# NVlabs/InstantSplat

Hardware: AMD Instinct MI355X
Metric: train_iters_per_sec (higher is better)
Workload: dtype f32

## Files before the change

### include/mi355gs.h

```cpp
#ifndef MI355GS_H
#define MI355GS_H

#include <stddef.h>
#include <stdint.h>

#ifdef __cplusplus
extern "C" {
#endif

#define MI355GS_ABI_VERSION 10

#define MI355GS_OK 0
#define MI355GS_EINVAL (-1)
#define MI355GS_ELAUNCH (-2)
#define MI355GS_EOVERFLOW (-3)

int mi355gs_abi_version(void);
const char* mi355gs_error_string(int code);

size_t mi355gs_raster_geom_bytes(int P);
size_t mi355gs_raster_tiles_bytes(int W, int H);
size_t mi355gs_raster_binning_bytes(int64_t num_instances, int W, int H);

int mi355gs_raster_forward_preprocess(
    void* stream, int P, int D, int M, int W, int H,
    const float* means3D, const float* shs, const float* shs_rest, const float* colors_precomp, const float* opacities,
    const float* scales, float scale_modifier, const float* rotations, const float* cov3D_precomp,
    const float* viewmatrix, const float* projmatrix, const float* campos,
    float tanfovx, float tanfovy, int prefiltered,
    int32_t* radii, void* geom, void* tiles, int32_t* num_rendered, uint8_t* visible, void* grad_scratch, int debug);

int mi355gs_raster_forward_render(
    void* stream, int P, int W, int H, int64_t capacity, const float* bg,
    const void* geom, void* tiles, void* binning, float* out_color, int debug);

size_t mi355gs_raster_binning_bytes_render_only(int64_t num_instances, int W, int H);
int mi355gs_raster_forward_render_only(
    void* stream, int P, int W, int H, int64_t capacity, const float* bg,
    const void* geom, void* tiles, void* binning, float* out_color, int debug);

size_t mi355gs_raster_grad_scratch_bytes(int P);
size_t mi355gs_raster_grad_gate_offset(int P);
int mi355gs_raster_backward(
    void* stream, int P, int D, int M, int W, int H, const float* bg,
    const float* means3D, const float* shs, const float* shs_rest, const float* colors_precomp, const float* opacities,
    const float* scales, float scale_modifier, const float* rotations, const float* cov3D_precomp,
    const float* viewmatrix, const float* projmatrix, const float* campos,
    float tanfovx, float tanfovy,
    const void* geom, void* tiles, const void* binning, int64_t capacity, const int32_t* radii,
    const float* out_color, const float* dL_dpix, void* grad_scratch,
    float* dL_dmeans3D, float* dL_dmeans2D, float* dL_dshs, float* dL_dshs_rest, float* dL_dcolors, float* dL_dopacities,
    float* dL_dscales, float* dL_drotations, float* dL_dcov3D, int grad_scratch_is_clear, int debug);

int mi355gs_raster_mark_visible(void* stream, int P, const float* means3D, const float* viewmatrix,
                                const float* projmatrix, uint8_t* present);

int mi355gs_raster_frame_stats(void* stream, int W, int H, const void* tiles, int64_t* stats);

int mi355gs_tune_min_units(int min_units);

int mi355gs_tune_deterministic(int on);

int mi355gs_tune_scale_grad(int mode);

int mi355gs_profile_begin(void);
int mi355gs_profile_set_period(int every);
int mi355gs_profile_work_counters(void* counters);
int mi355gs_profile_read(int kind, double* total_ms, int* launches);
int mi355gs_profile_end(void);
int mi355gs_profile_ranges(int on);

size_t mi355gs_ssim_scratch_bytes(int B, int C, int H, int W);
int mi355gs_ssim_forward(void* stream, int B, int C, int H, int W, const float* img1, const float* img2,
                         float* dm_dmu1, float* dm_dsigma1_sq, float* dm_dsigma12,
                         void* scratch, float* ssim_mean, float* l1_mean, int padding_valid);
int mi355gs_ssim_backward(void* stream, int B, int C, int H, int W, const float* img1, const float* img2,
                          const float* dm_dmu1, const float* dm_dsigma1_sq, const float* dm_dsigma12,
                          const float* ssim_grad_scale, const float* l1_grad_scale, float* dL_dimg1, int padding_valid);
int mi355gs_l1_ssim_loss_fused(void* stream, int B, int C, int H, int W, const float* img1, const float* img2, void* scratch,
                               float lambda_dssim, float* ssim_mean, float* l1_mean, float* loss, float* dloss_dimg1);

size_t mi355gs_l1_scratch_bytes(int64_t n);
int mi355gs_l1_loss_forward(void* stream, int64_t n, const float* a, const float* b, void* scratch, float* mean_out);
int mi355gs_l1_loss_backward(void* stream, int64_t n, const float* a, const float* b, const float* grad_scale, float* d_a);
#define MI355GS_LOSS_PROGRAM_MAX 16
#define MI355GS_LOSS_OP_L1 0
#define MI355GS_LOSS_OP_SSIM 1
#define MI355GS_LOSS_OP_MULK 2
#define MI355GS_LOSS_OP_ADDK 3
#define MI355GS_LOSS_OP_RSUBK 4
#define MI355GS_LOSS_OP_DIVK 5
#define MI355GS_LOSS_OP_NEG 6
#define MI355GS_LOSS_OP_ADD 7
#define MI355GS_LOSS_OP_SUB 8
int mi355gs_l1_ssim_pair_forward(void* stream, int B, int C, int H, int W, const float* img1, const float* img2, void* scratch,
                                 float* dssim_dimg1);
int mi355gs_l1_ssim_pair_backward(void* stream, int64_t n, const float* img1, const float* img2, const float* dssim_dimg1,
                                  const float* g_l1, float c_l1, const float* g_ssim, float c_ssim, float* d_img1);
int mi355gs_loss_program_eval(void* stream, int n_ops, const int32_t* ops, const float* consts, int B, int C, int H, int W,
                              const void* scratch, float* ssim_mean, float* l1_mean, float* out, float* host_out, float ticket);
int mi355gs_loss_program_eval_grad(void* stream, int n_ops, const int32_t* ops, const float* consts, int B, int C, int H, int W,
                                   const void* scratch, float* ssim_mean, float* l1_mean, float* out, float* host_out, float ticket,
                                   const float* img1, const float* img2, const float* dssim_dimg1, float c_l1, float c_ssim, float* d_img1);

size_t mi355gs_knn_scratch_bytes(int N);
int mi355gs_knn_dist2(void* stream, int N, const float* points, float* mean_dist2, void* scratch);

int mi355gs_adam_step(void* stream, int64_t n, int row, float* param, const float* grad, float* exp_avg,
                      float* exp_avg_sq, const float* per_point_lr, const float* grad_sumsq,
                      float lr, float beta1, float beta2, float eps, int step);

int mi355gs_adam_multi_step(void* stream, int ntensors, const int64_t* numel, const int32_t* row, float* const* params,
                            const float* const* grads, float* const* exp_avg, float* const* exp_avg_sq,
                            const float* const* per_point_lr, const float* lr, float beta1, float beta2, float eps,
                            const int32_t* step, float* scratch, const float* gate, const int32_t* gate_index,
                            uint32_t* live, uint32_t seq);

int mi355gs_pose_forward(void* stream, int P, const float* xyz, const float* rot, const float* scaling,
                         const float* opacity_logit, const float* pose, float* means_cam, float* rot_cam, float* scales,
                         float* opac);
int mi355gs_pose_backward(void* stream, int P, const float* xyz, const float* rot, const float* scales, const float* opac,
                          const float* pose, const float* g_means, const float* g_rot, const float* g_scales,
                          const float* g_opac, float* d_xyz, float* d_rot, float* d_scaling, float* d_opacity_logit,
                          float* d_pose, float* scratch);

int mi355gs_posed_forward_preprocess(void* stream, int P, int D, int W, int H, const float* xyz, const float* f_dc,
                                     const float* f_rest, const float* opacity_logit, const float* log_scales, float scale_modifier,
                                     const float* rotation, const float* pose, const float* view_identity, const float* projmatrix,
                                     const float* origin, float tanfovx, float tanfovy, int32_t* radii, void* geom, void* tiles,
                                     int32_t* num_rendered, uint8_t* visible, void* grad_scratch, int debug);
int mi355gs_posed_backward(void* stream, int P, int D, int W, int H, const float* bg, const float* xyz, const float* f_dc,
                           const float* f_rest, const float* opacity_logit, const float* log_scales, float scale_modifier,
                           const float* rotation, const float* pose, const float* view_identity, const float* projmatrix,
                           const float* origin, float tanfovx, float tanfovy, const void* geom, void* tiles, const void* binning,
                           int64_t capacity, const int32_t* radii, const float* out_color, const float* dL_dpix,
                           void* grad_scratch, float* pose_scratch, float* d_xyz, float* d_means2D, float* d_f_dc, float* d_f_rest,
                           float* d_opacity_logit, float* d_log_scales, float* d_rotation, float* d_pose, int pose_rows, int pose_row,
                           int grad_scratch_is_clear, int debug);

size_t mi355gs_trainer_workspace_bytes(int P, int W, int H, int V, int64_t capacity);
void* mi355gs_trainer_create(int P, int W, int H, int V, int64_t capacity, float* xyz, float* f_dc, float* f_rest, float* opacity,
                             float* scaling, float* rotation, float* poses, float* const* exp_avg, float* const* exp_avg_sq,
                             const float* per_point_lr, void* workspace);
int mi355gs_trainer_step(void* trainer, void* stream, int view, int sh_degree, const float* gt_image, const float* projmatrix,
                         float tanfovx, float tanfovy, const float* bg, const float* lr, const int32_t* step, float beta1, float beta2, float eps,
                         float lambda_dssim, int do_optimizer_step, float* loss_out, int32_t* num_rendered_out);
int mi355gs_trainer_optimizer_step(void* trainer, void* stream, const float* lr, const int32_t* step, float beta1, float beta2,
                                   float eps, int commit_gate);
void mi355gs_trainer_destroy(void* trainer);
const float* mi355gs_trainer_grad(void* trainer, int k);

#define MI355GS_TRACKER_STATE_FLOATS 40
#define MI355GS_TRACKER_POSE 0
#define MI355GS_TRACKER_EXP_AVG 8
#define MI355GS_TRACKER_EXP_AVG_SQ 16
#define MI355GS_TRACKER_BEST 24
#define MI355GS_TRACKER_INITIAL 25
#define MI355GS_TRACKER_FLAG 26
#define MI355GS_TRACKER_COUNT 27
#define MI355GS_TRACKER_CAND 32
size_t mi355gs_tracker_workspace_bytes(int P, int W, int H, int64_t capacity);
void* mi355gs_tracker_create(int P, int M, int W, int H, int64_t capacity, const float* xyz, const float* f_dc, const float* f_rest,
                             const float* opacity, const float* scaling, const float* rotation, void* workspace);
int mi355gs_tracker_count(void* tracker, void* stream, int sh_degree, const float* projmatrix, float tanfovx, float tanfovy,
                          const float* pose, int32_t* count_out);
int mi355gs_tracker_run(void* tracker, void* stream, int sh_degree, const float* gt_image, const float* projmatrix, float tanfovx,
                        float tanfovy, const float* bg, const float* sched, int num_iter, int first_iter, int n_iters, float* state,
                        float* pose_trace, float* loss_trace, float* grad_trace);
void mi355gs_tracker_destroy(void* tracker);

int mi355gs_rgb8_from_planar(void* stream, int H, int W, const float* img, uint8_t* out);
size_t mi355gs_path_workspace_bytes(int P, int W, int H, int64_t capacity);
void* mi355gs_path_create(int P, int M, int W, int H, int64_t capacity, const float* xyz, const float* f_dc, const float* f_rest,
                          const float* opacity, const float* scaling, const float* rotation, void* workspace);
int mi355gs_path_render(void* path, void* stream, int sh_degree, const float* projmatrix, float tanfovx, float tanfovy,
                        const float* bg, const float* poses, int first, int n, uint8_t* frames, int32_t* counts);
void mi355gs_path_destroy(void* path);

size_t mi355gs_metrics_rgb8_scratch_bytes(int N, int H, int W);
int mi355gs_metrics_rgb8(void* stream, int N, int H, int W, const uint8_t* a, const uint8_t* b, void* scratch, int64_t* sq_sum,
                         float* ssim_mean);

size_t mi355gs_lpips_vgg_scratch_bytes(int N, int H, int W, const int channels[5]);
int mi355gs_lpips_vgg_rgb8(void* stream, int N, int H, int W, const uint8_t* a, const uint8_t* b, const int channels[5],
                           const float* weights, void* scratch, float* lpips, float* taps);

size_t mi355gs_png_rgb8_scratch_bytes(int N, int H, int W, int rows_per_block);
size_t mi355gs_png_rgb8_stream_bytes(int N, int H, int W, int rows_per_block);
int mi355gs_png_rgb8(void* stream, int N, int H, int W, int rows_per_block, const uint8_t* frames, void* scratch, uint8_t* out,
                     int64_t* offsets);

size_t mi355gs_jpeg_rgb8_scratch_bytes(int N, int H, int W, int subsampling);
size_t mi355gs_jpeg_rgb8_stream_bytes(int N, int H, int W, int subsampling);
int mi355gs_jpeg_rgb8(void* stream, int N, int H, int W, int subsampling, const uint8_t* qtables, const uint8_t* frames, void* scratch,
                      uint8_t* out, size_t out_bytes, int64_t* offsets);

size_t mi355gs_pointmap_stats_scratch_bytes(int V, int H, int W);
int mi355gs_pointmap_stats(void* stream, int V, int H, int W, const float* depthmaps, const float* confidences, uint8_t* overlap,
                           void* scratch, double* stats);
int mi355gs_covis_masks(void* stream, int V, int H, int W, const int32_t* order, const float* pointmaps, const float* depthmaps,
                        const float* intrinsics, const float* w2c, const double* stats, float depth_threshold, uint8_t* overlap);
size_t mi355gs_compact_scratch_bytes(int64_t n);
int mi355gs_compact_pointmaps(void* stream, int64_t n, const uint8_t* overlap, const float* pointmaps, const float* images,
                              const float* confidences, void* scratch, float* out_points, uint8_t* out_rgb8, float* out_confidence,
                              int32_t* count_dev, int32_t* count_host);

#define MI355GS_ALIGN_OPT_DEPTH 1
#define MI355GS_ALIGN_OPT_IM_POSES 2
#define MI355GS_ALIGN_OPT_FOCALS 4
#define MI355GS_ALIGN_OPT_PW_POSES 8
#define MI355GS_ALIGN_NORM_PW_SCALE 16
size_t mi355gs_align_workspace_bytes(int V, int H, int W, int E, int flags);
void* mi355gs_align_create(void* workspace, int V, int H, int W, const int32_t* edges, int E, int flags, float base_scale);
void mi355gs_align_destroy(void* handle);
int mi355gs_align_pack(void* handle, void* stream, const float* pred_i, const float* pred_j, const float* conf_i, const float* conf_j);
int mi355gs_align_grad(void* handle, void* stream, const float* depth_log, const float* im_pose, const float* focal_log, const float* pp_raw,
                       const float* pw_pose, float* g_depth_log, float* g_im_pose, float* g_focal_log, float* g_pw_pose, float* loss);
int mi355gs_align_run(void* handle, void* stream, int niter, const float* step_table, float* depth_log, float* im_pose, float* focal_log,
                      const float* pp_raw, float* pw_pose, float* m_depth_log, float* v_depth_log, float* m_im_pose, float* v_im_pose,
                      float* m_focal_log, float* v_focal_log, float* m_pw_pose, float* v_pw_pose, float* losses);
int mi355gs_align_points(void* handle, void* stream, const float* depth_log, const float* im_pose, const float* focal_log,
                         const float* pp_raw, const float* pw_pose, float* pts3d, float* depth);
const float* mi355gs_align_records(void* handle);

size_t mi355gs_align_init_workspace_bytes(int B, int n);
int mi355gs_align_init_means(void* workspace, void* stream, int rows, int n, const float* x, float* means);
int mi355gs_align_init_register(void* workspace, void* stream, int B, int n, const float* src, const int32_t* src_idx, long long src_job_stride,
                                int src_pt_stride, const float* tgt, const int32_t* tgt_idx, long long tgt_job_stride, const float* weights,
                                const int32_t* w_idx, long long w_job_stride, float* srt, float* pw_pose);
int mi355gs_align_init_apply(void* stream, int n, const float* src, int src_pt_stride, const float* srt, float* dst);
int mi355gs_align_init_focals(void* workspace, void* stream, int B, int H, int W, const float* src, const int32_t* src_idx,
                              long long src_job_stride, int src_pt_stride, float* focals);
int mi355gs_align_init_state(void* workspace, void* stream, int V, int E, int H, int W, int norm_pw_scale, float base_scale, int focal_mode,
                             float known_focal, const float* srt, const int32_t* pose_row, const float* focals, const int32_t* focal_row,
                             const float* pw_pose, float* pts3d, float* depth_log, float* im_pose, float* focal_log);

#ifdef __cplusplus
}
#endif
#endif
```

### instantsplat_amd/_lib.py

```python
from __future__ import annotations

import ctypes
import os
from ctypes import c_float, c_int, c_int64, c_size_t, c_void_p

import torch

_HERE = os.path.dirname(os.path.abspath(__file__))
LIB_PATH = os.path.join(_HERE, "lib", "libmi355gs.so")
_LIB = None
_TEST_MODE = False

_P = c_void_p
_SIGNATURES = {
    "mi355gs_abi_version": (c_int, []),
    "mi355gs_error_string": (ctypes.c_char_p, [c_int]),
    "mi355gs_raster_geom_bytes": (c_size_t, [c_int]),
    "mi355gs_raster_tiles_bytes": (c_size_t, [c_int, c_int]),
    "mi355gs_raster_binning_bytes": (c_size_t, [c_int64, c_int, c_int]),
    "mi355gs_raster_grad_scratch_bytes": (c_size_t, [c_int]),
    "mi355gs_raster_grad_gate_offset": (c_size_t, [c_int]),
    "mi355gs_raster_forward_preprocess": (c_int, [_P, c_int, c_int, c_int, c_int, c_int, _P, _P, _P, _P, _P, _P, c_float, _P, _P,
                                                  _P, _P, _P, c_float, c_float, c_int, _P, _P, _P, _P, _P, _P, c_int]),
    "mi355gs_raster_forward_render": (c_int, [_P, c_int, c_int, c_int, c_int64, _P, _P, _P, _P, _P, c_int]),
    "mi355gs_raster_binning_bytes_render_only": (c_size_t, [c_int64, c_int, c_int]),
    "mi355gs_raster_forward_render_only": (c_int, [_P, c_int, c_int, c_int, c_int64, _P, _P, _P, _P, _P, c_int]),
    "mi355gs_raster_backward": (c_int, [_P, c_int, c_int, c_int, c_int, c_int, _P, _P, _P, _P, _P, _P, _P, c_float, _P, _P, _P, _P,
                                        _P, c_float, c_float, _P, _P, _P, c_int64, _P, _P, _P, _P, _P, _P, _P, _P, _P, _P, _P, _P, _P,
                                        c_int, c_int]),
    "mi355gs_raster_mark_visible": (c_int, [_P, c_int, _P, _P, _P, _P]),
    "mi355gs_raster_frame_stats": (c_int, [_P, c_int, c_int, _P, _P]),
    "mi355gs_tune_min_units": (c_int, [c_int]),
    "mi355gs_tune_scale_grad": (c_int, [c_int]),
    "mi355gs_tune_deterministic": (c_int, [c_int]),
    "mi355gs_profile_begin": (c_int, []),
    "mi355gs_profile_set_period": (c_int, [c_int]),
    "mi355gs_profile_work_counters": (c_int, [_P]),
    "mi355gs_profile_read": (c_int, [c_int, ctypes.POINTER(ctypes.c_double), ctypes.POINTER(c_int)]),
    "mi355gs_profile_end": (c_int, []),
    "mi355gs_profile_ranges": (c_int, [c_int]),
    "mi355gs_ssim_scratch_bytes": (c_size_t, [c_int, c_int, c_int, c_int]),
    "mi355gs_ssim_forward": (c_int, [_P, c_int, c_int, c_int, c_int, _P, _P, _P, _P, _P, _P, _P, _P, c_int]),
    "mi355gs_ssim_backward": (c_int, [_P, c_int, c_int, c_int, c_int, _P, _P, _P, _P, _P, _P, _P, _P, c_int]),
    "mi355gs_l1_ssim_loss_fused": (c_int, [_P, c_int, c_int, c_int, c_int, _P, _P, _P, c_float, _P, _P, _P, _P]),
    "mi355gs_l1_ssim_pair_forward": (c_int, [_P, c_int, c_int, c_int, c_int, _P, _P, _P, _P]),
    "mi355gs_l1_ssim_pair_backward": (c_int, [_P, c_int64, _P, _P, _P, _P, c_float, _P, c_float, _P]),
    "mi355gs_loss_program_eval": (c_int, [_P, c_int, _P, _P, c_int, c_int, c_int, c_int, _P, _P, _P, _P, _P, c_float]),
    "mi355gs_loss_program_eval_grad": (c_int, [_P, c_int, _P, _P, c_int, c_int, c_int, c_int, _P, _P, _P, _P, _P, c_float, _P, _P, _P, c_float,
                                               c_float, _P]),
    "mi355gs_knn_scratch_bytes": (c_size_t, [c_int]),
    "mi355gs_knn_dist2": (c_int, [_P, c_int, _P, _P, _P]),
    "mi355gs_adam_step": (c_int, [_P, c_int64, c_int, _P, _P, _P, _P, _P, _P, c_float, c_float, c_float, c_float, c_int]),
    "mi355gs_adam_multi_step": (c_int, [_P, c_int, _P, _P, _P, _P, _P, _P, _P, _P, c_float, c_float, c_float, _P, _P, _P, _P, _P,
                                        ctypes.c_uint32]),
    "mi355gs_pose_forward": (c_int, [_P, c_int, _P, _P, _P, _P, _P, _P, _P, _P, _P]),
    "mi355gs_pose_backward": (c_int, [_P, c_int, _P, _P, _P, _P, _P, _P, _P, _P, _P, _P, _P, _P, _P, _P, _P]),
    "mi355gs_posed_forward_preprocess": (c_int, [_P, c_int, c_int, c_int, c_int, _P, _P, _P, _P, _P, c_float, _P, _P, _P, _P, _P,
                                                 c_float, c_float, _P, _P, _P, _P, _P, _P, c_int]),
    "mi355gs_posed_backward": (c_int, [_P, c_int, c_int, c_int, c_int, _P, _P, _P, _P, _P, _P, c_float, _P, _P, _P, _P, _P, c_float,
                                       c_float, _P, _P, _P, c_int64, _P, _P, _P, _P, _P, _P, _P, _P, _P, _P, _P, _P, _P, c_int, c_int, c_int, c_int]),
    "mi355gs_l1_scratch_bytes": (c_size_t, [c_int64]),
    "mi355gs_l1_loss_forward": (c_int, [_P, c_int64, _P, _P, _P, _P]),
    "mi355gs_l1_loss_backward": (c_int, [_P, c_int64, _P, _P, _P, _P]),
    "mi355gs_trainer_workspace_bytes": (c_size_t, [c_int, c_int, c_int, c_int, c_int64]),
    "mi355gs_trainer_create": (c_void_p, [c_int, c_int, c_int, c_int, c_int64, _P, _P, _P, _P, _P, _P, _P, _P, _P, _P, _P]),
    "mi355gs_trainer_step": (c_int, [_P, _P, c_int, c_int, _P, _P, c_float, c_float, _P, _P, _P, c_float, c_float, c_float, c_float,
                                     c_int, _P, _P]),
    "mi355gs_trainer_optimizer_step": (c_int, [_P, _P, _P, _P, c_float, c_float, c_float, c_int]),
    "mi355gs_trainer_destroy": (None, [_P]),
    "mi355gs_trainer_grad": (_P, [_P, c_int]),
    "mi355gs_tracker_workspace_bytes": (c_size_t, [c_int, c_int, c_int, c_int64]),
    "mi355gs_tracker_create": (c_void_p, [c_int, c_int, c_int, c_int, c_int64, _P, _P, _P, _P, _P, _P, _P]),
    "mi355gs_tracker_count": (c_int, [_P, _P, c_int, _P, c_float, c_float, _P, _P]),
    "mi355gs_tracker_run": (c_int, [_P, _P, c_int, _P, _P, c_float, c_float, _P, _P, c_int, c_int, c_int, _P, _P, _P, _P]),
    "mi355gs_tracker_destroy": (None, [_P]),
    "mi355gs_rgb8_from_planar": (c_int, [_P, c_int, c_int, _P, _P]),
    "mi355gs_path_workspace_bytes": (c_size_t, [c_int, c_int, c_int, c_int64]),
    "mi355gs_path_create": (c_void_p, [c_int, c_int, c_int, c_int, c_int64, _P, _P, _P, _P, _P, _P, _P]),
    "mi355gs_path_render": (c_int, [_P, _P, c_int, _P, c_float, c_float, _P, _P, c_int, c_int, _P, _P]),
    "mi355gs_path_destroy": (None, [_P]),
    "mi355gs_metrics_rgb8_scratch_bytes": (c_size_t, [c_int, c_int, c_int]),
    "mi355gs_metrics_rgb8": (c_int, [_P, c_int, c_int, c_int, _P, _P, _P, _P, _P]),
    "mi355gs_png_rgb8_scratch_bytes": (c_size_t, [c_int, c_int, c_int, c_int]),
    "mi355gs_png_rgb8_stream_bytes": (c_size_t, [c_int, c_int, c_int, c_int]),
    "mi355gs_png_rgb8": (c_int, [_P, c_int, c_int, c_int, c_int, _P, _P, _P, _P]),
    "mi355gs_jpeg_rgb8_scratch_bytes": (c_size_t, [c_int, c_int, c_int, c_int]),
    "mi355gs_jpeg_rgb8_stream_bytes": (c_size_t, [c_int, c_int, c_int, c_int]),
    "mi355gs_jpeg_rgb8": (c_int, [_P, c_int, c_int, c_int, c_int, _P, _P, _P, _P, c_size_t, _P]),
    "mi355gs_lpips_vgg_scratch_bytes": (c_size_t, [c_int, c_int, c_int, _P]),
    "mi355gs_lpips_vgg_rgb8": (c_int, [_P, c_int, c_int, c_int, _P, _P, _P, _P, _P, _P, _P]),
    "mi355gs_pointmap_stats_scratch_bytes": (c_size_t, [c_int, c_int, c_int]),
    "mi355gs_pointmap_stats": (c_int, [_P, c_int, c_int, c_int, _P, _P, _P, _P, _P]),
    "mi355gs_covis_masks": (c_int, [_P, c_int, c_int, c_int, _P, _P, _P, _P, _P, _P, c_float, _P]),
    "mi355gs_compact_scratch_bytes": (c_size_t, [c_int64]),
    "mi355gs_compact_pointmaps": (c_int, [_P, c_int64, _P, _P, _P, _P, _P, _P, _P, _P, _P, _P]),
    "mi355gs_align_workspace_bytes": (c_size_t, [c_int, c_int, c_int, c_int, c_int]),
    "mi355gs_align_create": (c_void_p, [_P, c_int, c_int, c_int, _P, c_int, c_int, c_float]),
    "mi355gs_align_destroy": (None, [_P]),
    "mi355gs_align_pack": (c_int, [_P, _P, _P, _P, _P, _P]),
    "mi355gs_align_grad": (c_int, [_P] * 12),
    "mi355gs_align_run": (c_int, [_P, _P, c_int] + [_P] * 15),
    "mi355gs_align_points": (c_int, [_P] * 9),
    "mi355gs_align_records": (c_void_p, [_P]),
    "mi355gs_align_init_workspace_bytes": (c_size_t, [c_int, c_int]),
    "mi355gs_align_init_means": (c_int, [_P, _P, c_int, c_int, _P, _P]),
    "mi355gs_align_init_register": (c_int, [_P, _P, c_int, c_int, _P, _P, c_int64, c_int, _P, _P, c_int64, _P, _P, c_int64, _P, _P]),
    "mi355gs_align_init_apply": (c_int, [_P, c_int, _P, c_int, _P, _P]),
    "mi355gs_align_init_focals": (c_int, [_P, _P, c_int, c_int, c_int, _P, _P, c_int64, c_int, _P]),
    "mi355gs_align_init_state": (c_int, [_P, _P, c_int, c_int, c_int, c_int, c_int, c_float, c_int, c_float] + [_P] * 9),
}
EXPORTED_SYMBOLS = tuple(_SIGNATURES)


ABI_VERSION = 10


def _bind(path: str):
    lib = ctypes.CDLL(path)
    for name, (res, args) in _SIGNATURES.items():
        fn = getattr(lib, name)
        fn.restype, fn.argtypes = res, args
    got = lib.mi355gs_abi_version()
    if got != ABI_VERSION:
        raise RuntimeError(f"{path} implements ABI v{got}, this package binds v{ABI_VERSION}: rebuild it with "
                           "`python -c 'import __graft_entry__ as g; g.build()'`")
    return lib


def lib():
    global _LIB
    if _LIB is None:
        if not os.path.exists(LIB_PATH):
            raise RuntimeError(
                f"{LIB_PATH} is missing: build it with `python -c 'import __graft_entry__ as g; g.build()'` "
                "(hipcc --offload-arch=gfx950). instantsplat_amd has no CPU or PyTorch fallback.")
        _LIB = _bind(LIB_PATH)
        if os.environ.get("MI355GS_DETERMINISTIC", "0") == "1":
            _LIB.mi355gs_tune_deterministic(1)
    return _LIB


def _use_library_for_testing(path: str | None):
    global _LIB, _TEST_MODE, _EXT_BOUND_TO
    if path is None:
        _LIB, _TEST_MODE = None, False
    else:
        _LIB, _TEST_MODE = _bind(path), True
    _EXT_BOUND_TO = None


BINDING = os.environ.get("MI355GS_BINDING", "compiled")
EXT_PATH = os.path.join(_HERE, "lib", "_mi355gs_torch.so")
_EXT = None
_EXT_BOUND_TO = None


def compiled():
    global _EXT, _EXT_BOUND_TO
    if BINDING != "compiled":
        return None
    L = lib()
    if _EXT_BOUND_TO is L:
        return _EXT
    if _EXT is None:
        if not os.path.exists(EXT_PATH):
            raise RuntimeError(f"{EXT_PATH} is missing: build it with `python -c 'import __graft_entry__ as g; g.build()'` "
                               "(or set MI355GS_BINDING=ctypes to use the Python binding)")
        import importlib.util
        spec = importlib.util.spec_from_file_location("_mi355gs_torch", EXT_PATH)
        _EXT = importlib.util.module_from_spec(spec)
        spec.loader.exec_module(_EXT)
    _EXT.forget_gates()
    _EXT.bind({name: ctypes.cast(getattr(L, name), ctypes.c_void_p).value for name in _EXT.abi_symbols()}, _TEST_MODE)
    _EXT_BOUND_TO = L
    return _EXT


def check(code: int, what: str):
    if code != 0:
        raise RuntimeError(f"mi355gs: {what} failed: {lib().mi355gs_error_string(code).decode()} ({code})")


def ptr(t: torch.Tensor | None):
    return None if t is None else t.data_ptr()


_F32 = torch.float32


def f32c_on_one_device(*tensors):
    out, dev = [], None
    for t in tensors:
        if t.dtype is not _F32:
            raise RuntimeError(f"expected float32, got {t.dtype}")
        if not t.is_contiguous():
            t = t.contiguous()
        d = t.device
        if dev is None:
            if d.type != "cuda" and not _TEST_MODE:
                raise RuntimeError("instantsplat_amd operators run on the GPU only (got a CPU tensor; there is no CPU fallback)")
            dev = d
        elif d != dev:
            raise RuntimeError(f"tensors on different devices: {dev} vs {d}")
        out.append(t)
    return out, dev


def require_device(*tensors: torch.Tensor | None):
    dev = None
    for t in tensors:
        if t is None:
            continue
        if not t.is_cuda and not _TEST_MODE:
            raise RuntimeError("instantsplat_amd operators run on the GPU only (got a CPU tensor; there is no CPU fallback)")
        if not t.is_contiguous():
            raise RuntimeError("instantsplat_amd operators need contiguous tensors")
        if dev is None:
            dev = t.device
        elif t.device != dev:
            raise RuntimeError(f"tensors on different devices: {dev} vs {t.device}")
    return dev


class _NoGuard:
    def __enter__(self):
        return None

    def __exit__(self, *a):
        return False


_NO_GUARD = _NoGuard()


def on_device(device):
    if device is not None and device.type == "cuda" and device.index is not None and device.index != torch.cuda.current_device():
        return torch.cuda.device(device)
    return _NO_GUARD


def stream_ptr(device):
    if device is not None and device.type == "cuda":
        return torch.cuda.current_stream(device).cuda_stream
    return None


def f32c(t: torch.Tensor | None):
    if t is None:
        return None
    if t.dtype != torch.float32:
        raise RuntimeError(f"expected float32, got {t.dtype}")
    return t.contiguous()
```

### instantsplat_amd/csrc/ssim.hip

```cpp
#include "common.h"

namespace {

constexpr int TS = 16;
constexpr int TSX = 32;
constexpr int HALO = 5;
constexpr int TH = TS + 2 * HALO;
constexpr int THX = TSX + 2 * HALO;
constexpr int SXP = 48;
constexpr int ROW_ITEMS = TH * TS;
constexpr float C1 = 0.01f * 0.01f;
constexpr float C2 = 0.03f * 0.03f;

__device__ __forceinline__ float gw(int k) {
  constexpr float w[11] = {0.001028380123898387f, 0.0075987582094967365f, 0.036000773310661316f, 0.10936068743467331f,
                           0.21300552785396576f,  0.26601171493530273f,   0.21300552785396576f,  0.10936068743467331f,
                           0.036000773310661316f, 0.0075987582094967365f, 0.001028380123898387f};
  return w[k];
}

__device__ __forceinline__ bool ssim_equal_window(float mu1, float mu2, float exx, float eyy, float exy, bool zero_counts) {
  return mu1 == mu2 && exx == eyy && exx == exy && (zero_counts || exx != 0.f);
}

__device__ __forceinline__ float ssim_rcp(float x) {
  const float r = __builtin_amdgcn_rcpf(x);
  return fmaf(fmaf(-x, r, 1.0f), r, r);
}
__device__ __forceinline__ gs_v2f ssim_rcp(gs_v2f x) { return gs_v2f{ssim_rcp(x[0]), ssim_rcp(x[1])}; }

template <class T> struct SsimWindow { T m, d1, d2, d3, invB; };
__device__ __forceinline__ float ssim_lane(float v, int) { return v; }
__device__ __forceinline__ float ssim_lane(gs_v2f v, int h) { return v[h]; }
__device__ __forceinline__ float ssim_sum_sq(float mu1_sq, float, float mu2_sq) { return mu1_sq + mu2_sq; }
__device__ __forceinline__ gs_v2f ssim_sum_sq(gs_v2f mu1_sq, gs_v2f mu2, gs_v2f mu2_sq) {
#ifdef __clang__
  return __builtin_elementwise_fma(mu2, mu2, mu1_sq);
#else
  return mu1_sq + mu2_sq;
#endif
}
template <class T>
__device__ __forceinline__ T ssim_all(float v) {
  if constexpr (std::is_same<T, float>::value) return v;
  else return T{v, v};
}
template <class T>
__device__ __forceinline__ SsimWindow<T> ssim_window(T mu1, T mu2, T exx, T eyy, T exy) {
  const T two = ssim_all<T>(2.f), c1 = ssim_all<T>(C1), c2 = ssim_all<T>(C2);
  const T mu1_sq = mu1 * mu1, mu2_sq = mu2 * mu2, mu12 = mu1 * mu2;
  const T s1 = exx - mu1_sq, s2 = eyy - mu2_sq, s12 = exy - mu12;
  const T A = ssim_sum_sq(mu1_sq, mu2, mu2_sq) + c1, B = s1 + s2 + c2, Cc = two * mu12 + c1, Dd = two * s12 + c2;
  const T invA = ssim_rcp(A), invB = ssim_rcp(B), invAB = invA * invB;
  const T m = Cc * Dd * invAB;
  const T t = mu1 * two * Cc * Dd * invAB;
  const T d1 = (mu2 * two * Dd) * invAB - (mu2 * two * Cc) * invAB - t * invA + t * invB;
  const T d2 = -m * invB;
  const T d3 = two * Cc * invAB;
  return {m, d1, d2, d3, invB};
}
template <class T>
__device__ __forceinline__ SsimWindow<float> ssim_exact(const SsimWindow<T>& w, int h, bool same) {
  const float invB = ssim_lane(w.invB, h);
  return {same ? 1.f : ssim_lane(w.m, h), same ? 0.f : ssim_lane(w.d1, h), same ? -invB : ssim_lane(w.d2, h),
          same ? 2.f * invB : ssim_lane(w.d3, h), invB};
}

template <int N>
__device__ __forceinline__ void ssim_tile_stage(int tid, int H, int W, int ox, int oy, const float* const (&src)[N], float (*const (&dst)[N])[SXP]) {
  constexpr int ITERS = (TH * SXP + 255) / 256;
  float v[N][ITERS];
#pragma unroll
  for (int j = 0; j < ITERS; ++j) {
    const int i = tid + 256 * j, r = i / SXP, c = i - r * SXP;
    const size_t o = (size_t)min(max(oy + r - HALO, 0), H - 1) * W + min(max(ox + c - HALO, 0), W - 1);
#pragma unroll
    for (int p = 0; p < N; ++p) v[p][j] = src[p][o];
  }
#pragma unroll
  for (int j = 0; j < ITERS; ++j) {
    const int i = tid + 256 * j, r = i / SXP, c = i - r * SXP;
    const int gy = oy + r - HALO, gx = ox + c - HALO;
    const bool in = c < THX && gy >= 0 && gy < H && gx >= 0 && gx < W;
    if (i < TH * SXP) {
#pragma unroll
      for (int p = 0; p < N; ++p) dst[p][r][c] = in ? v[p][j] : 0.f;
    }
  }
}

__device__ __forceinline__ void ssim_tile_row_pass(int tid, const float (*s_x)[SXP], const float (*s_y)[SXP], gs_v2f (*s_h)[TH][TS]) {
  for (int i = tid; i < ROW_ITEMS; i += 256) {
    const int r = i >> 4, c = i & 15;
    gs_v2f sx = {0.f, 0.f}, sy = sx, sxx = sx, syy = sx, sxy = sx;
#pragma unroll
    for (int k = 0; k < 11; ++k) {
      const gs_v2f w = {gw(k), gw(k)};
      const gs_v2f x = {s_x[r][c + k], s_x[r][c + TS + k]}, y = {s_y[r][c + k], s_y[r][c + TS + k]};
      const gs_v2f wx = w * x, wy = w * y;
      sx = gs_fma2(w, x, sx); sy = gs_fma2(w, y, sy);
      sxx = gs_fma2(wx, x, sxx); syy = gs_fma2(wy, y, syy); sxy = gs_fma2(wx, y, sxy);
    }
    s_h[0][r][c] = sx; s_h[1][r][c] = sy; s_h[2][r][c] = sxx; s_h[3][r][c] = syy; s_h[4][r][c] = sxy;
  }
}
template <int N>
__device__ __forceinline__ void ssim_tile_col_pass(const gs_v2f (*s_h)[TH][TS], int ly, int lx, gs_v2f (&out)[N]) {
#pragma unroll
  for (int m = 0; m < N; ++m) out[m] = gs_v2f{0.f, 0.f};
#pragma unroll
  for (int k = 0; k < 11; ++k) {
    const gs_v2f w = {gw(k), gw(k)};
#pragma unroll
    for (int m = 0; m < N; ++m) out[m] = gs_fma2(w, s_h[m][ly + k][lx], out[m]);
  }
}

__global__ __launch_bounds__(256) void k_ssim_fwd(int H, int W, const float* __restrict__ img1, const float* __restrict__ img2,
                                                   float* __restrict__ dm_dmu1, float* __restrict__ dm_dsigma1_sq,
                                                   float* __restrict__ dm_dsigma12, float* __restrict__ partial ,
                                                   int crop ) {
  __shared__ float s_x[TH][SXP];
  __shared__ float s_y[TH][SXP];
  __shared__ gs_v2f s_h[5][TH][TS];
  __shared__ float s_red[2][4];
  const int tid = threadIdx.y * TS + threadIdx.x;
  const int plane = blockIdx.z;
  const int ox = blockIdx.x * TSX, oy = blockIdx.y * TS;
  const float* p1 = img1 + (size_t)plane * H * W;
  const float* p2 = img2 + (size_t)plane * H * W;
  ssim_tile_stage<2>(tid, H, W, ox, oy, {p1, p2}, {s_x, s_y});
  __syncthreads();
  ssim_tile_row_pass(tid, s_x, s_y, s_h);
  __syncthreads();
  const int ly = threadIdx.y, lx = threadIdx.x;
  float val = 0.f, l1 = 0.f;
  {
    gs_v2f mo[5];
    ssim_tile_col_pass(s_h, ly, lx, mo);
    const SsimWindow<gs_v2f> pair = ssim_window(mo[0], mo[1], mo[2], mo[3], mo[4]);
    const int gy = oy + ly;
#pragma unroll
    for (int half = 0; half < 2; ++half) {
      const int gx = ox + lx + half * TS;
      if (gx < W && gy < H) {
        const bool counted = gx >= crop && gx < W - crop && gy >= crop && gy < H - crop;
        const bool same = ssim_equal_window(mo[0][half], mo[1][half], mo[2][half], mo[3][half], mo[4][half], false);
        const SsimWindow<float> win = ssim_exact(pair, half, same);
        val += counted ? win.m : 0.f;
        const size_t o = (size_t)plane * H * W + (size_t)gy * W + gx;
        if (dm_dmu1) {
          dm_dmu1[o] = counted ? win.d1 : 0.f;
          dm_dsigma1_sq[o] = counted ? win.d2 : 0.f;
          dm_dsigma12[o] = counted ? win.d3 : 0.f;
        }
        l1 += fabsf(s_x[ly + HALO][lx + half * TS + HALO] - s_y[ly + HALO][lx + half * TS + HALO]);
      }
    }
  }
  val = gs_wave_sum_row3(val);
  l1 = gs_wave_sum_row3(l1);
  const int wave = tid >> 6, lane = tid & 63;
  if (lane == 63) { s_red[0][wave] = val; s_red[1][wave] = l1; }
  __syncthreads();
  if (tid == 0) {
    const size_t b = ((size_t)blockIdx.z * gridDim.y + blockIdx.y) * gridDim.x + blockIdx.x;
    partial[2 * b] = (s_red[0][0] + s_red[0][1]) + (s_red[0][2] + s_red[0][3]);
    partial[2 * b + 1] = (s_red[1][0] + s_red[1][1]) + (s_red[1][2] + s_red[1][3]);
  }
}

__global__ __launch_bounds__(1024) void k_ssim_finish(int nblocks, double inv_n, const float* __restrict__ partial,
                                                       float* __restrict__ ssim_mean, float* __restrict__ l1_mean,
                                                       float* __restrict__ loss, float lambda_dssim) {
  float sm, lm;
  gs_finish_two_means(nblocks, inv_n, partial, sm, lm);
  if (threadIdx.x == 0) {
    if (ssim_mean) *ssim_mean = sm;
    if (l1_mean) *l1_mean = lm;
    if (loss) *loss = gs_l1_ssim_loss(lambda_dssim, lm, sm);
  }
}

__global__ __launch_bounds__(256) void k_ssim_bwd(int H, int W, float inv_n, const float* __restrict__ img1, const float* __restrict__ img2,
                                                   const float* __restrict__ dm_dmu1, const float* __restrict__ dm_dsigma1_sq,
                                                   const float* __restrict__ dm_dsigma12, const float* __restrict__ ssim_scale,
                                                   const float* __restrict__ l1_scale, float ssim_scale_host, float l1_scale_host,
                                                   float* __restrict__ dL_dimg1) {
  __shared__ float s_a[TH][SXP];
  __shared__ float s_b[TH][SXP];
  __shared__ float s_c[TH][SXP];
  __shared__ gs_v2f s_h[3][TH][TS];
  const int tid = threadIdx.y * TS + threadIdx.x;
  const int plane = blockIdx.z;
  const int ox = blockIdx.x * TSX, oy = blockIdx.y * TS;
  const size_t po = (size_t)plane * H * W;
  const float ks = (ssim_scale ? *ssim_scale : 1.f) * ssim_scale_host * inv_n;
  const float kl = (l1_scale ? *l1_scale : 1.f) * l1_scale_host * inv_n;
  float px[2], py[2];
#pragma unroll
  for (int half = 0; half < 2; ++half) {
    const size_t o = po + (size_t)min(oy + (int)threadIdx.y, H - 1) * W + min(ox + (int)threadIdx.x + half * TS, W - 1);
    px[half] = img1[o]; py[half] = img2[o];
  }
  if (ks != 0.f) {
    ssim_tile_stage<3>(tid, H, W, ox, oy, {dm_dmu1 + po, dm_dsigma1_sq + po, dm_dsigma12 + po}, {s_a, s_b, s_c});
    __syncthreads();
    for (int i = tid; i < ROW_ITEMS; i += 256) {
      const int r = i >> 4, c = i & 15;
      gs_v2f a = {0.f, 0.f}, b = a, cc = a;
#pragma unroll
      for (int k = 0; k < 11; ++k) {
        const gs_v2f w = {gw(k), gw(k)};
        a = gs_fma2(w, gs_v2f{s_a[r][c + k], s_a[r][c + TS + k]}, a);
        b = gs_fma2(w, gs_v2f{s_b[r][c + k], s_b[r][c + TS + k]}, b);
        cc = gs_fma2(w, gs_v2f{s_c[r][c + k], s_c[r][c + TS + k]}, cc);
      }
      s_h[0][r][c] = a; s_h[1][r][c] = b; s_h[2][r][c] = cc;
    }
    __syncthreads();
  }
  const int ly = threadIdx.y, lx = threadIdx.x;
  const int gy = oy + ly;
  if (gy >= H) return;
  gs_v2f abc[3] = {{0.f, 0.f}, {0.f, 0.f}, {0.f, 0.f}};
  if (ks != 0.f) ssim_tile_col_pass(s_h, ly, lx, abc);
  const gs_v2f a = abc[0], b = abc[1], cc = abc[2];
#pragma unroll
  for (int half = 0; half < 2; ++half) {
    const int gx = ox + lx + half * TS;
    if (gx >= W) continue;
    const size_t o = po + (size_t)gy * W + gx;
    const float x = px[half], y = py[half];
    float g = 0.f;
    if (ks != 0.f) g = ks * ((x == y && cc[half] == -2.f * b[half]) ? a[half] : a[half] + 2.f * x * b[half] + y * cc[half]);
    if (kl != 0.f) {
      const float d = x - y;
      g += kl * (d > 0.f ? 1.f : (d < 0.f ? -1.f : 0.f));
    }
    dL_dimg1[o] = g;
  }
}


constexpr int FT = 32;
constexpr int FR1 = FT + 2 * HALO;
constexpr int FR2 = FT + 4 * HALO;
constexpr int FXP = 58;
constexpr int FHP = 43;
constexpr int FDP = 46;
constexpr int FEP = 33;
constexpr int FTHREADS = 512;
constexpr int F_STAGE_ITERS = (FR2 * FXP + FTHREADS - 1) / FTHREADS;
constexpr int FER = FT * FT / FTHREADS;
constexpr int FCR = 7, FC_GROUPS = (FR1 + FCR - 1) / FCR;
constexpr int FDR = 8, FD_GROUPS = FT / FDR;
static_assert(FC_GROUPS * FR1 <= FTHREADS && FD_GROUPS * FR1 <= FTHREADS && FT % FDR == 0 && FDR % 2 == 0, "one item per thread");

template <int RUN>
__device__ __forceinline__ void ssim_run(const float (&v)[RUN + 10], float (&out)[RUN]) {
#pragma unroll
  for (int j = 0; j < RUN; ++j) {
    float a = 0.f;
#pragma unroll
    for (int k = 0; k < 11; ++k) a = fmaf(gw(k), v[j + k], a);
    out[j] = a;
  }
}

__global__ __launch_bounds__(FTHREADS) void k_l1_ssim_fused(int H, int W, const float* __restrict__ img1, const float* __restrict__ img2,
                                                        float ks , float kl ,
                                                        float* __restrict__ dL_dimg1, float* __restrict__ partial ) {
  __shared__ float s_xy[2][FR2][FXP];
  __shared__ float s_h[5][FR2][FHP];
  static_assert(3 * FR1 * FDP <= 2 * FR2 * FXP && 3 * FR1 * FEP <= 5 * FR2 * FHP, "aliased LDS buffers must fit");
  __shared__ float s_red[2][FTHREADS / 64];
  float (*s_d)[FR1][FDP] = reinterpret_cast<float (*)[FR1][FDP]>(&s_xy[0][0][0]);
  float (*s_e)[FR1][FEP] = reinterpret_cast<float (*)[FR1][FEP]>(&s_h[0][0][0]);
  const int tid = threadIdx.x;
  const int plane = blockIdx.z;
  const int ox = blockIdx.x * FT, oy = blockIdx.y * FT;
  const size_t po = (size_t)plane * H * W;
  const float* p1 = img1 + po;
  const float* p2 = img2 + po;
  const int ec = tid & 31, er0 = (tid >> 5) * FER;
  float ex[FER], ey[FER];
#pragma unroll
  for (int j = 0; j < FER; ++j) {
    const size_t o = (size_t)min(oy + er0 + j, H - 1) * W + min(ox + ec, W - 1);
    ex[j] = p1[o]; ey[j] = p2[o];
  }
  {
    float vx[F_STAGE_ITERS], vy[F_STAGE_ITERS];
#pragma unroll
    for (int j = 0; j < F_STAGE_ITERS; ++j) {
      const int i = tid + FTHREADS * j, r = i / FXP, c = i - r * FXP;
      const size_t o = (size_t)min(max(oy + r - 2 * HALO, 0), H - 1) * W + min(max(ox + c - 2 * HALO, 0), W - 1);
      vx[j] = p1[o]; vy[j] = p2[o];
    }
#pragma unroll
    for (int j = 0; j < F_STAGE_ITERS; ++j) {
      const int i = tid + FTHREADS * j, r = i / FXP, c = i - r * FXP;
      const int gy = oy + r - 2 * HALO, gx = ox + c - 2 * HALO;
      const bool in = gy >= 0 && gy < H && gx >= 0 && gx < W;
      if (i < FR2 * FXP) { s_xy[0][r][c] = in ? vx[j] : 0.f; s_xy[1][r][c] = in ? vy[j] : 0.f; }
    }
  }
  __syncthreads();
  for (int i = tid; i < FR2 * 7; i += FTHREADS) {
    const int r = i % FR2, c0 = (i / FR2) * 6;
    float x[16], y[16];
#pragma unroll
    for (int t = 0; t < 16; t += 2) {
      const float2 a = *reinterpret_cast<const float2*>(&s_xy[0][r][c0 + t]);
      const float2 b = *reinterpret_cast<const float2*>(&s_xy[1][r][c0 + t]);
      x[t] = a.x; x[t + 1] = a.y; y[t] = b.x; y[t + 1] = b.y;
    }
    float sx[6], sy[6], sxx[6], syy[6], sxy[6];
#pragma unroll
    for (int j = 0; j < 6; ++j) { sx[j] = sy[j] = sxx[j] = syy[j] = sxy[j] = 0.f; }
#pragma unroll
    for (int t = 0; t < 16; ++t) {
      const float xx = x[t] * x[t], yy = y[t] * y[t], xy = x[t] * y[t];
#pragma unroll
      for (int j = 0; j < 6; ++j) {
        const int k = t - j;
        if (k >= 0 && k < 11) {
          const float w = gw(k);
          sx[j] = fmaf(w, x[t], sx[j]); sy[j] = fmaf(w, y[t], sy[j]);
          sxx[j] = fmaf(w, xx, sxx[j]); syy[j] = fmaf(w, yy, syy[j]); sxy[j] = fmaf(w, xy, sxy[j]);
        }
      }
    }
#pragma unroll
    for (int j = 0; j < 6; ++j) {
      s_h[0][r][c0 + j] = sx[j]; s_h[1][r][c0 + j] = sy[j]; s_h[2][r][c0 + j] = sxx[j]; s_h[3][r][c0 + j] = syy[j];
      s_h[4][r][c0 + j] = sxy[j];
    }
  }
  __syncthreads();
  float val = 0.f;
  if (tid < FR1 * FC_GROUPS) {
    const int c = tid % FR1, r0 = (tid / FR1) * FCR;
    float mo[5][FCR];
#pragma unroll
    for (int m = 0; m < 5; ++m) {
      float v[FCR + 10];
#pragma unroll
      for (int t = 0; t < FCR + 10; ++t) v[t] = s_h[m][min(r0 + t, FR2 - 1)][c];
      ssim_run(v, mo[m]);
    }
    const int gx = ox + c - HALO;
#pragma unroll
    for (int j = 0; j < FCR; ++j) {
      const int r = r0 + j, gy = oy + r - HALO;
      const SsimWindow<float> win = ssim_exact(ssim_window(mo[0][j], mo[1][j], mo[2][j], mo[3][j], mo[4][j]), 0,
                                               ssim_equal_window(mo[0][j], mo[1][j], mo[2][j], mo[3][j], mo[4][j], false));
      const bool in_img = gx >= 0 && gx < W && gy >= 0 && gy < H && r < FR1;
      mo[0][j] = in_img ? win.d1 : 0.f; mo[1][j] = in_img ? win.d2 : 0.f; mo[2][j] = in_img ? win.d3 : 0.f;
      const bool in_tile = c >= HALO && c < HALO + FT && r >= HALO && r < HALO + FT;
      val += (in_img && in_tile) ? win.m : 0.f;
    }
#pragma unroll
    for (int j = 0; j < FCR; ++j)
      if (FR1 % FCR == 0 || r0 + j < FR1) { s_d[0][r0 + j][c] = mo[0][j]; s_d[1][r0 + j][c] = mo[1][j]; s_d[2][r0 + j][c] = mo[2][j]; }
  }
  __syncthreads();
  if (tid < FR1 * FD_GROUPS) {
    const int r = tid % FR1, c0 = (tid / FR1) * FDR;
#pragma unroll
    for (int m = 0; m < 3; ++m) {
      float v[FDR + 10];
#pragma unroll
      for (int t = 0; t < FDR + 10; t += 2) {
        const float2 a = *reinterpret_cast<const float2*>(&s_d[m][r][c0 + t]);
        v[t] = a.x; v[t + 1] = a.y;
      }
      float e[FDR];
      ssim_run(v, e);
#pragma unroll
      for (int j = 0; j < FDR; ++j) s_e[m][r][c0 + j] = e[j];
    }
  }
  __syncthreads();
  float l1 = 0.f;
  {
    float out[3][FER];
#pragma unroll
    for (int m = 0; m < 3; ++m) {
      float v[FER + 10];
#pragma unroll
      for (int t = 0; t < FER + 10; ++t) v[t] = s_e[m][er0 + t][ec];
      ssim_run(v, out[m]);
    }
    const int gx = ox + ec;
#pragma unroll
    for (int j = 0; j < FER; ++j) {
      const int gy = oy + er0 + j;
      if (gx < W && gy < H) {
        const float x = ex[j], y = ey[j], d = x - y;
        l1 += fabsf(d);
        const float gs = (d == 0.f && out[2][j] == -2.f * out[1][j]) ? out[0][j] : out[0][j] + 2.f * x * out[1][j] + y * out[2][j];
        const float g = ks * gs + kl * (d > 0.f ? 1.f : (d < 0.f ? -1.f : 0.f));
        dL_dimg1[po + (size_t)gy * W + gx] = g;
      }
    }
  }
  val = gs_wave_sum_row3(val);
  l1 = gs_wave_sum_row3(l1);
  const int wave = tid >> 6, lane = tid & 63;
  if (lane == 63) { s_red[0][wave] = val; s_red[1][wave] = l1; }
  __syncthreads();
  if (tid == 0) {
    const size_t b = ((size_t)blockIdx.z * gridDim.y + blockIdx.y) * gridDim.x + blockIdx.x;
    float ta = 0.f, tb = 0.f;
#pragma unroll
    for (int w = 0; w < FTHREADS / 64; ++w) { ta += s_red[0][w]; tb += s_red[1][w]; }
    partial[2 * b] = ta;
    partial[2 * b + 1] = tb;
  }
}

constexpr int L1_THREADS = 256, L1_PER_THREAD = 16;
__global__ __launch_bounds__(L1_THREADS) void k_l1_partial(long long n, const float* __restrict__ a, const float* __restrict__ b,
                                                           float* __restrict__ partial) {
  __shared__ float s_red[L1_THREADS / 64];
  const long long base = (long long)blockIdx.x * (L1_THREADS * L1_PER_THREAD);
  float acc = 0.f;
  const bool vec = ((((uintptr_t)a | (uintptr_t)b) & 15) == 0) && base + L1_THREADS * L1_PER_THREAD <= n;
  if (vec) {
#pragma unroll
    for (int r = 0; r < L1_PER_THREAD / 4; ++r) {
      const long long j = (base >> 2) + threadIdx.x + (long long)L1_THREADS * r;
      const float4 x = reinterpret_cast<const float4*>(a)[j], y = reinterpret_cast<const float4*>(b)[j];
      acc += (fabsf(x.x - y.x) + fabsf(x.y - y.y)) + (fabsf(x.z - y.z) + fabsf(x.w - y.w));
    }
  } else {
    for (int r = 0; r < L1_PER_THREAD; ++r) {
      const long long i = base + threadIdx.x + (long long)L1_THREADS * r;
      if (i < n) acc += fabsf(a[i] - b[i]);
    }
  }
  acc = gs_wave_sum_row3(acc);
  if ((threadIdx.x & 63) == 63) s_red[threadIdx.x >> 6] = acc;
  __syncthreads();
  if (threadIdx.x == 0) {
    partial[2 * blockIdx.x] = (s_red[0] + s_red[1]) + (s_red[2] + s_red[3]);
    partial[2 * blockIdx.x + 1] = 0.f;
  }
}

__global__ __launch_bounds__(256) void k_l1_bwd(long long n, const float* __restrict__ a, const float* __restrict__ b,
                                                const float* __restrict__ grad_scale, float n_as_float, float* __restrict__ d_a) {
  const float s = *grad_scale / n_as_float;
  const long long i0 = ((long long)blockIdx.x * 256 + threadIdx.x) * 4;
  if (((((uintptr_t)a | (uintptr_t)b | (uintptr_t)d_a) & 15) == 0) && i0 + 4 <= n) {
    const float4 x = reinterpret_cast<const float4*>(a)[i0 >> 2], y = reinterpret_cast<const float4*>(b)[i0 >> 2];
    auto sg = [&](float d) { return d > 0.f ? s : (d < 0.f ? -s : 0.f); };
    reinterpret_cast<float4*>(d_a)[i0 >> 2] = make_float4(sg(x.x - y.x), sg(x.y - y.y), sg(x.z - y.z), sg(x.w - y.w));
  } else {
    for (long long i = i0; i < min(n, i0 + 4); ++i) { const float d = a[i] - b[i]; d_a[i] = d > 0.f ? s : (d < 0.f ? -s : 0.f); }
  }
}

struct GsLossProgram {
  int n;
  signed char op[MI355GS_LOSS_PROGRAM_MAX];
  float k[MI355GS_LOSS_PROGRAM_MAX];
};

__device__ __forceinline__ void loss_program_body(const GsLossProgram& p, int nblocks, double inv_n, const float* __restrict__ partial,
                                                  float* __restrict__ ssim_mean, float* __restrict__ l1_mean, float* __restrict__ out,
                                                  float* __restrict__ host_out, float ticket) {
#pragma clang fp contract(off)
  float sm, lm;
  gs_finish_two_means(nblocks, inv_n, partial, sm, lm);
  if (threadIdx.x != 0) return;
  *ssim_mean = sm; *l1_mean = lm;
  float st[MI355GS_LOSS_PROGRAM_MAX];
  int sp = 0;
  for (int i = 0; i < p.n; ++i) {
    const float k = p.k[i];
    switch (p.op[i]) {
      case MI355GS_LOSS_OP_L1: st[sp++] = lm; break;
      case MI355GS_LOSS_OP_SSIM: st[sp++] = sm; break;
      case MI355GS_LOSS_OP_MULK: st[sp - 1] = st[sp - 1] * k; break;
      case MI355GS_LOSS_OP_ADDK: st[sp - 1] = st[sp - 1] + k; break;
      case MI355GS_LOSS_OP_RSUBK: st[sp - 1] = k - st[sp - 1]; break;
      case MI355GS_LOSS_OP_DIVK: st[sp - 1] = st[sp - 1] * (1.0f / k); break;
      case MI355GS_LOSS_OP_NEG: st[sp - 1] = -st[sp - 1]; break;
      case MI355GS_LOSS_OP_ADD: st[sp - 2] = st[sp - 2] + st[sp - 1]; --sp; break;
      case MI355GS_LOSS_OP_SUB: st[sp - 2] = st[sp - 2] - st[sp - 1]; --sp; break;
      default: break;
    }
  }
  const float value = sp > 0 ? st[sp - 1] : 0.f;
  *out = value;
  if (host_out) {
    typedef float v2f __attribute__((vector_size(8)));
    v2f both = {value, ticket};
    *reinterpret_cast<v2f*>(host_out) = both;
  }
}

__global__ __launch_bounds__(1024) void k_loss_program(GsLossProgram p, int nblocks, double inv_n, const float* __restrict__ partial,
                                                      float* __restrict__ ssim_mean, float* __restrict__ l1_mean, float* __restrict__ out,
                                                      float* __restrict__ host_out, float ticket) {
  loss_program_body(p, nblocks, inv_n, partial, ssim_mean, l1_mean, out, host_out, ticket);
}

__device__ __forceinline__ void loss_pair_bwd_four(long long n, long long i0, const float* __restrict__ a, const float* __restrict__ b,
                                                   const float* __restrict__ dssim, float gl, float c_l1, float gs, float c_ssim,
                                                   float n_as_float, float* __restrict__ d_a) {
#pragma clang fp contract(off)
  const float sl = (gl * c_l1) / n_as_float;
  const float ss = gs * c_ssim;
  const bool use_l1 = c_l1 != 0.0f, use_ss = c_ssim != 0.0f && dssim != nullptr;
  auto one = [&](float x, float y, float ds) {
    const float d = x - y;
    const float tl = use_l1 ? (d > 0.f ? sl : (d < 0.f ? -sl : 0.f)) : 0.f;
    return use_ss ? tl + ss * ds : tl;
  };
  const uintptr_t al = (uintptr_t)a | (uintptr_t)b | (uintptr_t)d_a | (uintptr_t)(use_ss ? dssim : a);
  if (((al & 15) == 0) && i0 + 4 <= n) {
    const float4 x = reinterpret_cast<const float4*>(a)[i0 >> 2], y = reinterpret_cast<const float4*>(b)[i0 >> 2];
    const float4 s = use_ss ? reinterpret_cast<const float4*>(dssim)[i0 >> 2] : make_float4(0.f, 0.f, 0.f, 0.f);
    reinterpret_cast<float4*>(d_a)[i0 >> 2] = make_float4(one(x.x, y.x, s.x), one(x.y, y.y, s.y), one(x.z, y.z, s.z), one(x.w, y.w, s.w));
  } else {
    for (long long i = i0; i < min(n, i0 + 4); ++i) d_a[i] = one(a[i], b[i], use_ss ? dssim[i] : 0.f);
  }
}

__global__ __launch_bounds__(256) void k_loss_pair_bwd(long long n, const float* __restrict__ a, const float* __restrict__ b,
                                                       const float* __restrict__ dssim, const float* __restrict__ g_l1, float c_l1,
                                                       const float* __restrict__ g_ssim, float c_ssim, float n_as_float,
                                                       float* __restrict__ d_a) {
#pragma clang fp contract(off)
  loss_pair_bwd_four(n, ((long long)blockIdx.x * 256 + threadIdx.x) * 4, a, b, dssim, g_l1 ? *g_l1 : 1.0f, c_l1, g_ssim ? *g_ssim : 1.0f, c_ssim,
                     n_as_float, d_a);
}

__global__ __launch_bounds__(1024) void k_loss_program_grad(GsLossProgram p, int nblocks, double inv_n, const float* __restrict__ partial,
                                                           float* __restrict__ ssim_mean, float* __restrict__ l1_mean, float* __restrict__ out,
                                                           float* __restrict__ host_out, float ticket, long long n,
                                                           const float* __restrict__ a, const float* __restrict__ b,
                                                           const float* __restrict__ dssim, float c_l1, float c_ssim, float n_as_float,
                                                           float* __restrict__ d_a) {
#pragma clang fp contract(off)
  if (blockIdx.x == 0) {
    loss_program_body(p, nblocks, inv_n, partial, ssim_mean, l1_mean, out, host_out, ticket);
    return;
  }
  loss_pair_bwd_four(n, ((long long)(blockIdx.x - 1) * 1024 + threadIdx.x) * 4, a, b, dssim, 1.0f, c_l1, 1.0f, c_ssim, n_as_float, d_a);
}

constexpr int MB_ROW_BYTES = THX * 3;
constexpr int MB_ROW_WORDS = 32;
constexpr int MB_BYTE_ITERS = (TH * MB_ROW_BYTES + 255) / 256;
constexpr int MB_WORD_ITERS = (TH * MB_ROW_WORDS + 255) / 256;
static_assert(MB_ROW_WORDS * 4 >= MB_ROW_BYTES + 1 && (TSX * 3) % 4 == 0, "a staged row fits the aligned words");

__global__ __launch_bounds__(256) void k_metrics_rgb8(int H, int W, const uint8_t* __restrict__ a, const uint8_t* __restrict__ b,
                                                      float* __restrict__ part_ssim, uint32_t* __restrict__ part_sq, int aligned) {
  __shared__ float s_lut[256];
  __shared__ float s_x[3][TH][SXP];
  __shared__ float s_y[3][TH][SXP];
  __shared__ gs_v2f s_h[5][TH][TS];
  __shared__ float s_red[4];
  __shared__ uint32_t s_redu[4];
  const int tid = threadIdx.y * TS + threadIdx.x;
  const int ox = blockIdx.x * TSX, oy = blockIdx.y * TS;
  const int row_bytes = 3 * W;
  const size_t frame = (size_t)blockIdx.z * (size_t)H * (size_t)row_bytes;
  const uint8_t* __restrict__ pa = a + frame;
  const uint8_t* __restrict__ pb = b + frame;
  s_lut[tid] = (float)tid / 255.0f;
  uint32_t sq = 0;
  if (aligned) {
    uint32_t va[MB_WORD_ITERS], vb[MB_WORD_ITERS];
#pragma unroll
    for (int j = 0; j < MB_WORD_ITERS; ++j) {
      const int i = tid + 256 * j, r = min(i >> 5, TH - 1), w = i & 31;
      const int gy = min(max(oy + r - HALO, 0), H - 1), off = min(max(3 * ox - 16 + 4 * w, 0), row_bytes - 4);
      const size_t o = (size_t)gy * row_bytes + off;
      va[j] = *reinterpret_cast<const uint32_t*>(pa + o); vb[j] = *reinterpret_cast<const uint32_t*>(pb + o);
    }
    __syncthreads();
#pragma unroll
    for (int j = 0; j < MB_WORD_ITERS; ++j) {
      const int i = tid + 256 * j, r = i >> 5, w = i & 31;
      if (i >= TH * MB_ROW_WORDS) break;
      const int gy = oy + r - HALO, off = 3 * ox - 16 + 4 * w;
      const bool in = gy >= 0 && gy < H && off >= 0 && off < row_bytes;
      const uint32_t wa = in ? va[j] : 0u, wb = in ? vb[j] : 0u;
#pragma unroll
      for (int k = 0; k < 4; ++k) {
        const int p = 4 * w + k - 1;
        if (p < 0 || p >= MB_ROW_BYTES) continue;
        const int c = p / 3, ch = p - 3 * c;
        const uint32_t ba = (wa >> (8 * k)) & 255u, bb = (wb >> (8 * k)) & 255u;
        s_x[ch][r][c] = s_lut[ba]; s_y[ch][r][c] = s_lut[bb];
        if (r >= HALO && r < HALO + TS && c >= HALO && c < HALO + TSX) { const int d = (int)ba - (int)bb; sq += (uint32_t)(d * d); }
      }
    }
  } else {
    uint8_t va[MB_BYTE_ITERS], vb[MB_BYTE_ITERS];
#pragma unroll
    for (int j = 0; j < MB_BYTE_ITERS; ++j) {
      const int i = tid + 256 * j, r = min(i / MB_ROW_BYTES, TH - 1), p = i - (i / MB_ROW_BYTES) * MB_ROW_BYTES;
      const int gy = min(max(oy + r - HALO, 0), H - 1), off = min(max(3 * (ox - HALO) + p, 0), row_bytes - 1);
      const size_t o = (size_t)gy * row_bytes + off;
      va[j] = pa[o]; vb[j] = pb[o];
    }
    __syncthreads();
#pragma unroll
    for (int j = 0; j < MB_BYTE_ITERS; ++j) {
      const int i = tid + 256 * j, r = i / MB_ROW_BYTES, p = i - r * MB_ROW_BYTES;
      if (i >= TH * MB_ROW_BYTES) break;
      const int gy = oy + r - HALO, off = 3 * (ox - HALO) + p;
      const bool in = gy >= 0 && gy < H && off >= 0 && off < row_bytes;
      const int c = p / 3, ch = p - 3 * c;
      const uint32_t ba = in ? (uint32_t)va[j] : 0u, bb = in ? (uint32_t)vb[j] : 0u;
      s_x[ch][r][c] = s_lut[ba]; s_y[ch][r][c] = s_lut[bb];
      if (r >= HALO && r < HALO + TS && c >= HALO && c < HALO + TSX) { const int d = (int)ba - (int)bb; sq += (uint32_t)(d * d); }
    }
  }
  __syncthreads();
  const int ly = threadIdx.y, lx = threadIdx.x;
  const int gy = oy + ly;
  float val = 0.f;
  for (int ch = 0; ch < 3; ++ch) {
    if (ch) __syncthreads();
    ssim_tile_row_pass(tid, s_x[ch], s_y[ch], s_h);
    __syncthreads();
    gs_v2f mo[5];
    ssim_tile_col_pass(s_h, ly, lx, mo);
    const gs_v2f mu1 = mo[0], mu2 = mo[1], exx = mo[2], eyy = mo[3], exy = mo[4];
    const gs_v2f two = {2.f, 2.f}, c1 = {C1, C1}, c2 = {C2, C2};
    const gs_v2f mu1_sq = mu1 * mu1, mu2_sq = mu2 * mu2, mu12 = mu1 * mu2;
    const gs_v2f s1 = exx - mu1_sq, s2 = eyy - mu2_sq, s12 = exy - mu12;
    const gs_v2f A = ssim_sum_sq(mu1_sq, mu2, mu2_sq) + c1, B = s1 + s2 + c2, Cc = two * mu12 + c1, Dd = two * s12 + c2;
    const gs_v2f m = Cc * Dd * (ssim_rcp(A) * ssim_rcp(B));
#pragma unroll
    for (int half = 0; half < 2; ++half) {
      const bool same = ssim_equal_window(mu1[half], mu2[half], exx[half], eyy[half], exy[half], true);
      if (ox + lx + half * TS < W && gy < H) val += same ? 1.f : m[half];
    }
  }
  val = gs_wave_sum_row3(val);
  sq = gs_wave_sum_row3(sq);
  const int wave = tid >> 6, lane = tid & 63;
  if (lane == 63) { s_red[wave] = val; s_redu[wave] = sq; }
  __syncthreads();
  if (tid == 0) {
    const size_t t = ((size_t)blockIdx.z * gridDim.y + blockIdx.y) * gridDim.x + blockIdx.x;
    part_ssim[t] = (s_red[0] + s_red[1]) + (s_red[2] + s_red[3]);
    part_sq[t] = (s_redu[0] + s_redu[1]) + (s_redu[2] + s_redu[3]);
  }
}

__global__ __launch_bounds__(256) void k_metrics_rgb8_finish(int tiles, double n, const float* __restrict__ part_ssim,
                                                             const uint32_t* __restrict__ part_sq, int64_t* __restrict__ sq_sum,
                                                             float* __restrict__ ssim_mean) {
  __shared__ double s_a[4];
  __shared__ unsigned long long s_q[4];
  const size_t base = (size_t)blockIdx.x * (size_t)tiles;
  double acc = 0.0;
  unsigned long long q = 0;
  for (int i = threadIdx.x; i < tiles; i += 256) { acc += (double)part_ssim[base + i]; q += part_sq[base + i]; }
  acc = gs_wave_sum_row3(acc); q = gs_wave_sum_row3(q);
  const int wave = threadIdx.x >> 6, lane = threadIdx.x & 63;
  if (lane == 63) { s_a[wave] = acc; s_q[wave] = q; }
  __syncthreads();
  if (threadIdx.x == 0) {
    ssim_mean[blockIdx.x] = (float)((((s_a[0] + s_a[1]) + s_a[2]) + s_a[3]) / n);
    sq_sum[blockIdx.x] = (int64_t)(((s_q[0] + s_q[1]) + s_q[2]) + s_q[3]);
  }
}

}

static inline int l1_nblocks(long long n) { return (int)((n + L1_THREADS * L1_PER_THREAD - 1) / (L1_THREADS * L1_PER_THREAD)); }

static inline int ssim_nblocks(int B, int C, int H, int W) { return B * C * ((H + TS - 1) / TS) * ((W + TSX - 1) / TSX); }
static inline int fused_nblocks(int B, int C, int H, int W) { return B * C * ((H + FT - 1) / FT) * ((W + FT - 1) / FT); }

static inline bool planes_ok(int B, int C, int H, int W) { return B > 0 && C > 0 && H > 0 && W > 0 && (size_t)B * C <= 65535; }
static inline dim3 plane_grid(int planes, int H, int W, int tw, int th) { return dim3((W + tw - 1) / tw, (H + th - 1) / th, planes); }

static int launch_l1_ssim_fused(hipStream_t stream, int planes, int H, int W, const float* img1, const float* img2, float ks, float kl,
                                float* dL_dimg1, void* scratch, const char* name) {
  const int debug = 0;
  {
    GsProfScope prof(3, stream);
    GS_KRANGE(name);
    hipLaunchKernelGGL(k_l1_ssim_fused, plane_grid(planes, H, W, FT, FT), dim3(FTHREADS), 0, stream, H, W, img1, img2, ks, kl, dL_dimg1,
                       (float*)scratch);
  }
  GS_CHECK_LAUNCH(name);
  return MI355GS_OK;
}
static int launch_l1_ssim_loss(hipStream_t stream, int planes, int H, int W, const float* img1, const float* img2, float lambda_dssim,
                               float* dL_dimg1, void* scratch) {
  const double inv_n = 1.0 / ((double)planes * H * W);
  return launch_l1_ssim_fused(stream, planes, H, W, img1, img2, (float)(-(double)lambda_dssim * inv_n),
                              (float)((1.0 - (double)lambda_dssim) * inv_n), dL_dimg1, scratch, "l1_ssim_fused");
}

extern "C" {

size_t mi355gs_ssim_scratch_bytes(int B, int C, int H, int W) {
  if (B <= 0 || C <= 0 || H <= 0 || W <= 0) return 256;
  return gs_align((size_t)ssim_nblocks(B, C, H, W) * 2 * sizeof(float));
}

int mi355gs_ssim_forward(void* stream_, int B, int C, int H, int W, const float* img1, const float* img2, float* dm_dmu1,
                         float* dm_dsigma1_sq, float* dm_dsigma12, void* scratch, float* ssim_mean, float* l1_mean, int padding_valid) {
  GS_RANGE();
  hipStream_t stream = (hipStream_t)stream_;
  const int debug = 0;
  if (!planes_ok(B, C, H, W) || !img1 || !img2 || !scratch) return MI355GS_EINVAL;
  const int crop = padding_valid ? HALO : 0;
  if (padding_valid && (l1_mean || H <= 2 * HALO || W <= 2 * HALO)) return MI355GS_EINVAL;
  if ((dm_dmu1 == nullptr) != (dm_dsigma1_sq == nullptr) || (dm_dmu1 == nullptr) != (dm_dsigma12 == nullptr)) return MI355GS_EINVAL;
  GS_KRANGE("ssim_fwd");
  hipLaunchKernelGGL(k_ssim_fwd, plane_grid(B * C, H, W, TSX, TS), dim3(TS, TS), 0, stream, H, W, img1, img2, dm_dmu1, dm_dsigma1_sq, dm_dsigma12,
                     (float*)scratch, crop);
  GS_CHECK_LAUNCH("ssim_fwd");
  const double inv_n = 1.0 / ((double)B * C * (H - 2 * crop) * (W - 2 * crop));
  GS_KRANGE("ssim_finish");
  hipLaunchKernelGGL(k_ssim_finish, dim3(1), dim3(1024), 0, stream, ssim_nblocks(B, C, H, W), inv_n, (const float*)scratch, ssim_mean,
                     l1_mean, (float*)nullptr, 0.f);
  GS_CHECK_LAUNCH("ssim_finish");
  return MI355GS_OK;
}

int mi355gs_ssim_backward(void* stream_, int B, int C, int H, int W, const float* img1, const float* img2, const float* dm_dmu1,
                          const float* dm_dsigma1_sq, const float* dm_dsigma12, const float* ssim_grad_scale,
                          const float* l1_grad_scale, float* dL_dimg1, int padding_valid) {
  GS_RANGE();
  hipStream_t stream = (hipStream_t)stream_;
  const int debug = 0;
  if (!planes_ok(B, C, H, W) || !img1 || !img2 || !dL_dimg1) return MI355GS_EINVAL;
  if (ssim_grad_scale && (!dm_dmu1 || !dm_dsigma1_sq || !dm_dsigma12)) return MI355GS_EINVAL;
  const int crop = padding_valid ? HALO : 0;
  if (padding_valid && (l1_grad_scale || H <= 2 * HALO || W <= 2 * HALO)) return MI355GS_EINVAL;
  const float inv_n = (float)(1.0 / ((double)B * C * (H - 2 * crop) * (W - 2 * crop)));
  GS_KRANGE("ssim_bwd");
  hipLaunchKernelGGL(k_ssim_bwd, plane_grid(B * C, H, W, TSX, TS), dim3(TS, TS), 0, stream, H, W, inv_n, img1, img2, dm_dmu1, dm_dsigma1_sq,
                     dm_dsigma12, ssim_grad_scale, l1_grad_scale, ssim_grad_scale ? 1.f : 0.f, l1_grad_scale ? 1.f : 0.f, dL_dimg1);
  GS_CHECK_LAUNCH("ssim_bwd");
  return MI355GS_OK;
}

size_t mi355gs_l1_scratch_bytes(int64_t n) { return gs_align((size_t)(n > 0 ? l1_nblocks(n) : 1) * 2 * sizeof(float)); }

int mi355gs_l1_loss_forward(void* stream_, int64_t n, const float* a, const float* b, void* scratch, float* mean_out) {
  GS_RANGE();
  hipStream_t stream = (hipStream_t)stream_;
  const int debug = 0;
  if (n <= 0 || n > (int64_t)1 << 40 || !a || !b || !scratch || !mean_out) return MI355GS_EINVAL;
  GS_KRANGE("l1_partial");
  hipLaunchKernelGGL(k_l1_partial, dim3(l1_nblocks(n)), dim3(L1_THREADS), 0, stream, (long long)n, a, b, (float*)scratch);
  GS_CHECK_LAUNCH("l1_partial");
  GS_KRANGE("l1_finish");
  hipLaunchKernelGGL(k_ssim_finish, dim3(1), dim3(1024), 0, stream, l1_nblocks(n), 1.0 / (double)n, (const float*)scratch, mean_out,
                     (float*)nullptr, (float*)nullptr, 0.f);
  GS_CHECK_LAUNCH("l1_finish");
  return MI355GS_OK;
}

int mi355gs_l1_loss_backward(void* stream_, int64_t n, const float* a, const float* b, const float* grad_scale, float* d_a) {
  GS_RANGE();
  hipStream_t stream = (hipStream_t)stream_;
  const int debug = 0;
  if (n <= 0 || n > (int64_t)1 << 40 || !a || !b || !grad_scale || !d_a) return MI355GS_EINVAL;
  GS_KRANGE("l1_bwd");
  hipLaunchKernelGGL(k_l1_bwd, dim3((unsigned)((n + 1023) / 1024)), dim3(256), 0, stream, (long long)n, a, b, grad_scale, (float)n, d_a);
  GS_CHECK_LAUNCH("l1_bwd");
  return MI355GS_OK;
}

int mi355gs_l1_ssim_loss_fused(void* stream_, int B, int C, int H, int W, const float* img1, const float* img2, void* scratch,
                               float lambda_dssim, float* ssim_mean, float* l1_mean, float* loss, float* dloss_dimg1) {
  GS_RANGE();
  hipStream_t stream = (hipStream_t)stream_;
  const int debug = 0;
  if (!planes_ok(B, C, H, W) || !img1 || !img2 || !scratch || !loss || !dloss_dimg1) return MI355GS_EINVAL;
  const int rc = launch_l1_ssim_loss(stream, B * C, H, W, img1, img2, lambda_dssim, dloss_dimg1, scratch);
  if (rc != MI355GS_OK) return rc;
  const double inv_n = 1.0 / ((double)B * C * H * W);
  GS_KRANGE("ssim_finish");
  hipLaunchKernelGGL(k_ssim_finish, dim3(1), dim3(1024), 0, stream, fused_nblocks(B, C, H, W), inv_n, (const float*)scratch, ssim_mean,
                     l1_mean, loss, lambda_dssim);
  GS_CHECK_LAUNCH("ssim_finish");
  return MI355GS_OK;
}

int mi355gs_l1_ssim_pair_forward(void* stream_, int B, int C, int H, int W, const float* img1, const float* img2, void* scratch,
                                 float* dssim_dimg1) {
  GS_RANGE();
  if (!planes_ok(B, C, H, W) || !img1 || !img2 || !scratch || !dssim_dimg1) return MI355GS_EINVAL;
  return launch_l1_ssim_fused((hipStream_t)stream_, B * C, H, W, img1, img2, (float)(1.0 / ((double)B * C * H * W)), 0.0f, dssim_dimg1, scratch,
                              "l1_ssim_pair");
}

int mi355gs_l1_ssim_pair_backward(void* stream_, int64_t n, const float* img1, const float* img2, const float* dssim_dimg1,
                                  const float* g_l1, float c_l1, const float* g_ssim, float c_ssim, float* d_img1) {
  GS_RANGE();
  hipStream_t stream = (hipStream_t)stream_;
  const int debug = 0;
  if (n <= 0 || n > (int64_t)1 << 40 || !img1 || !img2 || !d_img1) return MI355GS_EINVAL;
  if (c_ssim != 0.0f && !dssim_dimg1) return MI355GS_EINVAL;
  GS_KRANGE("loss_pair_bwd");
  hipLaunchKernelGGL(k_loss_pair_bwd, dim3((unsigned)((n + 1023) / 1024)), dim3(256), 0, stream, (long long)n, img1, img2, dssim_dimg1, g_l1,
                     c_l1, g_ssim, c_ssim, (float)n, d_img1);
  GS_CHECK_LAUNCH("loss_pair_bwd");
  return MI355GS_OK;
}

static int build_loss_program(int n_ops, const int32_t* ops, const float* consts, GsLossProgram& p) {
  if (n_ops <= 0 || n_ops > MI355GS_LOSS_PROGRAM_MAX || !ops || !consts) return MI355GS_EINVAL;
  p.n = n_ops;
  int depth = 0;
  for (int i = 0; i < MI355GS_LOSS_PROGRAM_MAX; ++i) {
    p.op[i] = 0; p.k[i] = 0.f;
    if (i >= n_ops) continue;
    const int op = ops[i];
    if (op == MI355GS_LOSS_OP_L1 || op == MI355GS_LOSS_OP_SSIM) ++depth;
    else if (op == MI355GS_LOSS_OP_ADD || op == MI355GS_LOSS_OP_SUB) { if (depth < 2) return MI355GS_EINVAL; --depth; }
    else if (op >= MI355GS_LOSS_OP_MULK && op <= MI355GS_LOSS_OP_NEG) { if (depth < 1) return MI355GS_EINVAL; }
    else return MI355GS_EINVAL;
    p.op[i] = (signed char)op; p.k[i] = consts[i];
  }
  return depth == 1 ? MI355GS_OK : MI355GS_EINVAL;
}

int mi355gs_loss_program_eval(void* stream_, int n_ops, const int32_t* ops, const float* consts, int B, int C, int H, int W,
                              const void* scratch, float* ssim_mean, float* l1_mean, float* out, float* host_out, float ticket) {
  GS_RANGE();
  hipStream_t stream = (hipStream_t)stream_;
  const int debug = 0;
  if (!scratch || !l1_mean || !ssim_mean || !out) return MI355GS_EINVAL;
  if (B <= 0 || C <= 0 || H <= 0 || W <= 0 || ((uintptr_t)host_out & 7) != 0) return MI355GS_EINVAL;
  GsLossProgram p;
  if (build_loss_program(n_ops, ops, consts, p) != MI355GS_OK) return MI355GS_EINVAL;
  GS_KRANGE("loss_program");
  hipLaunchKernelGGL(k_loss_program, dim3(1), dim3(1024), 0, stream, p, fused_nblocks(B, C, H, W), 1.0 / ((double)B * C * H * W),
                     (const float*)scratch, ssim_mean, l1_mean, out, host_out, ticket);
  GS_CHECK_LAUNCH("loss_program");
  return MI355GS_OK;
}

int mi355gs_loss_program_eval_grad(void* stream_, int n_ops, const int32_t* ops, const float* consts, int B, int C, int H, int W,
                                   const void* scratch, float* ssim_mean, float* l1_mean, float* out, float* host_out, float ticket,
                                   const float* img1, const float* img2, const float* dssim_dimg1, float c_l1, float c_ssim, float* d_img1) {
  GS_RANGE();
  hipStream_t stream = (hipStream_t)stream_;
  const int debug = 0;
  if (!scratch || !l1_mean || !ssim_mean || !out || !img1 || !img2 || !d_img1) return MI355GS_EINVAL;
  if (B <= 0 || C <= 0 || H <= 0 || W <= 0 || ((uintptr_t)host_out & 7) != 0) return MI355GS_EINVAL;
  if (c_ssim != 0.0f && !dssim_dimg1) return MI355GS_EINVAL;
  GsLossProgram p;
  if (build_loss_program(n_ops, ops, consts, p) != MI355GS_OK) return MI355GS_EINVAL;
  const long long n = (long long)B * C * H * W;
  GS_KRANGE("loss_program_grad");
  hipLaunchKernelGGL(k_loss_program_grad, dim3(1u + (unsigned)((n + 4095) / 4096)), dim3(1024), 0, stream, p, fused_nblocks(B, C, H, W),
                     1.0 / (double)n, (const float*)scratch, ssim_mean, l1_mean, out, host_out, ticket, n, img1, img2, dssim_dimg1, c_l1, c_ssim,
                     (float)n, d_img1);
  GS_CHECK_LAUNCH("loss_program_grad");
  return MI355GS_OK;
}

static inline bool metrics_rgb8_size_ok(int N, int H, int W) {
  if (N <= 0 || H <= 0 || W <= 0 || N > 65535 || H > 65535 * TS) return false;
  if ((long long)H * W > 0x7fffffffLL / 3) return false;
  return (long long)N * ssim_nblocks(1, 1, H, W) <= 0x7fffffffLL;
}

size_t mi355gs_metrics_rgb8_scratch_bytes(int N, int H, int W) {
  if (!metrics_rgb8_size_ok(N, H, W)) return 0;
  return 2 * gs_align((size_t)N * ssim_nblocks(1, 1, H, W) * sizeof(float));
}

int mi355gs_metrics_rgb8(void* stream_, int N, int H, int W, const uint8_t* a, const uint8_t* b, void* scratch, int64_t* sq_sum,
                         float* ssim_mean) {
  GS_RANGE();
  hipStream_t stream = (hipStream_t)stream_;
  const int debug = 0;
  if (!metrics_rgb8_size_ok(N, H, W) || !a || !b || !scratch || !sq_sum || !ssim_mean) return MI355GS_EINVAL;
  const int tiles = ssim_nblocks(1, 1, H, W);
  float* part_ssim = (float*)scratch;
  uint32_t* part_sq = (uint32_t*)((char*)scratch + gs_align((size_t)N * tiles * sizeof(float)));
  const int aligned = (W % 4 == 0) && ((((uintptr_t)a | (uintptr_t)b) & 3) == 0);
  GS_KRANGE("metrics_rgb8");
  hipLaunchKernelGGL(k_metrics_rgb8, plane_grid(N, H, W, TSX, TS), dim3(TS, TS), 0, stream, H, W, a, b, part_ssim, part_sq, aligned);
  GS_CHECK_LAUNCH("metrics_rgb8");
  GS_KRANGE("metrics_rgb8_finish");
  hipLaunchKernelGGL(k_metrics_rgb8_finish, dim3(N), dim3(256), 0, stream, tiles, 3.0 * (double)H * (double)W, (const float*)part_ssim,
                     (const uint32_t*)part_sq, sq_sum, ssim_mean);
  GS_CHECK_LAUNCH("metrics_rgb8_finish");
  return MI355GS_OK;
}

}

int gs_loss_fused(hipStream_t stream, int C, int H, int W, const float* img1, const float* img2, float lambda_dssim, float* dL_dimg1,
                  void* scratch) {
  return launch_l1_ssim_loss(stream, C, H, W, img1, img2, lambda_dssim, dL_dimg1, scratch);
}
int gs_loss_fused_nblocks(int C, int H, int W) { return fused_nblocks(1, C, H, W); }
```

### instantsplat_amd/csrc_torch/binding.cpp

```cpp
#include <torch/extension.h>
#include <ATen/hip/impl/HIPGuardImplMasqueradingAsCUDA.h>
#include <c10/hip/HIPStream.h>

#include <chrono>
#include <optional>
#include <map>
#include <mutex>

#include "../../include/mi355gs.h"

namespace {

using torch::Tensor;
using torch::autograd::AutogradContext;
using torch::autograd::variable_list;

#define GS_ABI_LIST(X)                                                 \
  X(geom_bytes, mi355gs_raster_geom_bytes)                             \
  X(tiles_bytes, mi355gs_raster_tiles_bytes)                           \
  X(binning_bytes, mi355gs_raster_binning_bytes)                       \
  X(grad_scratch_bytes, mi355gs_raster_grad_scratch_bytes)             \
  X(grad_gate_offset, mi355gs_raster_grad_gate_offset)                 \
  X(posed_forward_preprocess, mi355gs_posed_forward_preprocess)        \
  X(forward_preprocess, mi355gs_raster_forward_preprocess)             \
  X(raster_backward, mi355gs_raster_backward)                          \
  X(forward_render, mi355gs_raster_forward_render)                     \
  X(binning_bytes_render_only, mi355gs_raster_binning_bytes_render_only) \
  X(forward_render_only, mi355gs_raster_forward_render_only)           \
  X(posed_backward, mi355gs_posed_backward)                            \
  X(ssim_scratch_bytes, mi355gs_ssim_scratch_bytes)                    \
  X(l1_ssim_loss_fused, mi355gs_l1_ssim_loss_fused)                    \
  X(l1_scratch_bytes, mi355gs_l1_scratch_bytes)                        \
  X(l1_loss_forward, mi355gs_l1_loss_forward)                          \
  X(l1_loss_backward, mi355gs_l1_loss_backward)                        \
  X(pair_forward, mi355gs_l1_ssim_pair_forward)                        \
  X(pair_backward, mi355gs_l1_ssim_pair_backward)                      \
  X(program_eval, mi355gs_loss_program_eval)                           \
  X(program_eval_grad, mi355gs_loss_program_eval_grad)                 \
  X(ssim_forward, mi355gs_ssim_forward)                                \
  X(ssim_backward, mi355gs_ssim_backward)                              \
  X(adam_multi_step, mi355gs_adam_multi_step)                          \
  X(error_string, mi355gs_error_string)

struct Abi {
#define GS_MEMBER(field, name) decltype(&name) field = nullptr;
  GS_ABI_LIST(GS_MEMBER)
#undef GS_MEMBER
  bool bound = false;
  bool allow_cpu = false;
} g_abi;

std::vector<std::string> abi_symbols() {
#define GS_NAME(field, name) #name,
  return {GS_ABI_LIST(GS_NAME)};
#undef GS_NAME
}

void bind_abi(const std::map<std::string, uintptr_t>& sym, bool allow_cpu_tensors) {
  g_abi.allow_cpu = allow_cpu_tensors;
  auto get = [&](const char* name) {
    auto it = sym.find(name);
    TORCH_CHECK(it != sym.end() && it->second, "mi355gs torch binding: entry point ", name, " was not provided");
    return it->second;
  };
#define GS_BIND(field, name) g_abi.field = reinterpret_cast<decltype(&name)>(get(#name));
  GS_ABI_LIST(GS_BIND)
#undef GS_BIND
  g_abi.bound = true;
}

void check(int code, const char* what) {
  TORCH_CHECK(code == 0, "mi355gs: ", what, " failed: ", g_abi.error_string ? g_abi.error_string(code) : "?", " (", code, ")");
}

struct DeviceScope {
  c10::hip::OptionalHIPGuardMasqueradingAsCUDA guard;
  void* stream = nullptr;
  explicit DeviceScope(const Tensor& t) {
    if (t.is_cuda()) {
      guard.set_device(t.device());
      stream = (void*)c10::hip::getCurrentHIPStream(t.device().index()).stream();
    }
  }
  void synchronize(const Tensor& t) const {
    if (t.is_cuda()) c10::hip::getCurrentHIPStream(t.device().index()).synchronize();
  }
};

void wait_for_count(const int32_t* count, const DeviceScope& dev, const Tensor& t) {
  if (!t.is_cuda()) return;
  std::optional<py::gil_scoped_release> nogil;
  if (PyGILState_Check()) nogil.emplace();
  const auto t0 = std::chrono::steady_clock::now();
  for (unsigned spin = 0;; ++spin) {
    if (*reinterpret_cast<const volatile int32_t*>(count) >= 0) return;
    if ((spin & 1023u) == 1023u && std::chrono::steady_clock::now() - t0 > std::chrono::milliseconds(2)) break;
  }
  dev.synchronize(t);
  TORCH_CHECK(*reinterpret_cast<const volatile int32_t*>(count) >= 0, "mi355gs: the forward did not report its instance count");
}

void wait_for_words(Tensor words, int64_t sentinel, Tensor like, int64_t timeout_us) {
  TORCH_CHECK(words.scalar_type() == at::kInt && !words.is_cuda() && words.is_contiguous(), "wait_for_words: an int32 host tensor");
  const volatile int32_t* w = words.data_ptr<int32_t>();
  const int64_t n = words.numel();
  auto all_there = [&]() {
    for (int64_t i = 0; i < n; ++i)
      if (w[i] == (int32_t)sentinel) return false;
    return true;
  };
  if (all_there()) return;
  {
    std::optional<py::gil_scoped_release> nogil;
    if (PyGILState_Check()) nogil.emplace();
    const auto t0 = std::chrono::steady_clock::now();
    for (unsigned spin = 0;; ++spin) {
      if (all_there()) return;
      if ((spin & 1023u) == 1023u && std::chrono::steady_clock::now() - t0 > std::chrono::microseconds(timeout_us)) break;
    }
    if (like.is_cuda()) {
      const DeviceScope dev(like);
      dev.synchronize(like);
    }
  }
  TORCH_CHECK(all_there(), "mi355gs: the step did not report its results");
}

Tensor f32c(const Tensor& t, const char* name, const Tensor& like) {
  TORCH_CHECK(t.is_cuda() || g_abi.allow_cpu, "instantsplat_amd operators run on the GPU only (got a CPU tensor; there is no CPU fallback)");
  TORCH_CHECK(t.scalar_type() == at::kFloat, "expected float32, got ", t.scalar_type(), " (", name, ")");
  TORCH_CHECK(t.device() == like.device(), "tensors on different devices: ", like.device(), " vs ", t.device(), " (", name, ")");
  return t.is_contiguous() ? t : t.contiguous();
}
float* fp(const Tensor& t) { return t.defined() && t.numel() ? t.data_ptr<float>() : nullptr; }

Tensor empty_bytes(size_t n, const Tensor& like) {
  return at::empty({(int64_t)(n > 0 ? n : 1)}, like.options().dtype(at::kByte));
}

struct HostClock {
  std::chrono::steady_clock::time_point t0 = std::chrono::steady_clock::now();
  double* acc;
  explicit HostClock(double* a) : acc(a) {}
  ~HostClock() { *acc += std::chrono::duration<double, std::micro>(std::chrono::steady_clock::now() - t0).count(); }
};
double g_host_us[6] = {0, 0, 0, 0, 0, 0};

struct GateRecord {
  Tensor scratch;
  const float* gate = nullptr;
  std::vector<c10::weak_intrusive_ptr<c10::StorageImpl>> storage;
  int64_t numel[7] = {0, 0, 0, 0, 0, 0, 0};
  int64_t version[7] = {0, 0, 0, 0, 0, 0, 0};
  bool valid = false;
};
std::mutex g_gate_mutex;
GateRecord g_gates;

template <class... T> bool any_requires_grad(const T&... t) {
  if (!at::GradMode::is_enabled()) return false;
  bool any = false;
  ((any = any || (t.defined() && t.requires_grad())), ...);
  return any;
}
thread_local bool t_backward_follows = false;
struct BackwardFollows {
  explicit BackwardFollows(bool v) { t_backward_follows = v; }
  ~BackwardFollows() { t_backward_follows = false; }
};

struct ZeroGrad { Tensor buf; uint32_t version = 0; };
std::mutex g_zero_mutex;
std::map<std::string, ZeroGrad> g_zero_pool;
bool g_share_zero_grad = true;
Tensor zero_grad_like(const Tensor& like) {
  if (!g_share_zero_grad) return at::zeros_like(like);
  std::ostringstream key;
  key << like.device() << ":" << like.sizes() << "@" << like.data_ptr();
  std::lock_guard<std::mutex> lock(g_zero_mutex);
  if (g_zero_pool.size() > 8 && !g_zero_pool.count(key.str())) g_zero_pool.clear();
  ZeroGrad& z = g_zero_pool[key.str()];
  if (!z.buf.defined()) {
    z.buf = at::zeros_like(like, like.options().requires_grad(false), at::MemoryFormat::Contiguous);
    z.version = z.buf._version();
  } else if (z.buf._version() != z.version) {
    z.buf.zero_();
    z.version = z.buf._version();
  }
  return z.buf.detach();
}

struct PoseRowSeen {
  c10::weak_intrusive_ptr<c10::TensorImpl> row{c10::intrusive_ptr<c10::TensorImpl>()};
  int64_t rows = 0, index = 0;
};
thread_local PoseRowSeen t_pose_row;
struct PoseTableWritten {
  c10::weak_intrusive_ptr<c10::StorageImpl> storage{c10::intrusive_ptr<c10::StorageImpl>()};
  int64_t rows = 0, index = 0;
  bool valid = false;
};
PoseTableWritten g_pose_table;

struct PoseRowFn : public torch::autograd::Function<PoseRowFn> {
  static Tensor forward(AutogradContext* ctx, Tensor table, int64_t index) {
    TORCH_CHECK(table.dim() == 2 && table.size(1) == 7, "pose_row: the pose table must be [views, 7]");
    const int64_t rows = table.size(0);
    if (index < 0) index += rows;
    TORCH_CHECK(index >= 0 && index < rows, "pose_row: index ", index, " is out of range for ", rows, " poses");
    ctx->saved_data["rows"] = rows;
    ctx->saved_data["index"] = index;
    Tensor row = table.select(0, index).detach();
    t_pose_row.row = c10::weak_intrusive_ptr<c10::TensorImpl>(row.getIntrusivePtr());
    t_pose_row.rows = table.is_contiguous() && table.scalar_type() == at::kFloat ? rows : 0;
    t_pose_row.index = index;
    return row;
  }
  static variable_list backward(AutogradContext* ctx, variable_list grad_out) {
    const int64_t rows = ctx->saved_data["rows"].toInt(), index = ctx->saved_data["index"].toInt();
    const Tensor& g = grad_out[0];
    if (!g.defined()) return {Tensor(), Tensor()};
    {
      std::lock_guard<std::mutex> lock(g_gate_mutex);
      auto strong = g_pose_table.storage.lock();
      const bool mine = g_pose_table.valid && strong && strong.get() == g.storage().unsafeGetStorageImpl() && g_pose_table.rows == rows &&
                        g_pose_table.index == index && g.scalar_type() == at::kFloat && g.dim() == 1 && g.numel() == 7 && g.is_contiguous() &&
                        g.storage_offset() == 7 * index;
      g_pose_table.valid = false;
      if (mine) {
        Tensor full = at::empty({0}, g.options());
        full.set_(g.storage(), 0, {rows, 7}, {7, 1});
        if (g_gates.valid && g_gates.storage.size() == 7) {
          g_gates.storage[6] = full.storage().getWeakStorageImpl();
          g_gates.numel[6] = full.numel();
          g_gates.version[6] = (int64_t)full._version();
        }
        return {full, Tensor()};
      }
    }
    Tensor full = at::zeros({rows, 7}, g.options());
    full.select(0, index).copy_(g);
    return {full, Tensor()};
  }
};

Tensor pose_row(Tensor table, int64_t index) { return PoseRowFn::apply(table, index); }

void check_frame_buffers(const Tensor& binning, const Tensor& scratch, int64_t R, int P, int W, int H) {
  const size_t need_b = g_abi.binning_bytes(R, W, H), need_s = g_abi.grad_scratch_bytes(P);
  TORCH_CHECK(!binning.defined() || (size_t)binning.numel() >= need_b || R <= 0,
              "mi355gs: this frame's binning buffer (", binning.numel(), " bytes) is smaller than the backward's layout needs (", need_b,
              "): the deterministic-backward mode was switched on between the frame's forward and its backward");
  TORCH_CHECK(!scratch.defined() || (size_t)scratch.numel() >= need_s,
              "mi355gs: this frame's gradient scratch (", scratch.numel(), " bytes) is smaller than the backward needs (", need_s,
              "): the deterministic-backward mode was switched on between the frame's forward and its backward");
}

struct FrameForward {
  Tensor radii, color, geom, tiles, binning;
  Tensor scratch;
  int64_t R = 0;
  int32_t* count;

  FrameForward(const Tensor& like, int P, const Tensor& count_slot) {
    TORCH_CHECK(count_slot.scalar_type() == at::kInt && count_slot.numel() == 1, "count_slot must be one int32");
    count = count_slot.data_ptr<int32_t>();
    radii = at::empty({P}, like.options().dtype(at::kInt));
  }

  template <class Project>
  void run(const DeviceScope& dev, const Tensor& like, int P, int W, int H, const Tensor& bg, int64_t capacity, int64_t count_hint,
           const Project& project) {
    color = at::empty({3, H, W}, like.options());
    geom = empty_bytes(g_abi.geom_bytes(P), like);
    tiles = empty_bytes(g_abi.tiles_bytes(W, H), like);
    if (t_backward_follows) scratch = empty_bytes(g_abi.grad_scratch_bytes(P), like);
    auto preprocess = [&]() {
      *reinterpret_cast<volatile int32_t*>(count) = -1;
      project(*this);
    };
    auto stage2 = [&](int64_t cap) {
      if (t_backward_follows) {
        binning = empty_bytes(g_abi.binning_bytes(cap, W, H), like);
        check(g_abi.forward_render(dev.stream, P, W, H, cap, fp(bg), geom.data_ptr(), tiles.data_ptr(), binning.data_ptr(), fp(color), 0),
              "raster_forward_render");
      } else {
        binning = empty_bytes(g_abi.binning_bytes_render_only(cap, W, H), like);
        check(g_abi.forward_render_only(dev.stream, P, W, H, cap, fp(bg), geom.data_ptr(), tiles.data_ptr(), binning.data_ptr(), fp(color), 0),
              "raster_forward_render_only");
      }
    };
    preprocess();
    R = capacity;
    if (R >= 0) {
      stage2(R);
      return;
    }
    const int64_t guess = count_hint > 0 ? count_hint + count_hint / 2 + 16384 : -1;
    if (guess > 0) stage2(guess);
    {
      HostClock wait_clock(&g_host_us[5]);
      wait_for_count(count, dev, like);
    }
    R = *reinterpret_cast<volatile int32_t*>(count);
    if (guess > 0 && R <= guess) {
      R = guess;
    } else {
      if (guess > 0) {
        preprocess();
        wait_for_count(count, dev, like);
      }
      stage2(R);
    }
  }
};

std::pair<Tensor, int> backward_scratch(AutogradContext* ctx, Tensor scratch, const Tensor& like, const Tensor& binning, int64_t R, int P,
                                        int W, int H) {
  const int is_clear = (scratch.defined() && ctx->saved_data["scratch_is_clear"].toBool()) ? 1 : 0;
  ctx->saved_data["scratch_is_clear"] = false;
  if (!scratch.defined()) scratch = empty_bytes(g_abi.grad_scratch_bytes(P), like);
  check_frame_buffers(binning, scratch, R, P, W, H);
  return {scratch, is_clear};
}

struct RenderPosedFn : public torch::autograd::Function<RenderPosedFn> {
  static variable_list forward(AutogradContext* ctx, Tensor xyz_, Tensor rot_, Tensor scaling_, Tensor opl_, Tensor f_dc_,
                               Tensor f_rest_, Tensor pose_, Tensor means2D, Tensor bg_, Tensor view_, Tensor proj_, Tensor origin_,
                               int64_t H, int64_t W, double tanfovx, double tanfovy, double scale_modifier, int64_t D,
                               int64_t capacity, int64_t count_hint, Tensor count_slot) {
    TORCH_CHECK(g_abi.bound, "mi355gs torch binding: bind() has not been called");
    HostClock clock(&g_host_us[0]);
    (void)means2D;
    const Tensor xyz = f32c(xyz_, "xyz", xyz_), rot = f32c(rot_, "rotation", xyz), scaling = f32c(scaling_, "scaling", xyz),
                 opl = f32c(opl_, "opacity", xyz), f_dc = f32c(f_dc_, "features_dc", xyz), f_rest = f32c(f_rest_, "features_rest", xyz),
                 pose = f32c(pose_, "camera_pose", xyz), bg = f32c(bg_, "bg", xyz), view = f32c(view_, "viewmatrix", xyz),
                 proj = f32c(proj_, "projmatrix", xyz), origin = f32c(origin_, "campos", xyz);
    TORCH_CHECK(xyz.dim() == 2 && xyz.size(1) == 3, "means3D must have dimensions (num_points, 3)");
    const int P = (int)xyz.size(0);
    const DeviceScope dev(xyz);
    FrameForward f(xyz, P, count_slot);
    Tensor visible = at::empty({P}, xyz.options().dtype(at::kBool));
    f.run(dev, xyz, P, (int)W, (int)H, bg, capacity, count_hint, [&](const FrameForward& frame) {
      check(g_abi.posed_forward_preprocess(dev.stream, P, (int)D, (int)W, (int)H, fp(xyz), fp(f_dc), fp(f_rest), fp(opl), fp(scaling),
                                           (float)scale_modifier, fp(rot), fp(pose), fp(view), fp(proj), fp(origin), (float)tanfovx,
                                           (float)tanfovy, frame.radii.data_ptr<int32_t>(), frame.geom.data_ptr(), frame.tiles.data_ptr(), frame.count,
                                           P > 0 ? reinterpret_cast<uint8_t*>(visible.data_ptr<bool>()) : nullptr,
                                           frame.scratch.defined() ? frame.scratch.data_ptr() : nullptr, 0),
            "posed_forward_preprocess");
    });
    ctx->saved_data["dims"] = std::vector<int64_t>{P, D, W, H, f.R};
    ctx->saved_data["scalars"] = std::vector<double>{tanfovx, tanfovy, scale_modifier};
    ctx->saved_data["scratch_is_clear"] = f.scratch.defined();
    {
      auto seen = t_pose_row.row.lock();
      const bool is_row = seen && seen.get() == pose_.unsafeGetTensorImpl() && t_pose_row.rows > 0;
      ctx->saved_data["pose_table"] = std::vector<int64_t>{is_row ? t_pose_row.rows : 0, is_row ? t_pose_row.index : 0};
    }
    ctx->save_for_backward({xyz, rot, scaling, opl, f_dc, f_rest, pose, f.radii, f.geom, f.tiles, f.binning, bg, view, proj, origin, f.color,
                            f.scratch});
    ctx->mark_non_differentiable({f.radii, visible});
    ctx->set_materialize_grads(false);
    return {f.color, f.radii, visible};
  }

  static variable_list backward(AutogradContext* ctx, variable_list grad_out) {
    HostClock clock(&g_host_us[1]);
    const auto saved = ctx->get_saved_variables();
    const Tensor &xyz = saved[0], &rot = saved[1], &scaling = saved[2], &opl = saved[3], &f_dc = saved[4], &f_rest = saved[5],
                 &pose = saved[6], &radii = saved[7], &geom = saved[8], &tiles = saved[9], &binning = saved[10], &bg = saved[11],
                 &view = saved[12], &proj = saved[13], &origin = saved[14], &color = saved[15];
    const auto dims = ctx->saved_data["dims"].toIntVector();
    const auto sc = ctx->saved_data["scalars"].toDoubleVector();
    const int P = (int)dims[0], D = (int)dims[1], W = (int)dims[2], H = (int)dims[3];
    const int64_t R = dims[4];
    if (!grad_out[0].defined()) return variable_list(21);
    const Tensor g = f32c(grad_out[0], "grad_color", xyz);
    const DeviceScope dev(xyz);
    Tensor d_xyz = at::empty_like(xyz), d_rot = at::empty_like(rot), d_scaling = at::empty_like(scaling), d_opl = at::empty_like(opl),
           d_fdc = at::empty_like(f_dc), d_m2d = at::empty_like(xyz);
    Tensor d_frest = D == 0 ? zero_grad_like(f_rest) : at::empty_like(f_rest);
    const auto pose_table = ctx->saved_data["pose_table"].toIntVector();
    const int64_t pose_rows = pose_table[0], pose_index = pose_table[1];
    Tensor d_pose_store = at::empty({pose_rows > 0 ? pose_rows * 7 : 7}, xyz.options());
    Tensor d_pose = d_pose_store;
    if (pose_rows > 0) {
      d_pose = at::empty({0}, xyz.options());
      d_pose.set_(d_pose_store.storage(), 7 * pose_index, {7}, {1});
    }
    const auto [scratch, scratch_is_clear] = backward_scratch(ctx, saved[16], xyz, binning, R, P, W, H);
    Tensor pose_scratch = at::empty({16 * (((int64_t)P + 255) / 256) + 32}, xyz.options());
    check(g_abi.posed_backward(dev.stream, P, D, W, H, fp(bg), fp(xyz), fp(f_dc), fp(f_rest), fp(opl), fp(scaling), (float)sc[2], fp(rot),
                               fp(pose), fp(view), fp(proj), fp(origin), (float)sc[0], (float)sc[1], geom.data_ptr(), tiles.data_ptr(),
                               binning.data_ptr(), R, radii.data_ptr<int32_t>(), fp(color), fp(g), scratch.data_ptr(), fp(pose_scratch),
                               fp(d_xyz), fp(d_m2d), fp(d_fdc), D ? fp(d_frest) : nullptr, fp(d_opl), fp(d_scaling), fp(d_rot),
                               fp(d_pose_store), (int)pose_rows, (int)pose_index, scratch_is_clear, 0),
          "posed_backward");
    {
      std::lock_guard<std::mutex> lock(g_gate_mutex);
      g_pose_table.valid = pose_rows > 0;
      if (pose_rows > 0) {
        g_pose_table.storage = d_pose_store.storage().getWeakStorageImpl();
        g_pose_table.rows = pose_rows; g_pose_table.index = pose_index;
      }
      const Tensor* outs[7] = {&d_xyz, &d_fdc, &d_frest, &d_opl, &d_scaling, &d_rot, &d_pose};
      g_gates.storage.clear();
      for (int k = 0; k < 7; ++k) {
        g_gates.storage.push_back(outs[k]->storage().getWeakStorageImpl());
        g_gates.numel[k] = outs[k]->numel();
        g_gates.version[k] = (int64_t)outs[k]->_version();
      }
      g_gates.scratch = scratch;
      g_gates.gate = reinterpret_cast<const float*>(static_cast<const char*>(scratch.data_ptr()) + g_abi.grad_gate_offset(P));
      g_gates.valid = true;
    }
    Tensor none;
    return {d_xyz, d_rot, d_scaling, d_opl, d_fdc, d_frest, d_pose, d_m2d, none, none, none, none,
            none, none, none, none, none, none, none, none, none};
  }
};

std::vector<Tensor> render_posed(Tensor xyz, Tensor rot, Tensor scaling, Tensor opl, Tensor f_dc, Tensor f_rest, Tensor pose,
                                 Tensor means2D, Tensor bg, Tensor view, Tensor proj, Tensor origin, int64_t H, int64_t W,
                                 double tanfovx, double tanfovy, double scale_modifier, int64_t D, int64_t capacity, int64_t count_hint,
                                 Tensor count_slot) {
  const BackwardFollows scope(any_requires_grad(xyz, rot, scaling, opl, f_dc, f_rest, pose, means2D));
  return RenderPosedFn::apply(xyz, rot, scaling, opl, f_dc, f_rest, pose, means2D, bg, view, proj, origin, H, W, tanfovx, tanfovy,
                              scale_modifier, D, capacity, count_hint, count_slot);
}

struct RasterizeFn : public torch::autograd::Function<RasterizeFn> {
  using OptTensor = c10::optional<Tensor>;
  static variable_list forward(AutogradContext* ctx, Tensor means3D_, Tensor means2D, OptTensor sh_, OptTensor colors_, Tensor opac_,
                               OptTensor scales_, OptTensor rot_, OptTensor cov_, OptTensor sh_rest_, Tensor bg_, Tensor view_, Tensor proj_,
                               Tensor campos_,
                               int64_t H, int64_t W, double tanfovx, double tanfovy, double scale_modifier, int64_t D, bool prefiltered,
                               int64_t capacity, int64_t count_hint, Tensor count_slot) {
    TORCH_CHECK(g_abi.bound, "mi355gs torch binding: bind() has not been called");
    HostClock clock(&g_host_us[0]);
    (void)means2D;
    auto opt = [&](const OptTensor& t, const char* name, const Tensor& like) {
      return (t.has_value() && t->defined() && t->numel()) ? f32c(*t, name, like) : Tensor();
    };
    const Tensor means3D = f32c(means3D_, "means3D", means3D_), opac = f32c(opac_, "opacities", means3D);
    const Tensor sh = opt(sh_, "sh", means3D), colors = opt(colors_, "colors_precomp", means3D), scales = opt(scales_, "scales", means3D),
                 rot = opt(rot_, "rotations", means3D), cov = opt(cov_, "cov3Ds_precomp", means3D), sh_rest = opt(sh_rest_, "sh_rest", means3D);
    const Tensor bg = f32c(bg_, "bg", means3D), view = f32c(view_, "viewmatrix", means3D), proj = f32c(proj_, "projmatrix", means3D),
                 campos = f32c(campos_, "campos", means3D);
    TORCH_CHECK(means3D.dim() == 2 && means3D.size(1) == 3, "means3D must have dimensions (num_points, 3)");
    const int P = (int)means3D.size(0);
    const int M = sh.defined() ? (int)(sh.size(1) + (sh_rest.defined() ? sh_rest.size(1) : 0)) : 0;
    const DeviceScope dev(means3D);
    FrameForward f(means3D, P, count_slot);
    f.run(dev, means3D, P, (int)W, (int)H, bg, capacity, count_hint, [&](const FrameForward& frame) {
      check(g_abi.forward_preprocess(dev.stream, P, (int)D, M, (int)W, (int)H, fp(means3D), fp(sh), fp(sh_rest), fp(colors), fp(opac), fp(scales),
                                     (float)scale_modifier, fp(rot), fp(cov), fp(view), fp(proj), fp(campos), (float)tanfovx, (float)tanfovy,
                                     prefiltered ? 1 : 0, frame.radii.data_ptr<int32_t>(), frame.geom.data_ptr(), frame.tiles.data_ptr(), frame.count, nullptr,
                                     frame.scratch.defined() ? frame.scratch.data_ptr() : nullptr, 0),
            "raster_forward_preprocess");
    });
    ctx->saved_data["dims"] = std::vector<int64_t>{P, D, M, W, H, f.R};
    ctx->saved_data["scalars"] = std::vector<double>{tanfovx, tanfovy, scale_modifier};
    ctx->saved_data["opacity_shape"] = opac_.sizes().vec();
    ctx->saved_data["scratch_is_clear"] = f.scratch.defined();
    ctx->save_for_backward({means3D, sh, colors, opac, scales, rot, cov, sh_rest, f.radii, f.geom, f.tiles, f.binning, bg, view, proj, campos,
                            f.color, f.scratch});
    ctx->mark_non_differentiable({f.radii});
    ctx->set_materialize_grads(false);
    return {f.color, f.radii};
  }

  static variable_list backward(AutogradContext* ctx, variable_list grad_out) {
    if (!grad_out[0].defined()) return variable_list(23);
    const auto saved = ctx->get_saved_variables();
    const Tensor &means3D = saved[0], &sh = saved[1], &colors = saved[2], &opac = saved[3], &scales = saved[4], &rot = saved[5], &cov = saved[6],
                 &sh_rest = saved[7], &radii = saved[8], &geom = saved[9], &tiles = saved[10], &binning = saved[11], &bg = saved[12],
                 &view = saved[13], &proj = saved[14], &campos = saved[15], &color = saved[16];
    const auto dims = ctx->saved_data["dims"].toIntVector();
    const auto sc = ctx->saved_data["scalars"].toDoubleVector();
    const int P = (int)dims[0], D = (int)dims[1], M = (int)dims[2], W = (int)dims[3], H = (int)dims[4];
    const int64_t R = dims[5];
    const Tensor g = f32c(grad_out[0], "grad_color", means3D);
    const DeviceScope dev(means3D);
    const auto o = means3D.options();
    Tensor d_means3D = at::empty({P, 3}, o), d_means2D = at::empty({P, 3}, o), d_opac = at::empty({P}, o), d_col = at::empty({P, 3}, o);
    Tensor d_sh, d_shr, d_scales, d_rot, d_cov;
    if (sh.defined()) d_sh = at::empty({P, sh_rest.defined() ? 1 : M, 3}, o);
    if (sh_rest.defined()) d_shr = at::empty({P, M - 1, 3}, o);
    if (cov.defined()) d_cov = at::empty({P, 6}, o); else { d_scales = at::empty({P, 3}, o); d_rot = at::empty({P, 4}, o); }
    const auto [scratch, scratch_is_clear] = backward_scratch(ctx, saved[17], means3D, binning, R, P, W, H);
    check(g_abi.raster_backward(dev.stream, P, D, M, W, H, fp(bg), fp(means3D), fp(sh), fp(sh_rest), fp(colors), fp(opac), fp(scales), (float)sc[2],
                                fp(rot), fp(cov), fp(view), fp(proj), fp(campos), (float)sc[0], (float)sc[1], geom.data_ptr(), tiles.data_ptr(),
                                binning.data_ptr(), R, radii.data_ptr<int32_t>(), fp(color), fp(g), scratch.data_ptr(), fp(d_means3D), fp(d_means2D),
                                fp(d_sh), fp(d_shr), fp(d_col), fp(d_opac), fp(d_scales), fp(d_rot), fp(d_cov), scratch_is_clear, 0),
          "raster_backward");
    Tensor none;
    const auto shape = ctx->saved_data["opacity_shape"].toIntVector();
    return {d_means3D, d_means2D, d_sh, sh.defined() ? none : d_col, d_opac.reshape(shape), d_scales, d_rot, d_cov, d_shr,
            none, none, none, none, none, none, none, none, none, none, none, none, none, none};
  }
};

std::vector<Tensor> rasterize(Tensor means3D, Tensor means2D, c10::optional<Tensor> sh, c10::optional<Tensor> colors, Tensor opac,
                              c10::optional<Tensor> scales, c10::optional<Tensor> rot, c10::optional<Tensor> cov, c10::optional<Tensor> sh_rest,
                              Tensor bg, Tensor view, Tensor proj, Tensor campos, int64_t H, int64_t W, double tanfovx, double tanfovy,
                              double scale_modifier, int64_t D, bool prefiltered, int64_t capacity, int64_t count_hint, Tensor count_slot) {
  const Tensor none;
  auto val = [&](const c10::optional<Tensor>& t) -> const Tensor& { return t.has_value() ? *t : none; };
  const BackwardFollows scope(any_requires_grad(means3D, means2D, opac, val(sh), val(colors), val(scales), val(rot), val(cov), val(sh_rest)));
  return RasterizeFn::apply(means3D, means2D, sh, colors, opac, scales, rot, cov, sh_rest, bg, view, proj, campos, H, W,
                            tanfovx, tanfovy, scale_modifier, D, prefiltered, capacity, count_hint, count_slot);
}

struct L1SsimLossFn : public torch::autograd::Function<L1SsimLossFn> {
  static variable_list forward(AutogradContext* ctx, Tensor img1, Tensor img2, double lambda_dssim) {
    TORCH_CHECK(g_abi.bound, "mi355gs torch binding: bind() has not been called");
    HostClock clock(&g_host_us[2]);
    const Tensor a = f32c(img1, "img1", img1), b = f32c(img2, "img2", a);
    TORCH_CHECK(a.dim() == 4 && a.sizes() == b.sizes(), "fused_ssim expects two [B,C,H,W] tensors of equal shape");
    const int B = (int)a.size(0), C = (int)a.size(1), H = (int)a.size(2), W = (int)a.size(3);
    const DeviceScope dev(a);
    Tensor scratch = empty_bytes(g_abi.ssim_scratch_bytes(B, C, H, W), a);
    Tensor out = at::empty({2}, a.options());
    Tensor loss = at::empty({}, a.options());
    Tensor grad = at::empty_like(a);
    check(g_abi.l1_ssim_loss_fused(dev.stream, B, C, H, W, fp(a), fp(b), scratch.data_ptr(), (float)lambda_dssim, fp(out), fp(out) + 1,
                                   fp(loss), fp(grad)),
          "l1_ssim_loss_fused");
    ctx->save_for_backward({grad});
    ctx->mark_non_differentiable({out});
    ctx->set_materialize_grads(false);
    return {loss, out};
  }
  static variable_list backward(AutogradContext* ctx, variable_list grad_out) {
    HostClock clock(&g_host_us[3]);
    Tensor none;
    if (!grad_out[0].defined()) return {none, none, none};
    const auto saved = ctx->get_saved_variables();
    return {saved[0] * grad_out[0], none, none};
  }
};

std::vector<Tensor> l1_ssim_loss(Tensor img1, Tensor img2, double lambda_dssim) { return L1SsimLossFn::apply(img1, img2, lambda_dssim); }

struct L1LossFn : public torch::autograd::Function<L1LossFn> {
  static Tensor forward(AutogradContext* ctx, Tensor a_, Tensor b_) {
    TORCH_CHECK(g_abi.bound, "mi355gs torch binding: bind() has not been called");
    const Tensor a = f32c(a_, "network_output", a_), b = f32c(b_, "gt", a);
    TORCH_CHECK(a.sizes() == b.sizes() && a.numel() > 0, "l1_loss expects two non-empty tensors of equal shape");
    const DeviceScope dev(a);
    Tensor scratch = empty_bytes(g_abi.l1_scratch_bytes(a.numel()), a);
    Tensor out = at::empty({}, a.options());
    check(g_abi.l1_loss_forward(dev.stream, a.numel(), fp(a), fp(b), scratch.data_ptr(), fp(out)), "l1_loss_forward");
    ctx->save_for_backward({a, b});
    return out;
  }
  static variable_list backward(AutogradContext* ctx, variable_list grad_out) {
    const auto saved = ctx->get_saved_variables();
    const Tensor &a = saved[0], &b = saved[1];
    const Tensor g = f32c(grad_out[0], "grad", a);
    const DeviceScope dev(a);
    Tensor d = at::empty_like(a);
    check(g_abi.l1_loss_backward(dev.stream, a.numel(), fp(a), fp(b), fp(g), fp(d)), "l1_loss_backward");
    return {d, Tensor()};
  }
};

Tensor l1_loss(Tensor a, Tensor b) { return L1LossFn::apply(a, b); }

std::vector<Tensor> loss_pair_forward(Tensor img1, Tensor img2) {
  TORCH_CHECK(g_abi.bound, "mi355gs torch binding: bind() has not been called");
  HostClock clock(&g_host_us[2]);
  const Tensor a = f32c(img1, "img1", img1), b = f32c(img2, "img2", a);
  TORCH_CHECK((a.dim() == 3 || a.dim() == 4) && a.sizes() == b.sizes() && a.numel() > 0, "the loss pair expects two [C,H,W] or [B,C,H,W] tensors of equal shape");
  const int64_t o = a.dim() == 4 ? 1 : 0;
  const int B = o ? (int)a.size(0) : 1, C = (int)a.size(o), H = (int)a.size(o + 1), W = (int)a.size(o + 2);
  const DeviceScope dev(a);
  Tensor scratch = empty_bytes(g_abi.ssim_scratch_bytes(B, C, H, W), a);
  Tensor means = at::empty({2}, a.options());
  Tensor dmap = at::empty_like(a);
  check(g_abi.pair_forward(dev.stream, B, C, H, W, fp(a), fp(b), scratch.data_ptr(), fp(dmap)), "l1_ssim_pair_forward");
  return {means, scratch, dmap, a, b};
}

struct LossAffineFn : public torch::autograd::Function<LossAffineFn> {
  static Tensor forward(AutogradContext* ctx, Tensor image, Tensor a, Tensor b, Tensor dmap, Tensor means, Tensor scratch,
                        std::vector<int64_t> ops, std::vector<double> consts, double c_l1, double c_ssim, Tensor host_slot, double ticket,
                        c10::optional<Tensor> unit_grad_) {
    const Tensor unit_grad = unit_grad_.has_value() ? *unit_grad_ : Tensor();
    TORCH_CHECK(g_abi.bound, "mi355gs torch binding: bind() has not been called");
    TORCH_CHECK(ops.size() == consts.size() && !ops.empty() && ops.size() <= MI355GS_LOSS_PROGRAM_MAX, "loss_affine: 1..16 operations");
    TORCH_CHECK(image.numel() == a.numel() && means.numel() == 2, "loss_affine: image and its contiguous copy differ in size");
    const int64_t o = a.dim() == 4 ? 1 : 0;
    const int B = o ? (int)a.size(0) : 1, C = (int)a.size(o), H = (int)a.size(o + 1), W = (int)a.size(o + 2);
    const DeviceScope dev(a);
    int32_t op32[MI355GS_LOSS_PROGRAM_MAX]; float k32[MI355GS_LOSS_PROGRAM_MAX];
    for (size_t i = 0; i < ops.size(); ++i) { op32[i] = (int32_t)ops[i]; k32[i] = (float)consts[i]; }
    Tensor out = at::empty({}, a.options());
    float* host_out = nullptr;
    if (host_slot.defined() && host_slot.numel() >= 2) {
      TORCH_CHECK(host_slot.scalar_type() == at::kFloat && !host_slot.is_cuda() && host_slot.is_contiguous(), "loss_affine: the host slot is float32[2] host memory");
      host_out = host_slot.data_ptr<float>();
    }
    Tensor d;
    const bool with_grad = unit_grad.defined() && unit_grad.numel() == 1;
    if (with_grad) {
      d = at::empty_like(a);
      check(g_abi.program_eval_grad(dev.stream, (int)ops.size(), op32, k32, B, C, H, W, scratch.data_ptr(), fp(means) + 1, fp(means), fp(out), host_out,
                                    (float)ticket, fp(a), fp(b), fp(dmap), (float)c_l1, (float)c_ssim, fp(d)),
            "loss_program_eval_grad");
    } else {
      check(g_abi.program_eval(dev.stream, (int)ops.size(), op32, k32, B, C, H, W, scratch.data_ptr(), fp(means) + 1, fp(means), fp(out), host_out,
                               (float)ticket),
            "loss_program_eval");
    }
    ctx->save_for_backward({a, b, dmap, with_grad ? d : Tensor()});
    ctx->saved_data["c"] = std::vector<double>{c_l1, c_ssim};
    ctx->saved_data["shape"] = image.sizes().vec();
    ctx->saved_data["unit_grad_ptr"] = with_grad ? (int64_t)(uintptr_t)unit_grad.data_ptr() : (int64_t)0;
    return out;
  }
  static variable_list backward(AutogradContext* ctx, variable_list grad_out) {
    HostClock clock(&g_host_us[3]);
    const auto saved = ctx->get_saved_variables();
    const Tensor &a = saved[0], &b = saved[1], &dmap = saved[2];
    const auto c = ctx->saved_data["c"].toDoubleVector();
    Tensor none;
    const int64_t unit_ptr = ctx->saved_data["unit_grad_ptr"].toInt();
    if (unit_ptr != 0 && saved.size() > 3 && saved[3].defined() && (int64_t)(uintptr_t)grad_out[0].data_ptr() == unit_ptr) {
      return {saved[3].view(ctx->saved_data["shape"].toIntVector()), none, none, none, none, none, none, none, none, none, none, none, none};
    }
    const Tensor g = f32c(grad_out[0].reshape({1}), "grad", a);
    const DeviceScope dev(a);
    Tensor d = at::empty_like(a);
    check(g_abi.pair_backward(dev.stream, a.numel(), fp(a), fp(b), fp(dmap), fp(g), (float)c[0], fp(g), (float)c[1], fp(d)), "l1_ssim_pair_backward");
    return {d.view(ctx->saved_data["shape"].toIntVector()), none, none, none, none, none, none, none, none, none, none, none, none};
  }
};

Tensor loss_affine(Tensor image, Tensor a, Tensor b, Tensor dmap, Tensor means, Tensor scratch, std::vector<int64_t> ops,
                   std::vector<double> consts, double c_l1, double c_ssim, Tensor host_slot, double ticket) {
  return LossAffineFn::apply(image, a, b, dmap, means, scratch, ops, consts, c_l1, c_ssim, host_slot, ticket, c10::optional<Tensor>());
}

py::object wait_for_loss(Tensor host_slot, double ticket, int64_t timeout_us) {
  TORCH_CHECK(host_slot.scalar_type() == at::kFloat && !host_slot.is_cuda() && host_slot.numel() >= 2, "wait_for_loss: float32[2] host memory");
  const volatile float* w = host_slot.data_ptr<float>();
  const float want = (float)ticket;
  auto taken_over = [want](float have) {
    if (have == 0.f || have == want) return false;
    float ahead = have - want;
    if (ahead < 0.f) ahead += 16000000.f;
    return ahead < 8000000.f;
  };
  bool there = w[1] == want;
  if (!there && !taken_over(w[1])) {
    py::gil_scoped_release nogil;
    const auto t0 = std::chrono::steady_clock::now();
    for (unsigned spin = 0;; ++spin) {
      const float have = w[1];
      if (have == want) { there = true; break; }
      if (taken_over(have)) break;
      if ((spin & 1023u) == 1023u && std::chrono::steady_clock::now() - t0 > std::chrono::microseconds(timeout_us)) break;
    }
  }
  if (!there) return py::none();
  const float v = w[0];
  if (w[1] != want) return py::none();
  return py::float_((double)v);
}

Tensor loss_affine_backward(Tensor image, Tensor a, Tensor b, Tensor dmap, Tensor means, Tensor scratch, std::vector<int64_t> ops,
                            std::vector<double> consts, double c_l1, double c_ssim, Tensor host_slot, double ticket) {
  static std::mutex mu;
  static std::map<std::string, std::pair<Tensor, uint32_t>> ones;
  Tensor one;
  {
    std::lock_guard<std::mutex> lock(mu);
    std::ostringstream key;
    key << a.device();
    auto& slot = ones[key.str()];
    if (!slot.first.defined() || slot.first._version() != slot.second) {
      slot.first = at::ones({}, a.options().requires_grad(false));
      slot.second = slot.first._version();
    }
    one = slot.first;
  }
  const bool will_run = at::GradMode::is_enabled() && image.requires_grad();
  Tensor out = LossAffineFn::apply(image, a, b, dmap, means, scratch, ops, consts, c_l1, c_ssim, host_slot, ticket, will_run ? c10::optional<Tensor>(one) : c10::optional<Tensor>());
  if (!out.requires_grad()) return out;
  py::gil_scoped_release nogil;
  torch::autograd::backward({out}, {one}, false, false);
  return out;
}

struct SsimFn : public torch::autograd::Function<SsimFn> {
  static Tensor forward(AutogradContext* ctx, Tensor img1, Tensor img2, bool train, bool valid) {
    TORCH_CHECK(g_abi.bound, "mi355gs torch binding: bind() has not been called");
    const Tensor a = f32c(img1, "img1", img1), b = f32c(img2, "img2", a);
    TORCH_CHECK(a.dim() == 4 && a.sizes() == b.sizes(), "fused_ssim expects two [B,C,H,W] tensors of equal shape");
    const int B = (int)a.size(0), C = (int)a.size(1), H = (int)a.size(2), W = (int)a.size(3);
    TORCH_CHECK(!valid || (H > 10 && W > 10), "fused_ssim(padding=\"valid\") needs images larger than the 11x11 window");
    const DeviceScope dev(a);
    Tensor dm1, dm2, dm3;
    if (train) { dm1 = at::empty_like(a); dm2 = at::empty_like(a); dm3 = at::empty_like(a); }
    Tensor scratch = empty_bytes(g_abi.ssim_scratch_bytes(B, C, H, W), a);
    Tensor out = at::empty({2}, a.options());
    check(g_abi.ssim_forward(dev.stream, B, C, H, W, fp(a), fp(b), fp(dm1), fp(dm2), fp(dm3), scratch.data_ptr(), fp(out),
                             valid ? nullptr : fp(out) + 1, valid ? 1 : 0),
          "ssim_forward");
    if (train) ctx->save_for_backward({a, b, dm1, dm2, dm3});
    ctx->saved_data["flags"] = std::vector<int64_t>{train ? 1 : 0, valid ? 1 : 0};
    return out.select(0, 0).clone();
  }
  static variable_list backward(AutogradContext* ctx, variable_list grad_out) {
    const auto flags = ctx->saved_data["flags"].toIntVector();
    TORCH_CHECK(flags[0] == 1, "fused_ssim was called with train=False; no gradient is available");
    const auto saved = ctx->get_saved_variables();
    const Tensor &a = saved[0], &b = saved[1];
    const int B = (int)a.size(0), C = (int)a.size(1), H = (int)a.size(2), W = (int)a.size(3);
    const DeviceScope dev(a);
    const Tensor scale = f32c(grad_out[0].reshape({1}), "grad", a);
    Tensor grad = at::empty_like(a);
    check(g_abi.ssim_backward(dev.stream, B, C, H, W, fp(a), fp(b), fp(saved[2]), fp(saved[3]), fp(saved[4]), fp(scale), nullptr, fp(grad),
                              (int)flags[1]),
          "ssim_backward");
    Tensor none;
    return {grad, none, none, none};
  }
};

Tensor fused_ssim(Tensor img1, Tensor img2, bool train, bool valid) { return SsimFn::apply(img1, img2, train, valid); }

struct AdamPlan {
  std::vector<Tensor> params, exp_avg, exp_avg_sq, pplr;
  std::vector<int64_t> numel;
  std::vector<int32_t> row;
  double beta1, beta2, eps;
  int64_t last_used_gates = 0;
  std::string last_gate_note;
  Tensor live;
  uint32_t seq = 0;
  std::vector<int64_t> moment_version;
  std::vector<Tensor> owners;

  AdamPlan(std::vector<Tensor> p, std::vector<Tensor> m, std::vector<Tensor> v, std::vector<c10::optional<Tensor>> pp, double b1, double b2,
           double e)
      : params(std::move(p)), exp_avg(std::move(m)), exp_avg_sq(std::move(v)), beta1(b1), beta2(b2), eps(e) {
    const size_t n = params.size();
    TORCH_CHECK(n >= 1 && n <= 8 && exp_avg.size() == n && exp_avg_sq.size() == n && pp.size() == n, "AdamPlan: 1..8 tensors, equal-length lists");
    for (size_t t = 0; t < n; ++t) {
      const Tensor& q = params[t];
      TORCH_CHECK(q.is_cuda() || g_abi.allow_cpu, "instantsplat_amd operators run on the GPU only (got a CPU tensor; there is no CPU fallback)");
      TORCH_CHECK(q.scalar_type() == at::kFloat && q.is_contiguous(), "AdamPlan: parameters must be contiguous float32");
      for (const Tensor* s : {&exp_avg[t], &exp_avg_sq[t]})
        TORCH_CHECK(s->scalar_type() == at::kFloat && s->is_contiguous() && s->device() == q.device() && s->numel() == q.numel(),
                    "AdamPlan: moments must match their parameter");
      numel.push_back(q.numel());
      if (pp[t].has_value() && pp[t]->defined()) {
        const Tensor& l = *pp[t];
        TORCH_CHECK(l.scalar_type() == at::kFloat && l.is_contiguous() && l.device() == q.device() && q.dim() >= 1 && q.size(0) > 0 &&
                        l.numel() == q.size(0),
                    "AdamPlan: per_point_lr must hold one contiguous float32 per point");
        pplr.push_back(l);
        row.push_back((int32_t)(q.numel() / q.size(0)));
      } else {
        pplr.emplace_back();
        row.push_back(1);
      }
    }
  }

  void set_owners(std::vector<Tensor> o) {
    TORCH_CHECK(o.size() == params.size(), "AdamPlan.set_owners: one Parameter per tensor");
    owners = std::move(o);
  }
  bool step_owned(const std::vector<double>& lr, const std::vector<int64_t>& step_counts) {
    const size_t n = params.size();
    if (owners.size() != n) return false;
    std::vector<Tensor> grads(n);
    for (size_t t = 0; t < n; ++t) {
      const Tensor& g = owners[t].grad();
      if (!g.defined() || g.is_sparse() || owners[t].data_ptr() != params[t].data_ptr() || g.numel() != numel[t]) return false;
      grads[t] = g;
    }
    this->step(grads, lr, step_counts);
    return true;
  }
  void zero_owned() {
    for (Tensor& o : owners) o.mutable_grad().reset();
  }

  void step(const std::vector<Tensor>& grads, const std::vector<double>& lr, const std::vector<int64_t>& step) {
    const size_t n = params.size();
    TORCH_CHECK(grads.size() == n && lr.size() == n && step.size() == n, "AdamPlan.step: list lengths");
    HostClock clock(&g_host_us[4]);
    const DeviceScope dev(params[0]);
    int64_t nm[8]; int32_t rw[8], st[8], gidx[8];
    float* pp[8]; const float* gg[8]; float* mm[8]; float* vv[8]; const float* ll[8]; float lrs[8];
    std::vector<Tensor> keep;
    int64_t n_flagged = 0;
    GateRecord rec;
    {
      std::lock_guard<std::mutex> lock(g_gate_mutex);
      rec = g_gates;
    }
    for (size_t t = 0; t < n; ++t) {
      Tensor g = grads[t];
      TORCH_CHECK(g.defined() && g.numel() == numel[t] && g.device() == params[t].device(), "AdamPlan.step: gradient ", t, " does not match its parameter");
      bool mine = false;
      if (rec.valid && g.scalar_type() == at::kFloat && g.is_contiguous() && g.storage_offset() == 0) {
        const c10::StorageImpl* impl = g.storage().unsafeGetStorageImpl();
        for (int k = 0; k < (int)rec.storage.size() && !mine; ++k) {
          auto strong = rec.storage[k].lock();
          if (strong && strong.get() == impl && rec.numel[k] == g.numel() && rec.version[k] == (int64_t)g._version()) { gidx[t] = k; mine = true; }
        }
      }
      if (!mine) {
        std::ostringstream why;
        why << "tensor " << t << ": record " << (rec.valid ? "valid" : "absent") << ", offset " << g.storage_offset() << ", version " << g._version()
            << ", storage " << (const void*)g.storage().unsafeGetStorageImpl() << ", numel " << g.numel();
        last_gate_note = why.str();
      }
      if (!mine) gidx[t] = -1;
      n_flagged += mine ? 1 : 0;
      if (g.scalar_type() != at::kFloat || !g.is_contiguous()) { g = g.to(at::kFloat).contiguous(); keep.push_back(g); }
      nm[t] = numel[t]; rw[t] = row[t]; st[t] = (int32_t)step[t]; lrs[t] = (float)lr[t];
      pp[t] = params[t].data_ptr<float>(); gg[t] = g.data_ptr<float>(); mm[t] = exp_avg[t].data_ptr<float>();
      vv[t] = exp_avg_sq[t].data_ptr<float>(); ll[t] = pplr[t].defined() ? pplr[t].data_ptr<float>() : nullptr;
    }
    const bool gated = n_flagged > 0;
    Tensor scratch;
    if (n_flagged < (int64_t)n) scratch = at::empty({8}, params[0].options());
    last_used_gates = n_flagged;
    bool moments_touched = !live.defined();
    if (moment_version.size() != 2 * n) moment_version.assign(2 * n, -1);
    for (size_t t = 0; t < n; ++t) {
      const int64_t v0 = (int64_t)exp_avg[t]._version(), v1 = (int64_t)exp_avg_sq[t]._version();
      moments_touched = moments_touched || v0 != moment_version[2 * t] || v1 != moment_version[2 * t + 1];
      moment_version[2 * t] = v0; moment_version[2 * t + 1] = v1;
    }
    if (!live.defined()) live = at::zeros({16}, params[0].options().dtype(at::kInt));
    else if (moments_touched) live.zero_();
    if (++seq == 0u) seq = 1u;
    check(g_abi.adam_multi_step(dev.stream, (int)n, nm, rw, pp, gg, mm, vv, ll, lrs, (float)beta1, (float)beta2, (float)eps, st,
                                scratch.defined() ? scratch.data_ptr<float>() : nullptr, gated ? rec.gate : nullptr, gated ? gidx : nullptr,
                                reinterpret_cast<uint32_t*>(live.data_ptr<int32_t>()), seq),
          "adam_multi_step");
  }
};

}

PYBIND11_MODULE(TORCH_EXTENSION_NAME, m) {
  m.doc() = "compiled PyTorch binding of libmi355gs.so's drop-in operators (no compute of its own)";
  m.def("abi_symbols", &abi_symbols, "the C symbols bind() must be given, in the order of the list they are generated from");
  m.def("bind", &bind_abi, "hand over the C-ABI entry points (name -> address) of the loaded libmi355gs build; allow_cpu_tensors: test tier only");
  m.def("l1_loss", &l1_loss, "utils/loss_utils.py::l1_loss as one node (the library's l1_loss forward / backward pair)");
  m.def("render_posed", &render_posed);
  m.def("wait_for_words", &wait_for_words, "spin (GIL released) until no element of an int32 pinned host tensor holds the sentinel; stream wait after timeout_us");
  m.def("pose_row", &pose_row, "GaussianModel.get_RT: row `index` of the [views, 7] pose table as a node the render node's backward cooperates with");
  m.def("rasterize", &rasterize);
  m.def("l1_ssim_loss", &l1_ssim_loss);
  m.def("loss_pair_forward", &loss_pair_forward, "-> [means (l1, ssim: filled by the first loss_affine), partial sums, d(ssim_mean)/dimg1, img1, img2 (contiguous)]: one launch, no autograd node");
  m.def("wait_for_loss", &wait_for_loss, "the value the program kernel stored to a pinned host slot under this ticket, or None (timeout / slot taken over)");
  m.def("loss_affine_backward", &loss_affine_backward, "loss_affine + the engine run of loss.backward() in one call (root gradient: a cached 1)");
  m.def("loss_affine", &loss_affine, "the recorded scalar expression over (l1_mean, ssim_mean) as ONE node on `image`");
  m.def("fused_ssim", &fused_ssim);
  m.def("host_times_us", [](bool reset) {
    std::vector<double> v(g_host_us, g_host_us + 6);
    if (reset) for (double& x : g_host_us) x = 0;
    return v;
  }, "accumulated host microseconds: render fwd (incl. the count wait), render bwd, loss fwd, loss bwd, adam step, count wait");
  m.def("forget_gates", []() { std::lock_guard<std::mutex> lock(g_gate_mutex); g_gates = GateRecord(); });
  m.def("shared_zero_grad", [](bool on) {
    std::lock_guard<std::mutex> lock(g_zero_mutex);
    const bool old = g_share_zero_grad;
    g_share_zero_grad = on;
    if (!on) g_zero_pool.clear();
    return old;
  }, "f_rest's all-zero gradient below its SH degree: true (default) = aliases of one persistent zero buffer, false = a fresh zeros tensor per backward");
  py::class_<AdamPlan>(m, "AdamPlan")
      .def(py::init<std::vector<Tensor>, std::vector<Tensor>, std::vector<Tensor>, std::vector<c10::optional<Tensor>>, double, double, double>())
      .def("step", &AdamPlan::step)
      .def("set_owners", &AdamPlan::set_owners)
      .def("step_owned", &AdamPlan::step_owned)
      .def("zero_owned", &AdamPlan::zero_owned)
      .def_readonly("last_used_gates", &AdamPlan::last_used_gates)
      .def_readonly("last_gate_note", &AdamPlan::last_gate_note);
}
```

### instantsplat_amd/fused_ssim/__init__.py

```python
from __future__ import annotations

import torch

from .. import _lib
from .. import lazy_loss


def _run_forward(img1, img2, train, valid=False):
    L = _lib.lib()
    a, b = _lib.f32c(img1), _lib.f32c(img2)
    if a.dim() != 4 or a.shape != b.shape:
        raise RuntimeError("fused_ssim expects two [B,C,H,W] tensors of equal shape")
    dev = _lib.require_device(a, b)
    B, C, H, W = a.shape
    new = lambda: torch.empty_like(a)
    dm1, dm2, dm3 = (new(), new(), new()) if train else (None, None, None)
    scratch = torch.empty(int(L.mi355gs_ssim_scratch_bytes(B, C, H, W)), dtype=torch.uint8, device=dev)
    if valid and (H <= 10 or W <= 10):
        raise RuntimeError('fused_ssim(padding="valid") needs images larger than the 11x11 window')
    out = torch.empty(2, dtype=torch.float32, device=dev)
    with _lib.on_device(dev):
        _lib.check(L.mi355gs_ssim_forward(_lib.stream_ptr(dev), B, C, H, W, _lib.ptr(a), _lib.ptr(b), _lib.ptr(dm1), _lib.ptr(dm2),
                                          _lib.ptr(dm3), _lib.ptr(scratch), _lib.ptr(out[0:1]), None if valid else _lib.ptr(out[1:2]),
                                          1 if valid else 0), "ssim_forward")
    return a, b, dm1, dm2, dm3, out


def _run_backward(a, b, dm1, dm2, dm3, ssim_scale, l1_scale, valid=False):
    L = _lib.lib()
    dev = a.device
    B, C, H, W = a.shape
    grad = torch.empty_like(a)
    with _lib.on_device(dev):
        _lib.check(L.mi355gs_ssim_backward(_lib.stream_ptr(dev), B, C, H, W, _lib.ptr(a), _lib.ptr(b), _lib.ptr(dm1), _lib.ptr(dm2),
                                           _lib.ptr(dm3), _lib.ptr(ssim_scale), _lib.ptr(l1_scale), _lib.ptr(grad), 1 if valid else 0),
                   "ssim_backward")
    return grad


class _FusedSSIM(torch.autograd.Function):
    @staticmethod
    def forward(ctx, img1, img2, train, valid=False):
        a, b, dm1, dm2, dm3, out = _run_forward(img1, img2, train, valid)
        if train:
            ctx.save_for_backward(a, b, dm1, dm2, dm3)
        ctx.train, ctx.valid = train, valid
        return out[0].clone()

    @staticmethod
    def backward(ctx, g):
        if not ctx.train:
            raise RuntimeError("fused_ssim was called with train=False; no gradient is available")
        a, b, dm1, dm2, dm3 = ctx.saved_tensors
        scale = _lib.f32c(g.reshape(1))
        return _run_backward(a, b, dm1, dm2, dm3, scale, None, ctx.valid), None, None, None


def fused_ssim(img1, img2, padding="same", train=True):
    if padding not in ("same", "valid"):
        raise ValueError(f'padding must be "same" or "valid", got {padding!r}')
    if train and padding == "same" and lazy_loss._LAST[0] is not None and isinstance(img1, torch.Tensor) and isinstance(img2, torch.Tensor):
        half = lazy_loss.ssim_of_pair(img1, img2)
        if half is not None:
            return half
    ext = _lib.compiled()
    if ext is not None:
        return ext.fused_ssim(img1, img2, bool(train), padding == "valid")
    return _FusedSSIM.apply(img1, img2, train, padding == "valid")


_SCRATCH_BYTES = {}


def _scratch_bytes(L, B, C, H, W):
    key = (B, C, H, W)
    n = _SCRATCH_BYTES.get(key)
    if n is None:
        if len(_SCRATCH_BYTES) > 64:
            _SCRATCH_BYTES.clear()
        n = _SCRATCH_BYTES[key] = int(L.mi355gs_ssim_scratch_bytes(B, C, H, W))
    return n


class _FusedL1SSIM(torch.autograd.Function):

    @staticmethod
    def forward(ctx, img1, img2, lambda_dssim):
        L = _lib.lib()
        (a, b), dev = _lib.f32c_on_one_device(img1, img2)
        if a.dim() != 4 or a.shape != b.shape:
            raise RuntimeError("fused_ssim expects two [B,C,H,W] tensors of equal shape")
        B, C, H, W = a.shape
        scratch = torch.empty(_scratch_bytes(L, B, C, H, W), dtype=torch.uint8, device=dev)
        out = torch.empty(2, dtype=torch.float32, device=dev)
        loss = torch.empty((), dtype=torch.float32, device=dev)
        grad = torch.empty_like(a)
        p0 = out.data_ptr()
        with _lib.on_device(dev):
            _lib.check(L.mi355gs_l1_ssim_loss_fused(_lib.stream_ptr(dev), B, C, H, W, _lib.ptr(a), _lib.ptr(b), _lib.ptr(scratch),
                                                    float(lambda_dssim), p0, p0 + 4, _lib.ptr(loss), _lib.ptr(grad)),
                       "l1_ssim_loss_fused")
        ctx.save_for_backward(grad)
        ctx.mark_non_differentiable(out)
        return loss, out

    @staticmethod
    def backward(ctx, g, _):
        (grad,) = ctx.saved_tensors
        return grad * g, None, None


def fused_l1_ssim_loss(img1, img2, lambda_dssim=0.2):
    ext = _lib.compiled()
    if ext is not None:
        return ext.l1_ssim_loss(img1, img2, float(lambda_dssim))
    return _FusedL1SSIM.apply(img1, img2, lambda_dssim)
```

### instantsplat_amd/lazy_loss.py

```python
from __future__ import annotations

import os
import time
import warnings

import numpy as np
import torch

from . import _lib

ENABLED = os.environ.get("MI355GS_LAZY_LOSS", "1") != "0"

OP_L1, OP_SSIM, OP_MULK, OP_ADDK, OP_RSUBK, OP_DIVK, OP_NEG, OP_ADD, OP_SUB = range(9)
PROGRAM_MAX = 16

_PLACEHOLDER = {}


def _placeholder(dev):
    t = _PLACEHOLDER.get(dev)
    if t is None:
        t = _PLACEHOLDER[dev] = torch.full((), float("nan"), dtype=torch.float32, device=dev)
    return t


def _tensor_key(t):
    return (t.data_ptr(), t._version, t.numel(), tuple(t.shape[-3:]))


class Pair:
    __slots__ = ("image", "gt", "image_key", "gt_key", "a", "b", "dmap", "means", "scratch", "dev")

    def __init__(self, image, gt):
        ext = _lib.compiled()
        if ext is not None:
            self.means, self.scratch, self.dmap, self.a, self.b = ext.loss_pair_forward(image, gt)
        else:
            self.means, self.scratch, self.dmap, self.a, self.b = _pair_forward_ctypes(image, gt)
        self.image, self.gt = image, gt
        self.image_key, self.gt_key = _tensor_key(image), _tensor_key(gt)
        self.dev = self.a.device

    @property
    def l1(self):
        return self.means[0]

    @property
    def ssim(self):
        return self.means[1]

    def matches(self, img1, img2):
        return (_tensor_key(img1) == self.image_key and _tensor_key(img2) == self.gt_key and img1.is_contiguous() and img2.is_contiguous()
                and img1.dtype is torch.float32 and img2.dtype is torch.float32 and not img2.requires_grad)


_LAST = [None]


def eligible(network_output, gt):
    return (ENABLED and torch.is_grad_enabled() and network_output.requires_grad and not gt.requires_grad
            and network_output.dim() in (3, 4) and network_output.dtype is torch.float32 and gt.dtype is torch.float32
            and network_output.shape == gt.shape and network_output.numel() > 0 and network_output.device == gt.device
            and (network_output.is_cuda or _lib._TEST_MODE) and network_output.is_contiguous() and gt.is_contiguous()
            and network_output.shape[-3] * (network_output.shape[0] if network_output.dim() == 4 else 1) <= 65535)


def l1_of_pair(network_output, gt):
    rec = _LAST[0] = Pair(network_output, gt)
    return _new(rec, ((OP_L1, 0.0),))


def ssim_of_pair(img1, img2):
    rec = _LAST[0]
    if rec is None or not ENABLED or not torch.is_grad_enabled() or not rec.matches(img1, img2):
        return None
    return _new(rec, ((OP_SSIM, 0.0),))


def forget():
    _LAST[0] = None


def _new(rec, prog):
    t = torch.Tensor._make_subclass(LazyScalar, _placeholder(rec.dev), False)
    t._rec, t._prog, t._real, t._slot = rec, prog, None, None
    return t


def _is_number(k):
    return isinstance(k, (int, float)) and not isinstance(k, bool)


def _is_lazy(x):
    return type(x) is LazyScalar


EARLY_ITEM = os.environ.get("MI355GS_EARLY_ITEM", "1") != "0"
_NO_SLOT = torch.empty(0)
_SLOTS = {}
_N_SLOTS = 64
_TICKET = [0]


def _host_slot(dev):
    ring = _SLOTS.get(dev)
    if ring is None:
        words = torch.zeros(_N_SLOTS, 2, dtype=torch.float32, pin_memory=(dev.type == "cuda"))
        ring = _SLOTS[dev] = [words, [words[i] for i in range(_N_SLOTS)], 0]
    k = ring[2]
    ring[2] = (k + 1) % _N_SLOTS
    t = _TICKET[0] = _TICKET[0] % 16000000 + 1
    return ring[1][k], float(t)


_PARTIALS = {}


def partials(prog):
    c = _PARTIALS.get(prog)
    if c is not None:
        return c
    f = np.float32
    st = []
    for op, k in prog:
        k = f(k)
        if op == OP_L1:
            st.append((f(1), f(0)))
        elif op == OP_SSIM:
            st.append((f(0), f(1)))
        elif op == OP_MULK:
            a = st[-1]
            st[-1] = (a[0] * k, a[1] * k)
        elif op == OP_DIVK:
            a, r = st[-1], f(1) / k
            st[-1] = (a[0] * r, a[1] * r)
        elif op in (OP_RSUBK, OP_NEG):
            a = st[-1]
            st[-1] = (-a[0], -a[1])
        elif op == OP_ADD:
            b, a = st.pop(), st.pop()
            st.append((a[0] + b[0], a[1] + b[1]))
        elif op == OP_SUB:
            b, a = st.pop(), st.pop()
            st.append((a[0] - b[0], a[1] - b[1]))
        elif op != OP_ADDK:
            raise ValueError(f"unknown loss-program operation {op}")
    assert len(st) == 1, prog
    if len(_PARTIALS) > 256:
        _PARTIALS.clear()
    c = _PARTIALS[prog] = (float(st[0][0]), float(st[0][1]))
    return c


def materialize(x):
    rec = x._rec
    need_grad = torch.is_grad_enabled() and rec.image.requires_grad
    real = x._real
    if real is not None and (real.requires_grad or not need_grad):
        return real
    c_l1, c_ssim = partials(x._prog)
    ops, consts = [p[0] for p in x._prog], [float(p[1]) for p in x._prog]
    ext = _lib.compiled()
    if ext is not None:
        slot, ticket = _host_slot(rec.dev) if EARLY_ITEM else (None, 0.0)
        real = ext.loss_affine(rec.image, rec.a, rec.b, rec.dmap, rec.means, rec.scratch, ops, consts, c_l1, c_ssim, _NO_SLOT if slot is None else slot, ticket)
        x._slot = (slot, ticket) if slot is not None else None
    else:
        real = _LossAffine.apply(rec.image, rec, ops, consts, c_l1, c_ssim)
        x._slot = None
    x._real = real
    return real


def _unary(x, op, k=0.0):
    if len(x._prog) >= PROGRAM_MAX:
        return NotImplemented
    return _new(x._rec, x._prog + ((op, float(k)),))


def _binary(a, b, op):
    if a._rec is not b._rec or len(a._prog) + len(b._prog) >= PROGRAM_MAX:
        return NotImplemented
    return _new(a._rec, a._prog + b._prog + ((op, 0.0),))


def _h_mul(a, b):
    if _is_lazy(a) and _is_number(b):
        return _unary(a, OP_MULK, b)
    if _is_lazy(b) and _is_number(a):
        return _unary(b, OP_MULK, a)
    return NotImplemented


def _h_add(a, b, alpha=1):
    if alpha != 1:
        return NotImplemented
    if _is_lazy(a) and _is_lazy(b):
        return _binary(a, b, OP_ADD)
    if _is_lazy(a) and _is_number(b):
        return _unary(a, OP_ADDK, b)
    if _is_lazy(b) and _is_number(a):
        return _unary(b, OP_ADDK, a)
    return NotImplemented


def _h_sub(a, b, alpha=1):
    if alpha != 1:
        return NotImplemented
    if _is_lazy(a) and _is_lazy(b):
        return _binary(a, b, OP_SUB)
    if _is_lazy(a) and _is_number(b):
        return _unary(a, OP_ADDK, -b)
    if _is_lazy(b) and _is_number(a):
        return _unary(b, OP_RSUBK, a)
    return NotImplemented


def _h_rsub(a, b, alpha=1):
    return _h_sub(b, a, alpha)


def _h_div(a, b, rounding_mode=None):
    if rounding_mode is None and _is_lazy(a) and _is_number(b) and b != 0:
        return _unary(a, OP_DIVK, b)
    return NotImplemented


def _h_neg(a):
    return _unary(a, OP_NEG) if _is_lazy(a) else NotImplemented


_T = torch.Tensor
_HANDLERS = {}
for _fns, _h in (((_T.__mul__, _T.__rmul__, _T.mul, torch.mul, _T.multiply, torch.multiply), _h_mul),
                 ((_T.__add__, _T.__radd__, _T.add, torch.add), _h_add),
                 ((_T.__sub__, _T.sub, torch.sub, _T.subtract, torch.subtract), _h_sub),
                 ((_T.__rsub__, torch.rsub), _h_rsub),
                 ((_T.__truediv__, _T.div, torch.div, _T.true_divide, torch.true_divide, _T.divide, torch.divide), _h_div),
                 ((_T.__neg__, _T.neg, torch.neg, _T.negative, torch.negative), _h_neg)):
    for _f in _fns:
        _HANDLERS[_f] = _h


def _real_args(x):
    if _is_lazy(x):
        return materialize(x)
    if isinstance(x, (list, tuple)):
        return type(x)(_real_args(v) for v in x)
    if isinstance(x, dict):
        return {k: _real_args(v) for k, v in x.items()}
    return x


class LazyScalar(torch.Tensor):

    def __mul__(self, k):
        return _unary(self, OP_MULK, k) if _is_number(k) and len(self._prog) < PROGRAM_MAX else _T.__mul__(self, k)

    __rmul__ = __mul__

    def __add__(self, k):
        if type(k) is LazyScalar:
            out = _binary(self, k, OP_ADD)
            return out if out is not NotImplemented else _T.__add__(self, k)
        return _unary(self, OP_ADDK, k) if _is_number(k) and len(self._prog) < PROGRAM_MAX else _T.__add__(self, k)

    __radd__ = __add__

    def __sub__(self, k):
        if type(k) is LazyScalar:
            out = _binary(self, k, OP_SUB)
            return out if out is not NotImplemented else _T.__sub__(self, k)
        return _unary(self, OP_ADDK, -k) if _is_number(k) and len(self._prog) < PROGRAM_MAX else _T.__sub__(self, k)

    def __rsub__(self, k):
        return _unary(self, OP_RSUBK, k) if _is_number(k) and len(self._prog) < PROGRAM_MAX else _T.__rsub__(self, k)

    def __truediv__(self, k):
        return _unary(self, OP_DIVK, k) if _is_number(k) and k != 0 and len(self._prog) < PROGRAM_MAX else _T.__truediv__(self, k)

    def __neg__(self):
        return _unary(self, OP_NEG) if len(self._prog) < PROGRAM_MAX else _T.__neg__(self)

    def backward(self, gradient=None, retain_graph=None, create_graph=False, inputs=None):
        if gradient is None and not retain_graph and not create_graph and inputs is None and torch.is_grad_enabled():
            real = self._real
            if real is None or not real.requires_grad:
                ext = _lib.compiled()
                rec = self._rec
                if ext is not None and rec.image.requires_grad:
                    c_l1, c_ssim = partials(self._prog)
                    prog = self._prog
                    slot, ticket = _host_slot(rec.dev) if EARLY_ITEM else (None, 0.0)
                    self._real = ext.loss_affine_backward(rec.image, rec.a, rec.b, rec.dmap, rec.means, rec.scratch, [p[0] for p in prog],
                                                          [p[1] for p in prog], c_l1, c_ssim, _NO_SLOT if slot is None else slot, ticket)
                    self._slot = (slot, ticket) if slot is not None else None
                    return None
        return materialize(self).backward(gradient, retain_graph, create_graph, inputs)

    def item(self):
        real = materialize(self)
        slot = self._slot
        if slot is not None:
            ext = _lib.compiled()
            if ext is not None:
                t0 = time.perf_counter()
                v = ext.wait_for_loss(slot[0], slot[1], 200_000)
                if v is not None:
                    return v
                if time.perf_counter() - t0 > 0.1:
                    global EARLY_ITEM
                    EARLY_ITEM = False
                    warnings.warn("instantsplat_amd.lazy_loss: the pinned loss slot did not receive the value within 200 ms; "
                                  "loss.item() falls back to an ordinary read for the rest of the process (MI355GS_EARLY_ITEM=0)")
        return real.item()

    def __float__(self):
        return float(materialize(self).detach())

    def detach(self):
        return materialize(self).detach()

    @classmethod
    def __torch_function__(cls, func, types, args=(), kwargs=None):
        kwargs = kwargs or {}
        h = _HANDLERS.get(func)
        if h is not None:
            try:
                out = h(*args, **kwargs)
            except TypeError:
                out = NotImplemented
            if out is not NotImplemented:
                return out
        args, kwargs = _real_args(args), _real_args(kwargs)
        with torch._C.DisableTorchFunctionSubclass():
            return func(*args, **kwargs)


def _pair_forward_ctypes(img1, img2):
    L = _lib.lib()
    (a, b), dev = _lib.f32c_on_one_device(img1, img2)
    if a.dim() not in (3, 4) or a.shape != b.shape or a.numel() == 0:
        raise RuntimeError("the loss pair expects two [C,H,W] or [B,C,H,W] tensors of equal shape")
    B = a.shape[0] if a.dim() == 4 else 1
    C, H, W = a.shape[-3:]
    scratch = torch.empty(int(L.mi355gs_ssim_scratch_bytes(B, C, H, W)), dtype=torch.uint8, device=dev)
    means = torch.empty(2, dtype=torch.float32, device=dev)
    dmap = torch.empty_like(a)
    with _lib.on_device(dev):
        _lib.check(L.mi355gs_l1_ssim_pair_forward(_lib.stream_ptr(dev), B, C, H, W, _lib.ptr(a), _lib.ptr(b), _lib.ptr(scratch),
                                                  _lib.ptr(dmap)), "l1_ssim_pair_forward")
    return means, scratch, dmap, a, b


class _LossAffine(torch.autograd.Function):
    @staticmethod
    def forward(ctx, image, rec, ops, consts, c_l1, c_ssim):
        import ctypes
        L = _lib.lib()
        dev = rec.dev
        out = torch.empty((), dtype=torch.float32, device=dev)
        n = len(ops)
        a = rec.a
        B = a.shape[0] if a.dim() == 4 else 1
        C, H, W = a.shape[-3:]
        with _lib.on_device(dev):
            _lib.check(L.mi355gs_loss_program_eval(_lib.stream_ptr(dev), n, (ctypes.c_int32 * n)(*ops), (ctypes.c_float * n)(*consts), B, C, H, W,
                                                   _lib.ptr(rec.scratch), rec.means.data_ptr() + 4, rec.means.data_ptr(), _lib.ptr(out), None, 0.0),
                       "loss_program_eval")
        ctx.save_for_backward(rec.a, rec.b, rec.dmap)
        ctx.c, ctx.shape = (c_l1, c_ssim), image.shape
        return out

    @staticmethod
    def backward(ctx, g):
        a, b, dmap = ctx.saved_tensors
        L = _lib.lib()
        g = _lib.f32c(g.reshape(1))
        d = torch.empty_like(a)
        with _lib.on_device(a.device):
            _lib.check(L.mi355gs_l1_ssim_pair_backward(_lib.stream_ptr(a.device), a.numel(), _lib.ptr(a), _lib.ptr(b), _lib.ptr(dmap),
                                                       _lib.ptr(g), ctx.c[0], _lib.ptr(g), ctx.c[1], _lib.ptr(d)), "l1_ssim_pair_backward")
        return d.view(ctx.shape), None, None, None, None, None
```

Before: 3554.

## Cache ground-truth SSIM window moments across iterations and skip recomputing them

Adds a kernel that precomputes the Gaussian-windowed mean and second moment of each ground-truth image. These maps are kept in an LRU cache keyed by pointer, version, shape and device, and fed to a templated cached variant of the fused L1+SSIM kernel. That variant convolves only three moment channels instead of five, uses less LDS, and asks for higher occupancy through launch bounds. The cost is extra memory for the cached maps and a risk of stale entries if an image is changed in place without its version being bumped.

```diff
diff --git a/include/mi355gs.h b/include/mi355gs.h
--- a/include/mi355gs.h
+++ b/include/mi355gs.h
@@ -79,6 +79,10 @@
                           const float* ssim_grad_scale, const float* l1_grad_scale, float* dL_dimg1, int padding_valid);
 int mi355gs_l1_ssim_loss_fused(void* stream, int B, int C, int H, int W, const float* img1, const float* img2, void* scratch,
                                float lambda_dssim, float* ssim_mean, float* l1_mean, float* loss, float* dloss_dimg1);
+size_t mi355gs_ssim_gt_moments_bytes(int B, int C, int H, int W);
+int mi355gs_ssim_gt_moments(void* stream, int B, int C, int H, int W, const float* img2, void* maps);
+int mi355gs_l1_ssim_loss_fused_cached(void* stream, int B, int C, int H, int W, const float* img1, const float* img2, const void* gt_maps,
+                                      void* scratch, float lambda_dssim, float* ssim_mean, float* l1_mean, float* loss, float* dloss_dimg1);
 
 size_t mi355gs_l1_scratch_bytes(int64_t n);
 int mi355gs_l1_loss_forward(void* stream, int64_t n, const float* a, const float* b, void* scratch, float* mean_out);
@@ -95,6 +99,8 @@
 #define MI355GS_LOSS_OP_SUB 8
 int mi355gs_l1_ssim_pair_forward(void* stream, int B, int C, int H, int W, const float* img1, const float* img2, void* scratch,
                                  float* dssim_dimg1);
+int mi355gs_l1_ssim_pair_forward_cached(void* stream, int B, int C, int H, int W, const float* img1, const float* img2, const void* gt_maps,
+                                        void* scratch, float* dssim_dimg1);
 int mi355gs_l1_ssim_pair_backward(void* stream, int64_t n, const float* img1, const float* img2, const float* dssim_dimg1,
                                   const float* g_l1, float c_l1, const float* g_ssim, float c_ssim, float* d_img1);
 int mi355gs_loss_program_eval(void* stream, int n_ops, const int32_t* ops, const float* consts, int B, int C, int H, int W,
diff --git a/instantsplat_amd/_lib.py b/instantsplat_amd/_lib.py
--- a/instantsplat_amd/_lib.py
+++ b/instantsplat_amd/_lib.py
@@ -44,6 +44,10 @@
     "mi355gs_ssim_backward": (c_int, [_P, c_int, c_int, c_int, c_int, _P, _P, _P, _P, _P, _P, _P, _P, c_int]),
     "mi355gs_l1_ssim_loss_fused": (c_int, [_P, c_int, c_int, c_int, c_int, _P, _P, _P, c_float, _P, _P, _P, _P]),
     "mi355gs_l1_ssim_pair_forward": (c_int, [_P, c_int, c_int, c_int, c_int, _P, _P, _P, _P]),
+    "mi355gs_ssim_gt_moments_bytes": (c_size_t, [c_int, c_int, c_int, c_int]),
+    "mi355gs_ssim_gt_moments": (c_int, [_P, c_int, c_int, c_int, c_int, _P, _P]),
+    "mi355gs_l1_ssim_loss_fused_cached": (c_int, [_P, c_int, c_int, c_int, c_int, _P, _P, _P, _P, c_float, _P, _P, _P, _P]),
+    "mi355gs_l1_ssim_pair_forward_cached": (c_int, [_P, c_int, c_int, c_int, c_int, _P, _P, _P, _P, _P]),
     "mi355gs_l1_ssim_pair_backward": (c_int, [_P, c_int64, _P, _P, _P, _P, c_float, _P, c_float, _P]),
     "mi355gs_loss_program_eval": (c_int, [_P, c_int, _P, _P, c_int, c_int, c_int, c_int, _P, _P, _P, _P, _P, c_float]),
     "mi355gs_loss_program_eval_grad": (c_int, [_P, c_int, _P, _P, c_int, c_int, c_int, c_int, _P, _P, _P, _P, _P, c_float, _P, _P, _P, c_float,
@@ -170,7 +174,12 @@
         spec = importlib.util.spec_from_file_location("_mi355gs_torch", EXT_PATH)
         _EXT = importlib.util.module_from_spec(spec)
         spec.loader.exec_module(_EXT)
+        import atexit
+        from . import gt_cache
+        _EXT.gt_cache_cap(gt_cache._CAP[0])
+        atexit.register(_EXT.gt_cache_clear)
     _EXT.forget_gates()
+    _EXT.gt_cache_clear()
     _EXT.bind({name: ctypes.cast(getattr(L, name), ctypes.c_void_p).value for name in _EXT.abi_symbols()}, _TEST_MODE)
     _EXT_BOUND_TO = L
     return _EXT
diff --git a/instantsplat_amd/csrc/ssim.hip b/instantsplat_amd/csrc/ssim.hip
--- a/instantsplat_amd/csrc/ssim.hip
+++ b/instantsplat_amd/csrc/ssim.hip
@@ -268,13 +268,18 @@
   }
 }
 
-__global__ __launch_bounds__(FTHREADS) void k_l1_ssim_fused(int H, int W, const float* __restrict__ img1, const float* __restrict__ img2,
+constexpr int F_LDS_BUDGET = 53248;
+template <bool GT_CACHED>
+__global__ __launch_bounds__(FTHREADS, GT_CACHED ? 6 : 1) void k_l1_ssim_fused(int H, int W, const float* __restrict__ img1, const float* __restrict__ img2,
+                                                        const float* __restrict__ gt_my, const float* __restrict__ gt_myy,
                                                         float ks , float kl ,
                                                         float* __restrict__ dL_dimg1, float* __restrict__ partial ) {
+  constexpr int NM = GT_CACHED ? 3 : 5;
   __shared__ float s_xy[2][FR2][FXP];
-  __shared__ float s_h[5][FR2][FHP];
-  static_assert(3 * FR1 * FDP <= 2 * FR2 * FXP && 3 * FR1 * FEP <= 5 * FR2 * FHP, "aliased LDS buffers must fit");
+  __shared__ float s_h[NM][FR2][FHP];
+  static_assert(3 * FR1 * FDP <= 2 * FR2 * FXP && 3 * FR1 * FEP <= NM * FR2 * FHP, "aliased LDS buffers must fit");
   __shared__ float s_red[2][FTHREADS / 64];
+  static_assert(!GT_CACHED || sizeof(s_xy) + sizeof(s_h) + sizeof(s_red) <= F_LDS_BUDGET, "three workgroups per CU");
   float (*s_d)[FR1][FDP] = reinterpret_cast<float (*)[FR1][FDP]>(&s_xy[0][0][0]);
   float (*s_e)[FR1][FEP] = reinterpret_cast<float (*)[FR1][FEP]>(&s_h[0][0][0]);
   const int tid = threadIdx.x;
@@ -285,10 +290,12 @@
   const float* p2 = img2 + po;
   const int ec = tid & 31, er0 = (tid >> 5) * FER;
   float ex[FER], ey[FER];
-#pragma unroll
-  for (int j = 0; j < FER; ++j) {
-    const size_t o = (size_t)min(oy + er0 + j, H - 1) * W + min(ox + ec, W - 1);
-    ex[j] = p1[o]; ey[j] = p2[o];
+  if constexpr (!GT_CACHED) {
+#pragma unroll
+    for (int j = 0; j < FER; ++j) {
+      const size_t o = (size_t)min(oy + er0 + j, H - 1) * W + min(ox + ec, W - 1);
+      ex[j] = p1[o]; ey[j] = p2[o];
+    }
   }
   {
     float vx[F_STAGE_ITERS], vy[F_STAGE_ITERS];
@@ -327,15 +334,35 @@
         const int k = t - j;
         if (k >= 0 && k < 11) {
           const float w = gw(k);
-          sx[j] = fmaf(w, x[t], sx[j]); sy[j] = fmaf(w, y[t], sy[j]);
-          sxx[j] = fmaf(w, xx, sxx[j]); syy[j] = fmaf(w, yy, syy[j]); sxy[j] = fmaf(w, xy, sxy[j]);
+          if constexpr (GT_CACHED) {
+            sx[j] = fmaf(w, x[t], sx[j]); sxx[j] = fmaf(w, xx, sxx[j]); sxy[j] = fmaf(w, xy, sxy[j]);
+          } else {
+            sx[j] = fmaf(w, x[t], sx[j]); sy[j] = fmaf(w, y[t], sy[j]);
+            sxx[j] = fmaf(w, xx, sxx[j]); syy[j] = fmaf(w, yy, syy[j]); sxy[j] = fmaf(w, xy, sxy[j]);
+          }
         }
       }
     }
 #pragma unroll
     for (int j = 0; j < 6; ++j) {
-      s_h[0][r][c0 + j] = sx[j]; s_h[1][r][c0 + j] = sy[j]; s_h[2][r][c0 + j] = sxx[j]; s_h[3][r][c0 + j] = syy[j];
-      s_h[4][r][c0 + j] = sxy[j];
+      if constexpr (GT_CACHED) {
+        s_h[0][r][c0 + j] = sx[j]; s_h[1][r][c0 + j] = sxx[j]; s_h[2][r][c0 + j] = sxy[j];
+      } else {
+        s_h[0][r][c0 + j] = sx[j]; s_h[1][r][c0 + j] = sy[j]; s_h[2][r][c0 + j] = sxx[j]; s_h[3][r][c0 + j] = syy[j];
+        s_h[4][r][c0 + j] = sxy[j];
+      }
+    }
+  }
+  float gmy[FCR], gmyy[FCR];
+  if constexpr (GT_CACHED) {
+    if (tid < FR1 * FC_GROUPS) {
+      const int c = tid % FR1, r0 = (tid / FR1) * FCR;
+      const int cx = min(max(ox + c - HALO, 0), W - 1);
+#pragma unroll
+      for (int j = 0; j < FCR; ++j) {
+        const size_t o = po + (size_t)min(max(oy + r0 + j - HALO, 0), H - 1) * W + cx;
+        gmy[j] = gt_my[o]; gmyy[j] = gt_myy[o];
+      }
     }
   }
   __syncthreads();
@@ -344,11 +371,15 @@
     const int c = tid % FR1, r0 = (tid / FR1) * FCR;
     float mo[5][FCR];
 #pragma unroll
-    for (int m = 0; m < 5; ++m) {
+    for (int m = 0; m < NM; ++m) {
       float v[FCR + 10];
 #pragma unroll
       for (int t = 0; t < FCR + 10; ++t) v[t] = s_h[m][min(r0 + t, FR2 - 1)][c];
-      ssim_run(v, mo[m]);
+      ssim_run(v, mo[GT_CACHED ? 2 * m : m]);
+    }
+    if constexpr (GT_CACHED) {
+#pragma unroll
+      for (int j = 0; j < FCR; ++j) { mo[1][j] = gmy[j]; mo[3][j] = gmyy[j]; }
     }
     const int gx = ox + c - HALO;
 #pragma unroll
@@ -366,6 +397,13 @@
       if (FR1 % FCR == 0 || r0 + j < FR1) { s_d[0][r0 + j][c] = mo[0][j]; s_d[1][r0 + j][c] = mo[1][j]; s_d[2][r0 + j][c] = mo[2][j]; }
   }
   __syncthreads();
+  if constexpr (GT_CACHED) {
+#pragma unroll
+    for (int j = 0; j < FER; ++j) {
+      const size_t o = (size_t)min(oy + er0 + j, H - 1) * W + min(ox + ec, W - 1);
+      ex[j] = p1[o]; ey[j] = p2[o];
+    }
+  }
   if (tid < FR1 * FD_GROUPS) {
     const int r = tid % FR1, c0 = (tid / FR1) * FDR;
 #pragma unroll
@@ -418,6 +456,49 @@
     for (int w = 0; w < FTHREADS / 64; ++w) { ta += s_red[0][w]; tb += s_red[1][w]; }
     partial[2 * b] = ta;
     partial[2 * b + 1] = tb;
+  }
+}
+
+constexpr int GR = 4;
+__global__ __launch_bounds__(256) void k_ssim_gt_moments(int H, int W, const float* __restrict__ y, float* __restrict__ my,
+                                                         float* __restrict__ myy) {
+  __shared__ float s_y[FR1][FR1 + 1];
+  __shared__ float s_r[2][FR1][FT + 1];
+  const int tid = threadIdx.x;
+  const int ox = blockIdx.x * FT, oy = blockIdx.y * FT;
+  const size_t po = (size_t)blockIdx.z * H * W;
+  for (int i = tid; i < FR1 * FR1; i += 256) {
+    const int r = i / FR1, c = i - r * FR1;
+    const int gy = oy + r - HALO, gx = ox + c - HALO;
+    const bool in = gy >= 0 && gy < H && gx >= 0 && gx < W;
+    s_y[r][c] = in ? y[po + (size_t)gy * W + gx] : 0.f;
+  }
+  __syncthreads();
+  for (int i = tid; i < FR1 * FT; i += 256) {
+    const int r = i / FT, c = i - r * FT;
+    float a = 0.f, b = 0.f;
+#pragma unroll
+    for (int k = 0; k < 11; ++k) {
+      const float v = s_y[r][c + k], vv = v * v;
+      a = fmaf(gw(k), v, a); b = fmaf(gw(k), vv, b);
+    }
+    s_r[0][r][c] = a; s_r[1][r][c] = b;
+  }
+  __syncthreads();
+  const int c = tid & 31, r0 = (tid >> 5) * GR;
+  const int gx = ox + c;
+#pragma unroll
+  for (int m = 0; m < 2; ++m) {
+    float v[GR + 10], out[GR];
+#pragma unroll
+    for (int t = 0; t < GR + 10; ++t) v[t] = s_r[m][r0 + t][c];
+    ssim_run(v, out);
+    float* __restrict__ dst = m == 0 ? my : myy;
+#pragma unroll
+    for (int j = 0; j < GR; ++j) {
+      const int gy = oy + r0 + j;
+      if (gx < W && gy < H) dst[po + (size_t)gy * W + gx] = out[j];
+    }
   }
 }
 
@@ -688,22 +769,28 @@
 static inline bool planes_ok(int B, int C, int H, int W) { return B > 0 && C > 0 && H > 0 && W > 0 && (size_t)B * C <= 65535; }
 static inline dim3 plane_grid(int planes, int H, int W, int tw, int th) { return dim3((W + tw - 1) / tw, (H + th - 1) / th, planes); }
 
-static int launch_l1_ssim_fused(hipStream_t stream, int planes, int H, int W, const float* img1, const float* img2, float ks, float kl,
-                                float* dL_dimg1, void* scratch, const char* name) {
+static int launch_l1_ssim_fused(hipStream_t stream, int planes, int H, int W, const float* img1, const float* img2, const void* gt_maps,
+                                float ks, float kl, float* dL_dimg1, void* scratch, const char* name) {
   const int debug = 0;
+  const float* my = (const float*)gt_maps;
+  const float* myy = my ? my + (size_t)planes * H * W : nullptr;
   {
     GsProfScope prof(3, stream);
     GS_KRANGE(name);
-    hipLaunchKernelGGL(k_l1_ssim_fused, plane_grid(planes, H, W, FT, FT), dim3(FTHREADS), 0, stream, H, W, img1, img2, ks, kl, dL_dimg1,
-                       (float*)scratch);
+    if (my)
+      hipLaunchKernelGGL(k_l1_ssim_fused<true>, plane_grid(planes, H, W, FT, FT), dim3(FTHREADS), 0, stream, H, W, img1, img2, my, myy, ks, kl,
+                         dL_dimg1, (float*)scratch);
+    else
+      hipLaunchKernelGGL(k_l1_ssim_fused<false>, plane_grid(planes, H, W, FT, FT), dim3(FTHREADS), 0, stream, H, W, img1, img2, my, myy, ks, kl,
+                         dL_dimg1, (float*)scratch);
   }
   GS_CHECK_LAUNCH(name);
   return MI355GS_OK;
 }
-static int launch_l1_ssim_loss(hipStream_t stream, int planes, int H, int W, const float* img1, const float* img2, float lambda_dssim,
-                               float* dL_dimg1, void* scratch) {
+static int launch_l1_ssim_loss(hipStream_t stream, int planes, int H, int W, const float* img1, const float* img2, const void* gt_maps,
+                               float lambda_dssim, float* dL_dimg1, void* scratch) {
   const double inv_n = 1.0 / ((double)planes * H * W);
-  return launch_l1_ssim_fused(stream, planes, H, W, img1, img2, (float)(-(double)lambda_dssim * inv_n),
+  return launch_l1_ssim_fused(stream, planes, H, W, img1, img2, gt_maps, (float)(-(double)lambda_dssim * inv_n),
                               (float)((1.0 - (double)lambda_dssim) * inv_n), dL_dimg1, scratch, "l1_ssim_fused");
 }
 
@@ -781,13 +868,12 @@
   return MI355GS_OK;
 }
 
-int mi355gs_l1_ssim_loss_fused(void* stream_, int B, int C, int H, int W, const float* img1, const float* img2, void* scratch,
-                               float lambda_dssim, float* ssim_mean, float* l1_mean, float* loss, float* dloss_dimg1) {
-  GS_RANGE();
+static int l1_ssim_loss_fused(void* stream_, int B, int C, int H, int W, const float* img1, const float* img2, const void* gt_maps,
+                              void* scratch, float lambda_dssim, float* ssim_mean, float* l1_mean, float* loss, float* dloss_dimg1) {
   hipStream_t stream = (hipStream_t)stream_;
   const int debug = 0;
   if (!planes_ok(B, C, H, W) || !img1 || !img2 || !scratch || !loss || !dloss_dimg1) return MI355GS_EINVAL;
-  const int rc = launch_l1_ssim_loss(stream, B * C, H, W, img1, img2, lambda_dssim, dloss_dimg1, scratch);
+  const int rc = launch_l1_ssim_loss(stream, B * C, H, W, img1, img2, gt_maps, lambda_dssim, dloss_dimg1, scratch);
   if (rc != MI355GS_OK) return rc;
   const double inv_n = 1.0 / ((double)B * C * H * W);
   GS_KRANGE("ssim_finish");
@@ -796,13 +882,51 @@
   GS_CHECK_LAUNCH("ssim_finish");
   return MI355GS_OK;
 }
-
-int mi355gs_l1_ssim_pair_forward(void* stream_, int B, int C, int H, int W, const float* img1, const float* img2, void* scratch,
+int mi355gs_l1_ssim_loss_fused(void* stream, int B, int C, int H, int W, const float* img1, const float* img2, void* scratch,
+                               float lambda_dssim, float* ssim_mean, float* l1_mean, float* loss, float* dloss_dimg1) {
+  GS_RANGE();
+  return l1_ssim_loss_fused(stream, B, C, H, W, img1, img2, nullptr, scratch, lambda_dssim, ssim_mean, l1_mean, loss, dloss_dimg1);
+}
+int mi355gs_l1_ssim_loss_fused_cached(void* stream, int B, int C, int H, int W, const float* img1, const float* img2, const void* gt_maps,
+                                      void* scratch, float lambda_dssim, float* ssim_mean, float* l1_mean, float* loss, float* dloss_dimg1) {
+  GS_RANGE();
+  if (!gt_maps) return MI355GS_EINVAL;
+  return l1_ssim_loss_fused(stream, B, C, H, W, img1, img2, gt_maps, scratch, lambda_dssim, ssim_mean, l1_mean, loss, dloss_dimg1);
+}
+
+size_t mi355gs_ssim_gt_moments_bytes(int B, int C, int H, int W) {
+  if (B <= 0 || C <= 0 || H <= 0 || W <= 0) return 256;
+  return gs_align((size_t)2 * B * C * H * W * sizeof(float));
+}
+
+int mi355gs_ssim_gt_moments(void* stream_, int B, int C, int H, int W, const float* img2, void* maps) {
+  GS_RANGE();
+  hipStream_t stream = (hipStream_t)stream_;
+  const int debug = 0;
+  if (!planes_ok(B, C, H, W) || !img2 || !maps) return MI355GS_EINVAL;
+  float* my = (float*)maps;
+  GS_KRANGE("ssim_gt_moments");
+  hipLaunchKernelGGL(k_ssim_gt_moments, plane_grid(B * C, H, W, FT, FT), dim3(256), 0, stream, H, W, img2, my, my + (size_t)B * C * H * W);
+  GS_CHECK_LAUNCH("ssim_gt_moments");
+  return MI355GS_OK;
+}
+
+static int l1_ssim_pair_forward(void* stream_, int B, int C, int H, int W, const float* img1, const float* img2, const void* gt_maps,
+                                void* scratch, float* dssim_dimg1) {
+  if (!planes_ok(B, C, H, W) || !img1 || !img2 || !scratch || !dssim_dimg1) return MI355GS_EINVAL;
+  return launch_l1_ssim_fused((hipStream_t)stream_, B * C, H, W, img1, img2, gt_maps, (float)(1.0 / ((double)B * C * H * W)), 0.0f, dssim_dimg1,
+                              scratch, "l1_ssim_pair");
+}
+int mi355gs_l1_ssim_pair_forward(void* stream, int B, int C, int H, int W, const float* img1, const float* img2, void* scratch,
                                  float* dssim_dimg1) {
   GS_RANGE();
-  if (!planes_ok(B, C, H, W) || !img1 || !img2 || !scratch || !dssim_dimg1) return MI355GS_EINVAL;
-  return launch_l1_ssim_fused((hipStream_t)stream_, B * C, H, W, img1, img2, (float)(1.0 / ((double)B * C * H * W)), 0.0f, dssim_dimg1, scratch,
-                              "l1_ssim_pair");
+  return l1_ssim_pair_forward(stream, B, C, H, W, img1, img2, nullptr, scratch, dssim_dimg1);
+}
+int mi355gs_l1_ssim_pair_forward_cached(void* stream, int B, int C, int H, int W, const float* img1, const float* img2, const void* gt_maps,
+                                        void* scratch, float* dssim_dimg1) {
+  GS_RANGE();
+  if (!gt_maps) return MI355GS_EINVAL;
+  return l1_ssim_pair_forward(stream, B, C, H, W, img1, img2, gt_maps, scratch, dssim_dimg1);
 }
 
 int mi355gs_l1_ssim_pair_backward(void* stream_, int64_t n, const float* img1, const float* img2, const float* dssim_dimg1,
@@ -907,6 +1031,6 @@
 
 int gs_loss_fused(hipStream_t stream, int C, int H, int W, const float* img1, const float* img2, float lambda_dssim, float* dL_dimg1,
                   void* scratch) {
-  return launch_l1_ssim_loss(stream, C, H, W, img1, img2, lambda_dssim, dL_dimg1, scratch);
+  return launch_l1_ssim_loss(stream, C, H, W, img1, img2, nullptr, lambda_dssim, dL_dimg1, scratch);
 }
 int gs_loss_fused_nblocks(int C, int H, int W) { return fused_nblocks(1, C, H, W); }
diff --git a/instantsplat_amd/csrc_torch/binding.cpp b/instantsplat_amd/csrc_torch/binding.cpp
--- a/instantsplat_amd/csrc_torch/binding.cpp
+++ b/instantsplat_amd/csrc_torch/binding.cpp
@@ -3,6 +3,7 @@
 #include <c10/hip/HIPStream.h>
 
 #include <chrono>
+#include <cstdlib>
 #include <optional>
 #include <map>
 #include <mutex>
@@ -30,6 +31,10 @@
   X(posed_backward, mi355gs_posed_backward)                            \
   X(ssim_scratch_bytes, mi355gs_ssim_scratch_bytes)                    \
   X(l1_ssim_loss_fused, mi355gs_l1_ssim_loss_fused)                    \
+  X(gt_moments_bytes, mi355gs_ssim_gt_moments_bytes)                   \
+  X(gt_moments, mi355gs_ssim_gt_moments)                               \
+  X(l1_ssim_loss_fused_cached, mi355gs_l1_ssim_loss_fused_cached)      \
+  X(pair_forward_cached, mi355gs_l1_ssim_pair_forward_cached)          \
   X(l1_scratch_bytes, mi355gs_l1_scratch_bytes)                        \
   X(l1_loss_forward, mi355gs_l1_loss_forward)                          \
   X(l1_loss_backward, mi355gs_l1_loss_backward)                        \
@@ -512,6 +517,69 @@
                             tanfovx, tanfovy, scale_modifier, D, prefiltered, capacity, count_hint, count_slot);
 }
 
+struct GtEntry {
+  Tensor gt, maps;
+  uint32_t version = 0;
+  int64_t numel = 0, c = 0, h = 0, w = 0;
+  uint64_t used = 0;
+  size_t bytes = 0;
+};
+size_t gt_cache_default_cap() {
+  const char* e = std::getenv("MI355GS_GT_CACHE_MB");
+  if (!e || !*e) return (size_t)1 << 30;
+  const double mb = std::atof(e);
+  return mb > 0 ? (size_t)(mb * 1048576.0) : 0;
+}
+std::mutex g_gt_mutex;
+std::map<const void*, GtEntry> g_gt_cache;
+size_t g_gt_bytes = 0, g_gt_cap = gt_cache_default_cap();
+uint64_t g_gt_tick = 0, g_gt_hits = 0, g_gt_computed = 0, g_gt_evicted = 0;
+
+void gt_cache_clear() {
+  std::lock_guard<std::mutex> lock(g_gt_mutex);
+  g_gt_cache.clear();
+  g_gt_bytes = 0;
+}
+
+Tensor gt_maps_for(const Tensor& b, const Tensor& given, int B, int C, int H, int W, const DeviceScope& dev) {
+  if (b.requires_grad() || !b.is_same(given)) return Tensor();
+  std::lock_guard<std::mutex> lock(g_gt_mutex);
+  if (g_gt_cap == 0) return Tensor();
+  const void* key = b.data_ptr();
+  const uint32_t version = b._version();
+  auto it = g_gt_cache.find(key);
+  if (it != g_gt_cache.end()) {
+    GtEntry& e = it->second;
+    if (e.version == version && e.numel == b.numel() && e.c == C && e.h == H && e.w == W && e.gt.device() == b.device()) {
+      e.used = ++g_gt_tick;
+      ++g_gt_hits;
+      return e.maps;
+    }
+    g_gt_bytes -= e.bytes;
+    g_gt_cache.erase(it);
+  }
+  const size_t bytes = g_abi.gt_moments_bytes(B, C, H, W);
+  if (bytes > g_gt_cap) return Tensor();
+  while (g_gt_bytes + bytes > g_gt_cap && !g_gt_cache.empty()) {
+    auto old = g_gt_cache.begin();
+    for (auto j = g_gt_cache.begin(); j != g_gt_cache.end(); ++j)
+      if (j->second.used < old->second.used) old = j;
+    g_gt_bytes -= old->second.bytes;
+    g_gt_cache.erase(old);
+    ++g_gt_evicted;
+  }
+  GtEntry e;
+  e.gt = b.detach();
+  e.maps = empty_bytes(bytes, b);
+  e.version = version; e.numel = b.numel(); e.c = C; e.h = H; e.w = W; e.used = ++g_gt_tick; e.bytes = bytes;
+  check(g_abi.gt_moments(dev.stream, B, C, H, W, fp(b), e.maps.data_ptr()), "ssim_gt_moments");
+  ++g_gt_computed;
+  g_gt_bytes += bytes;
+  Tensor maps = e.maps;
+  g_gt_cache.emplace(key, std::move(e));
+  return maps;
+}
+
 struct L1SsimLossFn : public torch::autograd::Function<L1SsimLossFn> {
   static variable_list forward(AutogradContext* ctx, Tensor img1, Tensor img2, double lambda_dssim) {
     TORCH_CHECK(g_abi.bound, "mi355gs torch binding: bind() has not been called");
@@ -524,9 +592,15 @@
     Tensor out = at::empty({2}, a.options());
     Tensor loss = at::empty({}, a.options());
     Tensor grad = at::empty_like(a);
-    check(g_abi.l1_ssim_loss_fused(dev.stream, B, C, H, W, fp(a), fp(b), scratch.data_ptr(), (float)lambda_dssim, fp(out), fp(out) + 1,
-                                   fp(loss), fp(grad)),
-          "l1_ssim_loss_fused");
+    const Tensor maps = gt_maps_for(b, img2, B, C, H, W, dev);
+    if (maps.defined())
+      check(g_abi.l1_ssim_loss_fused_cached(dev.stream, B, C, H, W, fp(a), fp(b), maps.data_ptr(), scratch.data_ptr(), (float)lambda_dssim,
+                                            fp(out), fp(out) + 1, fp(loss), fp(grad)),
+            "l1_ssim_loss_fused_cached");
+    else
+      check(g_abi.l1_ssim_loss_fused(dev.stream, B, C, H, W, fp(a), fp(b), scratch.data_ptr(), (float)lambda_dssim, fp(out), fp(out) + 1,
+                                     fp(loss), fp(grad)),
+            "l1_ssim_loss_fused");
     ctx->save_for_backward({grad});
     ctx->mark_non_differentiable({out});
     ctx->set_materialize_grads(false);
@@ -579,7 +653,11 @@
   Tensor scratch = empty_bytes(g_abi.ssim_scratch_bytes(B, C, H, W), a);
   Tensor means = at::empty({2}, a.options());
   Tensor dmap = at::empty_like(a);
-  check(g_abi.pair_forward(dev.stream, B, C, H, W, fp(a), fp(b), scratch.data_ptr(), fp(dmap)), "l1_ssim_pair_forward");
+  const Tensor maps = gt_maps_for(b, img2, B, C, H, W, dev);
+  if (maps.defined())
+    check(g_abi.pair_forward_cached(dev.stream, B, C, H, W, fp(a), fp(b), maps.data_ptr(), scratch.data_ptr(), fp(dmap)), "l1_ssim_pair_forward_cached");
+  else
+    check(g_abi.pair_forward(dev.stream, B, C, H, W, fp(a), fp(b), scratch.data_ptr(), fp(dmap)), "l1_ssim_pair_forward");
   return {means, scratch, dmap, a, b};
 }
 
@@ -872,6 +950,17 @@
     if (reset) for (double& x : g_host_us) x = 0;
     return v;
   }, "accumulated host microseconds: render fwd (incl. the count wait), render bwd, loss fwd, loss bwd, adam step, count wait");
+  m.def("gt_cache_clear", &gt_cache_clear, "drop every kept ground-truth image and its window-moment maps");
+  m.def("gt_cache_cap", [](int64_t bytes) {
+    std::lock_guard<std::mutex> lock(g_gt_mutex);
+    const int64_t old = (int64_t)g_gt_cap;
+    if (bytes >= 0) g_gt_cap = (size_t)bytes;
+    return old;
+  }, "set the bound in bytes (0 = off; negative: query only) -> the previous bound; entries are dropped as later calls need room");
+  m.def("gt_cache_stats", []() {
+    std::lock_guard<std::mutex> lock(g_gt_mutex);
+    return std::vector<int64_t>{(int64_t)g_gt_cache.size(), (int64_t)g_gt_bytes, (int64_t)g_gt_hits, (int64_t)g_gt_computed, (int64_t)g_gt_evicted};
+  }, "-> [entries, bytes, hits, maps computed, evictions]");
   m.def("forget_gates", []() { std::lock_guard<std::mutex> lock(g_gate_mutex); g_gates = GateRecord(); });
   m.def("shared_zero_grad", [](bool on) {
     std::lock_guard<std::mutex> lock(g_zero_mutex);
diff --git a/instantsplat_amd/fused_ssim/__init__.py b/instantsplat_amd/fused_ssim/__init__.py
--- a/instantsplat_amd/fused_ssim/__init__.py
+++ b/instantsplat_amd/fused_ssim/__init__.py
@@ -3,6 +3,7 @@
 import torch
 
 from .. import _lib
+from .. import gt_cache
 from .. import lazy_loss
 
 
@@ -96,10 +97,16 @@
         loss = torch.empty((), dtype=torch.float32, device=dev)
         grad = torch.empty_like(a)
         p0 = out.data_ptr()
+        maps = gt_cache.maps_for(b, img2, B, C, H, W)
         with _lib.on_device(dev):
-            _lib.check(L.mi355gs_l1_ssim_loss_fused(_lib.stream_ptr(dev), B, C, H, W, _lib.ptr(a), _lib.ptr(b), _lib.ptr(scratch),
-                                                    float(lambda_dssim), p0, p0 + 4, _lib.ptr(loss), _lib.ptr(grad)),
-                       "l1_ssim_loss_fused")
+            if maps is not None:
+                _lib.check(L.mi355gs_l1_ssim_loss_fused_cached(_lib.stream_ptr(dev), B, C, H, W, _lib.ptr(a), _lib.ptr(b), _lib.ptr(maps),
+                                                               _lib.ptr(scratch), float(lambda_dssim), p0, p0 + 4, _lib.ptr(loss),
+                                                               _lib.ptr(grad)), "l1_ssim_loss_fused_cached")
+            else:
+                _lib.check(L.mi355gs_l1_ssim_loss_fused(_lib.stream_ptr(dev), B, C, H, W, _lib.ptr(a), _lib.ptr(b), _lib.ptr(scratch),
+                                                        float(lambda_dssim), p0, p0 + 4, _lib.ptr(loss), _lib.ptr(grad)),
+                           "l1_ssim_loss_fused")
         ctx.save_for_backward(grad)
         ctx.mark_non_differentiable(out)
         return loss, out
diff --git a/instantsplat_amd/gt_cache.py b/instantsplat_amd/gt_cache.py
--- /dev/null
+++ b/instantsplat_amd/gt_cache.py
@@ -0,0 +1,76 @@
+from __future__ import annotations
+
+import os
+from collections import OrderedDict
+
+import torch
+
+from . import _lib
+
+
+def _default_cap():
+    e = os.environ.get("MI355GS_GT_CACHE_MB", "")
+    if not e:
+        return 1 << 30
+    mb = float(e)
+    return int(mb * 1048576) if mb > 0 else 0
+
+
+_CAP = [_default_cap()]
+_ENTRIES = OrderedDict()
+_STATS = {"bytes": 0, "hits": 0, "computed": 0, "evicted": 0}
+
+
+def set_cap_bytes(n):
+    old = _CAP[0]
+    _CAP[0] = int(n)
+    if _lib._EXT is not None:
+        _lib._EXT.gt_cache_cap(int(n))
+    return old
+
+
+def clear():
+    _ENTRIES.clear()
+    _STATS["bytes"] = 0
+    if _lib._EXT is not None:
+        _lib._EXT.gt_cache_clear()
+
+
+def stats():
+    out = dict(_STATS, entries=len(_ENTRIES))
+    if _lib._EXT is not None:
+        n, b, h, c, e = _lib._EXT.gt_cache_stats()
+        out = {"entries": out["entries"] + n, "bytes": out["bytes"] + b, "hits": out["hits"] + h, "computed": out["computed"] + c,
+               "evicted": out["evicted"] + e}
+    return out
+
+
+def maps_for(b, given, B, C, H, W):
+    cap = _CAP[0]
+    if cap == 0 or b is not given or b.requires_grad:
+        return None
+    ptr = b.data_ptr()
+    key = (ptr, b._version, b.numel(), (C, H, W), b.device)
+    hit = _ENTRIES.get(ptr)
+    if hit is not None:
+        if hit[0] == key:
+            _ENTRIES.move_to_end(ptr)
+            _STATS["hits"] += 1
+            return hit[2]
+        _STATS["bytes"] -= hit[2].numel()
+        del _ENTRIES[ptr]
+    L = _lib.lib()
+    nbytes = int(L.mi355gs_ssim_gt_moments_bytes(B, C, H, W))
+    if nbytes > cap:
+        return None
+    while _ENTRIES and _STATS["bytes"] + nbytes > cap:
+        _, old = _ENTRIES.popitem(last=False)
+        _STATS["bytes"] -= old[2].numel()
+        _STATS["evicted"] += 1
+    maps = torch.empty(nbytes, dtype=torch.uint8, device=b.device)
+    with _lib.on_device(b.device):
+        _lib.check(L.mi355gs_ssim_gt_moments(_lib.stream_ptr(b.device), B, C, H, W, _lib.ptr(b), _lib.ptr(maps)), "ssim_gt_moments")
+    _ENTRIES[ptr] = (key, b.detach(), maps)
+    _STATS["bytes"] += nbytes
+    _STATS["computed"] += 1
+    return maps
diff --git a/instantsplat_amd/lazy_loss.py b/instantsplat_amd/lazy_loss.py
--- a/instantsplat_amd/lazy_loss.py
+++ b/instantsplat_amd/lazy_loss.py
@@ -8,6 +8,7 @@
 import torch
 
 from . import _lib
+from . import gt_cache
 
 ENABLED = os.environ.get("MI355GS_LAZY_LOSS", "1") != "0"
 
@@ -79,6 +80,7 @@
 
 def forget():
     _LAST[0] = None
+    gt_cache.clear()
 
 
 def _new(rec, prog):
@@ -347,9 +349,14 @@
     scratch = torch.empty(int(L.mi355gs_ssim_scratch_bytes(B, C, H, W)), dtype=torch.uint8, device=dev)
     means = torch.empty(2, dtype=torch.float32, device=dev)
     dmap = torch.empty_like(a)
+    maps = gt_cache.maps_for(b, img2, B, C, H, W)
     with _lib.on_device(dev):
-        _lib.check(L.mi355gs_l1_ssim_pair_forward(_lib.stream_ptr(dev), B, C, H, W, _lib.ptr(a), _lib.ptr(b), _lib.ptr(scratch),
-                                                  _lib.ptr(dmap)), "l1_ssim_pair_forward")
+        if maps is not None:
+            _lib.check(L.mi355gs_l1_ssim_pair_forward_cached(_lib.stream_ptr(dev), B, C, H, W, _lib.ptr(a), _lib.ptr(b), _lib.ptr(maps),
+                                                             _lib.ptr(scratch), _lib.ptr(dmap)), "l1_ssim_pair_forward_cached")
+        else:
+            _lib.check(L.mi355gs_l1_ssim_pair_forward(_lib.stream_ptr(dev), B, C, H, W, _lib.ptr(a), _lib.ptr(b), _lib.ptr(scratch),
+                                                      _lib.ptr(dmap)), "l1_ssim_pair_forward")
     return means, scratch, dmap, a, b
 
 
```

Result: no change. 3572, median of 4 (+0.5%).
